# mynameisfiber/baton

Measured on NVIDIA H100. Metric: federated local samples/sec (whole box), ResNet-18 FedAvg, synthetic non-IID 32x32 shards, higher is better.
Workload: dtype bf16

## Files before the change

### baton_b200/build_ext.py

```python
from __future__ import annotations

import os
import shutil
import subprocess
import sys
import sysconfig
import time
from concurrent.futures import ThreadPoolExecutor

HERE = os.path.dirname(os.path.abspath(__file__))
CSRC = os.path.join(HERE, "csrc")
BUILD = os.path.join(HERE, "csrc", "build")
TRACE = os.environ.get("BATON_BUILD_TRACE") == "1"
if TRACE:
    BUILD = os.path.join(HERE, "csrc", "build_trace")
TARGET = os.path.join(HERE, "_C_trace.so" if TRACE else "_C.so")

CU_SOURCES = ["gemm_wgmma.cu", "gemm_fp8.cu", "quant.cu", "attention.cu", "im2col_tma.cu", "gemm_simt.cu", "fedavg.cu", "elementwise.cu", "conv.cu", "norm.cu", "loss.cu", "conv_halo.cu"]
HEADERS = ["ptx.cuh", "launch.h", "pdl.cuh", "mx.cuh", "sgd.cuh", "dp.cuh", "epilogue.cuh"]
NVCC_FLAGS = ["-gencode", "arch=compute_90a,code=sm_90a", "-lineinfo", "-O3", "-std=c++17",
              "-Xcompiler", "-fPIC", "--use_fast_math", "-Xptxas", "-v"]
if os.environ.get("BATON_BUILD_PHASE_TIMING") == "1":
    NVCC_FLAGS.append("-DB200_FEDAVG_PHASE_TIMING")
if TRACE:
    NVCC_FLAGS += ["-DB200_TRACE", "-DB200_FEDAVG_PHASE_TIMING"]


def _nvcc() -> str:
    for cand in (os.environ.get("CUDA_HOME", "") + "/bin/nvcc", "/usr/local/cuda/bin/nvcc", shutil.which("nvcc") or ""):
        if cand and os.path.exists(cand):
            return cand
    raise RuntimeError("nvcc not found")


def _newer(src_paths, out_path) -> bool:
    if not os.path.exists(out_path):
        return True
    t = os.path.getmtime(out_path)
    return any(os.path.getmtime(p) > t for p in src_paths)


def _run(cmd, verbose, log_path=None):
    proc = subprocess.run(cmd, stdout=subprocess.PIPE, stderr=subprocess.STDOUT, text=True)
    if log_path:
        with open(log_path, "w") as f:
            f.write(" ".join(cmd) + "\n" + proc.stdout)
    if proc.returncode != 0:
        sys.stderr.write(proc.stdout)
        raise RuntimeError("build step failed: {}".format(" ".join(cmd[:3])))
    if verbose:
        sys.stdout.write(proc.stdout)


def build(force: bool = False, verbose: bool = False) -> str:
    import torch
    from torch.utils import cpp_extension

    os.makedirs(BUILD, exist_ok=True)
    nvcc = _nvcc()
    stamp = os.path.join(BUILD, "flags.txt")
    want = "\n".join([nvcc] + NVCC_FLAGS + [torch.__version__]) + "\n"
    if not force and (not os.path.exists(stamp) or open(stamp).read() != want):
        force = True
    headers = [os.path.join(CSRC, h) for h in HEADERS]
    t0 = time.time()
    jobs = []
    objs = []
    for cu in CU_SOURCES:
        src = os.path.join(CSRC, cu)
        obj = os.path.join(BUILD, cu.replace(".cu", ".o"))
        objs.append(obj)
        if force or _newer([src] + headers, obj):
            jobs.append(([nvcc] + NVCC_FLAGS + ["-I", CSRC, "-c", src, "-o", obj], obj + ".log"))
    bind_src = os.path.join(CSRC, "bindings.cpp")
    bind_obj = os.path.join(BUILD, "bindings.o")
    objs.append(bind_obj)
    if force or _newer([bind_src] + headers, bind_obj):
        inc = []
        for p in cpp_extension.include_paths("cuda") if hasattr(cpp_extension, "include_paths") else []:
            inc += ["-isystem", p]
        inc += ["-isystem", sysconfig.get_paths()["include"]]
        abi = int(getattr(torch._C, "_GLIBCXX_USE_CXX11_ABI", True))
        jobs.append((["g++", "-O2", "-std=c++17", "-fPIC", "-DTORCH_EXTENSION_NAME=_C",
                      "-DTORCH_API_INCLUDE_EXTENSION_H", "-D_GLIBCXX_USE_CXX11_ABI={}".format(abi),
                      "-I", CSRC] + inc + ["-c", bind_src, "-o", bind_obj], bind_obj + ".log"))
    if jobs:
        with ThreadPoolExecutor(max_workers=min(8, len(jobs))) as pool:
            list(pool.map(lambda j: _run(j[0], verbose, j[1]), jobs))
    if jobs or force or not os.path.exists(TARGET):
        torch_lib = os.path.join(os.path.dirname(torch.__file__), "lib")
        cuda_lib = os.path.join(os.path.dirname(os.path.dirname(nvcc)), "lib64")
        link = ["g++", "-shared", "-o", TARGET] + objs + [
            "-L" + torch_lib, "-L" + cuda_lib, "-lc10", "-lc10_cuda", "-ltorch_cpu", "-ltorch_cuda", "-ltorch",
            "-ltorch_python", "-lcudart", "-Wl,-rpath," + torch_lib, "-Wl,--no-as-needed"]
        _run(link, verbose)
    with open(stamp, "w") as fh:
        fh.write(want)
    if verbose:
        print("built {} in {:.1f}s ({} compile steps)".format(TARGET, time.time() - t0, len(jobs)))
    return TARGET


if __name__ == "__main__":
    build(force="--force" in sys.argv, verbose="--verbose" in sys.argv or "-v" in sys.argv)
    print(TARGET)
```

### baton_b200/csrc/bindings.cpp

```cpp
#include <ATen/cuda/CUDAContext.h>
#include <c10/cuda/CUDAGuard.h>
#include <torch/extension.h>

#include <optional>
#include <vector>

#include "launch.h"

namespace {

inline cudaStream_t cur_stream() { return at::cuda::getCurrentCUDAStream().stream(); }
inline void check(int rc, const char* what) {
  TORCH_CHECK(rc == 0, "baton_b200::", what, " failed with code ", rc,
              rc > 0 ? std::string(" (") + cudaGetErrorString(static_cast<cudaError_t>(rc)) + ")" : std::string());
}
inline const void* cptr(const at::Tensor& t) { return t.data_ptr(); }
inline void* ptr(at::Tensor& t) { return t.data_ptr(); }
template <class T>
inline T* opt_ptr(const std::optional<at::Tensor>& t) {
  return (t.has_value() && t->defined()) ? reinterpret_cast<T*>(t->data_ptr()) : nullptr;
}
#define CHECK_CUDA(x) TORCH_CHECK((x).is_cuda(), #x " must be a CUDA tensor")

inline const float* prox_anchor(const std::optional<at::Tensor>& anchor, int64_t numel, const at::Tensor& hyper) {
  if (!anchor.has_value() || !anchor->defined()) return nullptr;
  CHECK_CUDA(*anchor);
  TORCH_CHECK(anchor->scalar_type() == at::kFloat && anchor->is_contiguous() && anchor->numel() >= numel,
              "prox anchor: contiguous fp32 covering the parameters");
  TORCH_CHECK(hyper.numel() >= 5, "prox anchor: hyper needs 5 floats {lr, momentum, weight_decay, dampening, prox_mu}");
  return anchor->data_ptr<float>();
}

inline const float* scaf_corr(const std::optional<at::Tensor>& corr, int64_t numel, const float* anchor) {
  if (!corr.has_value() || !corr->defined()) return nullptr;
  CHECK_CUDA(*corr);
  TORCH_CHECK(corr->scalar_type() == at::kFloat && corr->is_contiguous() && corr->numel() >= numel,
              "scaffold correction: contiguous fp32 covering the parameters");
  TORCH_CHECK(anchor == nullptr, "an SGD step takes a FedProx anchor or a SCAFFOLD correction, not both");
  return corr->data_ptr<float>();
}

inline float* adam_v_ptr(const std::optional<at::Tensor>& v, int64_t numel, const float* mom, const at::Tensor& hyper,
                         const float* anchor, const float* corr) {
  if (!v.has_value() || !v->defined()) return nullptr;
  CHECK_CUDA(*v);
  TORCH_CHECK(v->scalar_type() == at::kFloat && v->is_contiguous() && v->numel() >= numel,
              "adamw second moment: contiguous fp32 covering the parameters");
  TORCH_CHECK(mom != nullptr, "an AdamW step needs the first-moment (momentum) buffer");
  TORCH_CHECK(hyper.numel() >= 12, "an AdamW step takes its step row (12 floats) as hyper");
  TORCH_CHECK(anchor == nullptr && corr == nullptr, "an AdamW step takes no FedProx anchor or SCAFFOLD correction");
  return v->data_ptr<float>();
}

inline std::optional<B200SgdEpilogue> sgd_epilogue(const std::optional<at::Tensor>& theta,
                                                   const std::optional<at::Tensor>& theta_bf16,
                                                   const std::optional<at::Tensor>& mom,
                                                   const std::optional<at::Tensor>& hyper, bool nesterov,
                                                   const std::optional<at::Tensor>& anchor,
                                                   const std::optional<at::Tensor>& corr,
                                                   const std::optional<at::Tensor>& adam_v) {
  if (!hyper.has_value() || !hyper->defined()) return std::nullopt;
  TORCH_CHECK(theta.has_value() && theta->scalar_type() == at::kFloat && hyper->scalar_type() == at::kFloat &&
                  (!theta_bf16.has_value() || theta_bf16->scalar_type() == at::kBFloat16) &&
                  (!mom.has_value() || mom->scalar_type() == at::kFloat),
              "sgd epilogue: fp32 theta / momentum / hyper, bf16 shadow");
  const float* a = prox_anchor(anchor, theta->numel(), *hyper);
  const float* c = scaf_corr(corr, 0, a);
  return B200SgdEpilogue{theta->data_ptr<float>(), opt_ptr<void>(theta_bf16), opt_ptr<float>(mom),
                         hyper->data_ptr<float>(), nesterov ? 1 : 0, a, c,
                         adam_v_ptr(adam_v, 0, opt_ptr<float>(mom), *hyper, a, c)};
}

inline std::optional<B200AffineEpilogue> affine_epilogue(const std::optional<at::Tensor>& scale,
                                                         const std::optional<at::Tensor>& shift,
                                                         const std::optional<at::Tensor>& residual, bool relu,
                                                         int64_t rows, int64_t N) {
  if (!scale.has_value() || !scale->defined()) return std::nullopt;
  TORCH_CHECK(shift.has_value() && shift->defined(), "affine epilogue: scale without shift");
  CHECK_CUDA(*scale); CHECK_CUDA(*shift);
  TORCH_CHECK(scale->scalar_type() == at::kFloat && shift->scalar_type() == at::kFloat &&
                  scale->is_contiguous() && shift->is_contiguous() && scale->numel() >= N && shift->numel() >= N,
              "affine epilogue: fp32 [N] scale / shift");
  long long ldr = 0;
  if (residual.has_value() && residual->defined()) {
    CHECK_CUDA(*residual);
    TORCH_CHECK(residual->scalar_type() == at::kBFloat16 && residual->stride(-1) == 1 && residual->size(-1) == N &&
                    residual->numel() >= rows * N,
                "affine epilogue: bf16 [rows, N] residual with unit inner stride");
    ldr = residual->dim() >= 2 ? residual->stride(-2) : N;
  }
  return B200AffineEpilogue{scale->data_ptr<float>(), shift->data_ptr<float>(), opt_ptr<const void>(residual), ldr,
                            relu ? 1 : 0};
}

extern "C" {
#define B200_TRACE_TUS(X) X(gemm_wgmma) X(gemm_fp8) X(quant) X(attention) X(im2col_tma) X(gemm_simt) X(fedavg) \
  X(elementwise) X(conv) X(norm) X(loss) X(conv_halo)
#define B200_DECL(tu) int b200_trace_set_##tu(unsigned long long* p);
B200_TRACE_TUS(B200_DECL)
#undef B200_DECL
}
bool trace_set(const std::optional<at::Tensor>& buf) {
  unsigned long long* p = nullptr;
  if (buf.has_value() && buf->defined()) {
    CHECK_CUDA(*buf);
    TORCH_CHECK(buf->scalar_type() == at::kLong && buf->is_contiguous() && buf->numel() >= 4, "trace buffer: int64 [2+2n]");
    p = reinterpret_cast<unsigned long long*>(buf->data_ptr());
  }
  int rc = 0;
#define B200_SET(tu) rc |= b200_trace_set_##tu(p);
  B200_TRACE_TUS(B200_SET)
#undef B200_SET
  return rc == 0;
}

bool gemm(const at::Tensor& a, const at::Tensor& b, at::Tensor d, const std::optional<at::Tensor>& bias, int64_t M,
          int64_t N, int64_t K, int64_t lda, int64_t ldb, int64_t ldd, bool a_mn, bool b_mn, int64_t act,
          int64_t split_k, bool accumulate, double alpha, const std::optional<at::Tensor>& flags, int64_t flag_epoch,
          int64_t flag_elem_off, int64_t flag_tile_elems, int64_t flag_bias_off, int64_t force_bn, bool simt,
          const std::optional<at::Tensor>& col_stats, const std::optional<at::Tensor>& flag_epoch_word,
          const std::optional<at::Tensor>& sgd_theta, const std::optional<at::Tensor>& sgd_theta_bf16,
          const std::optional<at::Tensor>& sgd_mom, const std::optional<at::Tensor>& sgd_hyper, bool sgd_nesterov,
          const std::optional<at::Tensor>& sgd_anchor, const std::optional<at::Tensor>& sgd_corr,
          const std::optional<at::Tensor>& sgd_v, const std::optional<at::Tensor>& bn_scale, const std::optional<at::Tensor>& bn_shift,
          const std::optional<at::Tensor>& residual, bool bn_relu) {
  CHECK_CUDA(a); CHECK_CUDA(b); CHECK_CUDA(d);
  TORCH_CHECK(a.scalar_type() == at::kBFloat16 && b.scalar_type() == at::kBFloat16, "gemm operands must be bf16");
  TORCH_CHECK(d.scalar_type() == at::kBFloat16 || d.scalar_type() == at::kFloat, "gemm output must be bf16/fp32");
  const c10::cuda::CUDAGuard guard(a.device());
  const int out_fp32 = d.scalar_type() == at::kFloat;
  const float* bp = opt_ptr<const float>(bias);
  TORCH_CHECK(!col_stats.has_value() || (!simt && col_stats->scalar_type() == at::kFloat && col_stats->numel() >= 2 * N),
              "col_stats needs the tensor-core path and a [2N] fp32 buffer");
  if (simt) {
    TORCH_CHECK(!sgd_hyper.has_value(), "the SIMT GEMM has no optimizer epilogue");
    TORCH_CHECK(!bn_scale.has_value(), "the SIMT GEMM has no BatchNorm epilogue");
    check(b200_gemm_simt(cptr(a), cptr(b), ptr(d), bp, M, N, K, lda, ldb, ldd, a_mn, b_mn, out_fp32, act, accumulate,
                         static_cast<float>(alpha), cur_stream()),
          "gemm_simt");
    return true;
  }
  const std::optional<B200SgdEpilogue> sgd =
      sgd_epilogue(sgd_theta, sgd_theta_bf16, sgd_mom, sgd_hyper, sgd_nesterov, sgd_anchor, sgd_corr, sgd_v);
  const std::optional<B200AffineEpilogue> affine = affine_epilogue(bn_scale, bn_shift, residual, bn_relu, M, N);
  const int rc = b200_gemm_bf16(cptr(a), cptr(b), ptr(d), bp, M, N, K, lda, ldb, ldd, a_mn, b_mn, out_fp32, act, split_k,
                                accumulate, static_cast<float>(alpha), opt_ptr<const uint32_t>(flags),
                                static_cast<uint32_t>(flag_epoch), flag_elem_off, static_cast<int>(flag_tile_elems),
                                flag_bias_off, static_cast<int>(force_bn), opt_ptr<float>(col_stats),
                                opt_ptr<const uint32_t>(flag_epoch_word), sgd ? &*sgd : nullptr,
                                affine ? &*affine : nullptr, cur_stream());
  if (rc == B200_SGD_EPILOGUE_DECLINED || rc == B200_AFFINE_EPILOGUE_DECLINED) return false;
  check(rc, "gemm_bf16");
  return true;
}

void gemm_batched(const at::Tensor& a, const at::Tensor& b, at::Tensor d, int64_t M, int64_t N, int64_t K, int64_t lda,
                  int64_t ldb, int64_t ldd, bool a_mn, bool b_mn, int64_t act, double alpha, int64_t n_outer,
                  int64_t n_inner, int64_t a_outer, int64_t a_inner, int64_t b_outer, int64_t b_inner, int64_t d_outer,
                  int64_t d_inner, bool accumulate) {
  CHECK_CUDA(a); CHECK_CUDA(b); CHECK_CUDA(d);
  TORCH_CHECK(a.scalar_type() == at::kBFloat16 && b.scalar_type() == at::kBFloat16, "gemm operands must be bf16");
  const c10::cuda::CUDAGuard guard(a.device());
  check(b200_gemm_bf16_batched(cptr(a), cptr(b), ptr(d), M, N, K, lda, ldb, ldd, a_mn, b_mn,
                               d.scalar_type() == at::kFloat, act, static_cast<float>(alpha), n_outer, n_inner, a_outer,
                               a_inner, b_outer, b_inner, d_outer, d_inner, accumulate, cur_stream()),
        "gemm_bf16_batched");
}

bool attention_fwd(const at::Tensor& qkv, at::Tensor out, at::Tensor probs, int64_t B, int64_t S, int64_t H, int64_t dh,
                   double scale) {
  CHECK_CUDA(qkv); CHECK_CUDA(out); CHECK_CUDA(probs);
  TORCH_CHECK(qkv.scalar_type() == at::kBFloat16 && out.scalar_type() == at::kBFloat16 &&
              probs.scalar_type() == at::kBFloat16 && qkv.is_contiguous() && out.is_contiguous() && probs.is_contiguous());
  const c10::cuda::CUDAGuard guard(qkv.device());
  const int rc = b200_attention_fwd(cptr(qkv), ptr(out), ptr(probs), static_cast<int>(B), static_cast<int>(S),
                                    static_cast<int>(H), static_cast<int>(dh), static_cast<float>(scale), cur_stream());
  if (rc == -2) return false;
  check(rc, "attention_fwd");
  return true;
}

bool im2col_tma_probe(const at::Tensor& x, at::Tensor col, int64_t kh, int64_t kw, int64_t stride, int64_t pad,
                      int64_t ho, int64_t wo) {
  CHECK_CUDA(x); CHECK_CUDA(col);
  TORCH_CHECK(x.scalar_type() == at::kBFloat16 && col.scalar_type() == at::kBFloat16 && x.dim() == 4 && x.is_contiguous() &&
              col.is_contiguous());
  const c10::cuda::CUDAGuard guard(x.device());
  const int rc = b200_im2col_tma_probe(cptr(x), ptr(col), static_cast<int>(x.size(0)), static_cast<int>(x.size(1)),
                                       static_cast<int>(x.size(2)), static_cast<int>(x.size(3)), static_cast<int>(kh),
                                       static_cast<int>(kw), static_cast<int>(stride), static_cast<int>(pad),
                                       static_cast<int>(ho), static_cast<int>(wo), cur_stream());
  if (rc == -2) return false;
  check(rc, "im2col_tma_probe");
  return true;
}

bool attention_bwd(const at::Tensor& qkv, const at::Tensor& dout, const at::Tensor& probs, at::Tensor dqkv, int64_t B,
                   int64_t S, int64_t H, int64_t dh, double scale) {
  CHECK_CUDA(qkv); CHECK_CUDA(dout); CHECK_CUDA(probs); CHECK_CUDA(dqkv);
  TORCH_CHECK(qkv.scalar_type() == at::kBFloat16 && dout.scalar_type() == at::kBFloat16 &&
              probs.scalar_type() == at::kBFloat16 && dqkv.scalar_type() == at::kBFloat16 && qkv.is_contiguous() &&
              dout.is_contiguous() && probs.is_contiguous() && dqkv.is_contiguous());
  const c10::cuda::CUDAGuard guard(qkv.device());
  const int rc = b200_attention_bwd(cptr(qkv), cptr(dout), cptr(probs), ptr(dqkv), static_cast<int>(B), static_cast<int>(S),
                                    static_cast<int>(H), static_cast<int>(dh), static_cast<float>(scale), cur_stream());
  if (rc == -2) return false;
  check(rc, "attention_bwd");
  return true;
}

bool conv_igemm_fwd(const at::Tensor& x, const at::Tensor& w, at::Tensor y, int64_t kh, int64_t kw, int64_t stride,
                    int64_t pad, int64_t ho, int64_t wo, int64_t cluster_k, int64_t force_bn,
                    const std::optional<at::Tensor>& col_stats, const std::optional<at::Tensor>& bn_scale,
                    const std::optional<at::Tensor>& bn_shift, const std::optional<at::Tensor>& residual, bool bn_relu) {
  CHECK_CUDA(x); CHECK_CUDA(w); CHECK_CUDA(y);
  TORCH_CHECK(x.scalar_type() == at::kBFloat16 && w.scalar_type() == at::kBFloat16 && y.scalar_type() == at::kBFloat16 &&
              x.dim() == 4 && x.is_contiguous() && w.is_contiguous() && y.is_contiguous());
  TORCH_CHECK(y.numel() == x.size(0) * ho * wo * w.size(0), "conv_igemm_fwd: y must hold [N*Ho*Wo, Cout] elements");
  const c10::cuda::CUDAGuard guard(x.device());
  const std::optional<B200AffineEpilogue> affine =
      affine_epilogue(bn_scale, bn_shift, residual, bn_relu, x.size(0) * ho * wo, w.size(0));
  const int rc = b200_conv_igemm_fwd(cptr(x), cptr(w), ptr(y), static_cast<int>(x.size(0)), static_cast<int>(x.size(1)),
                                     static_cast<int>(x.size(2)), static_cast<int>(x.size(3)), static_cast<int>(w.size(0)),
                                     static_cast<int>(kh), static_cast<int>(kw), static_cast<int>(stride),
                                     static_cast<int>(pad), static_cast<int>(ho), static_cast<int>(wo),
                                     static_cast<int>(cluster_k), static_cast<int>(force_bn), opt_ptr<float>(col_stats),
                                     affine ? &*affine : nullptr, cur_stream());
  if (rc == -2 || rc == B200_AFFINE_EPILOGUE_DECLINED) return false;
  check(rc, "conv_igemm_fwd");
  return true;
}
bool conv_igemm_dgrad(const at::Tensor& dy, const at::Tensor& w, at::Tensor dx, int64_t kh, int64_t kw, int64_t pad,
                      int64_t cluster_k, int64_t force_bn) {
  CHECK_CUDA(dy); CHECK_CUDA(w); CHECK_CUDA(dx);
  TORCH_CHECK(dy.scalar_type() == at::kBFloat16 && w.scalar_type() == at::kBFloat16 && dx.scalar_type() == at::kBFloat16 &&
              dy.dim() == 4 && dx.dim() == 4 && dy.is_contiguous() && w.is_contiguous() && dx.is_contiguous());
  const c10::cuda::CUDAGuard guard(dy.device());
  const int rc = b200_conv_igemm_dgrad(cptr(dy), cptr(w), ptr(dx), static_cast<int>(dx.size(0)), static_cast<int>(dx.size(1)),
                                       static_cast<int>(dx.size(2)), static_cast<int>(dx.size(3)), static_cast<int>(dy.size(3)),
                                       static_cast<int>(kh), static_cast<int>(kw), static_cast<int>(pad),
                                       static_cast<int>(dy.size(1)), static_cast<int>(dy.size(2)),
                                       static_cast<int>(cluster_k), static_cast<int>(force_bn), cur_stream());
  if (rc == -2) return false;
  check(rc, "conv_igemm_dgrad");
  return true;
}
bool conv_halo(const at::Tensor& src, const at::Tensor& w, at::Tensor out, bool dgrad, int64_t mc,
               const std::optional<at::Tensor>& col_stats) {
  CHECK_CUDA(src); CHECK_CUDA(w); CHECK_CUDA(out);
  TORCH_CHECK(src.scalar_type() == at::kBFloat16 && w.scalar_type() == at::kBFloat16 && out.scalar_type() == at::kBFloat16 &&
              src.dim() == 4 && src.size(3) == 64 && src.is_contiguous() && w.is_contiguous() && out.is_contiguous());
  const int64_t rows = src.size(0) * src.size(1) * src.size(2);
  TORCH_CHECK(rows > 0 && out.numel() % rows == 0, "conv_halo: out must hold [N*H*W, Nout] elements");
  const int64_t nout = out.numel() / rows;
  TORCH_CHECK(w.numel() == (dgrad ? 64 * 9 * nout : nout * 9 * 64), "conv_halo: w must be [Cout, 9*Cin]");
  TORCH_CHECK(dgrad ? !col_stats.has_value()
                    : (!col_stats.has_value() || (col_stats->scalar_type() == at::kFloat && col_stats->numel() >= 2 * nout)),
              "conv_halo: col_stats is a [2 Cout] fp32 buffer of the forward");
  const c10::cuda::CUDAGuard guard(src.device());
  const int rc = b200_conv_halo(cptr(src), cptr(w), ptr(out), static_cast<int>(src.size(0)), static_cast<int>(src.size(1)),
                                static_cast<int>(src.size(2)), static_cast<int>(nout), dgrad ? 1 : 0,
                                static_cast<int>(mc), opt_ptr<float>(col_stats), cur_stream());
  if (rc == -2) return false;
  check(rc, "conv_halo");
  return true;
}
bool conv_igemm_dgrad_s2(const at::Tensor& dy, const at::Tensor& w, at::Tensor dx, int64_t kh, int64_t kw,
                         const std::vector<int64_t>& ntaps, const std::vector<int64_t>& taps, int64_t force_bn) {
  CHECK_CUDA(dy); CHECK_CUDA(w); CHECK_CUDA(dx);
  TORCH_CHECK(dy.scalar_type() == at::kBFloat16 && w.scalar_type() == at::kBFloat16 && dx.scalar_type() == at::kBFloat16 &&
              dy.dim() == 4 && dx.dim() == 4 && dy.is_contiguous() && w.is_contiguous() && dx.is_contiguous());
  TORCH_CHECK(ntaps.size() == 4 && taps.size() == 16, "conv_igemm_dgrad_s2: 4 classes x 4 taps");
  int nt[4], tw[16];
  for (int i = 0; i < 4; ++i) nt[i] = static_cast<int>(ntaps[i]);
  for (int i = 0; i < 16; ++i) tw[i] = static_cast<int>(taps[i]);
  const c10::cuda::CUDAGuard guard(dy.device());
  const int rc = b200_conv_igemm_dgrad_s2(cptr(dy), cptr(w), ptr(dx), static_cast<int>(dx.size(0)),
                                          static_cast<int>(dx.size(1)), static_cast<int>(dx.size(2)),
                                          static_cast<int>(dx.size(3)), static_cast<int>(dy.size(3)), static_cast<int>(kh),
                                          static_cast<int>(kw), static_cast<int>(dy.size(1)), static_cast<int>(dy.size(2)),
                                          nt, tw, static_cast<int>(force_bn), cur_stream());
  if (rc == -2) return false;
  check(rc, "conv_igemm_dgrad_s2");
  return true;
}
bool conv_igemm_wgrad(const at::Tensor& dy, const at::Tensor& x, at::Tensor dw, int64_t cout, int64_t kh, int64_t kw,
                      int64_t stride, int64_t pad, int64_t ho, int64_t wo, int64_t split_k, int64_t force_bn,
                      const std::optional<at::Tensor>& sgd_theta, const std::optional<at::Tensor>& sgd_theta_bf16,
                      const std::optional<at::Tensor>& sgd_mom, const std::optional<at::Tensor>& sgd_hyper,
                      bool sgd_nesterov, const std::optional<at::Tensor>& sgd_anchor,
                      const std::optional<at::Tensor>& sgd_corr, const std::optional<at::Tensor>& sgd_v) {
  CHECK_CUDA(dy); CHECK_CUDA(x); CHECK_CUDA(dw);
  TORCH_CHECK(x.scalar_type() == at::kBFloat16 && dy.scalar_type() == at::kBFloat16 && dw.scalar_type() == at::kFloat &&
              x.dim() == 4 && x.is_contiguous() && dy.is_contiguous());
  const c10::cuda::CUDAGuard guard(x.device());
  const std::optional<B200SgdEpilogue> sgd =
      sgd_epilogue(sgd_theta, sgd_theta_bf16, sgd_mom, sgd_hyper, sgd_nesterov, sgd_anchor, sgd_corr, sgd_v);
  const int rc = b200_conv_igemm_wgrad(cptr(dy), cptr(x), dw.data_ptr<float>(), static_cast<int>(x.size(0)),
                                       static_cast<int>(x.size(1)), static_cast<int>(x.size(2)), static_cast<int>(x.size(3)),
                                       static_cast<int>(cout), static_cast<int>(kh), static_cast<int>(kw),
                                       static_cast<int>(stride), static_cast<int>(pad), static_cast<int>(ho),
                                       static_cast<int>(wo), static_cast<int>(split_k), static_cast<int>(force_bn),
                                       sgd ? &*sgd : nullptr, cur_stream());
  if (rc == -2 || rc == B200_SGD_EPILOGUE_DECLINED) return false;
  check(rc, "conv_igemm_wgrad");
  return true;
}

void gemm_fp8(const at::Tensor& a, const at::Tensor& b, at::Tensor d, const std::optional<at::Tensor>& bias,
              const std::optional<at::Tensor>& sfa, const std::optional<at::Tensor>& sfb, int64_t M, int64_t N, int64_t K,
              int64_t lda, int64_t ldb, int64_t ldd, int64_t act, int64_t split_k, bool accumulate, double alpha) {
  CHECK_CUDA(a); CHECK_CUDA(b); CHECK_CUDA(d);
  TORCH_CHECK(a.element_size() == 1 && b.element_size() == 1, "gemm_fp8 operands must be 1-byte (e4m3)");
  const c10::cuda::CUDAGuard guard(a.device());
  check(b200_gemm_fp8(cptr(a), cptr(b), ptr(d), opt_ptr<const float>(bias), opt_ptr<const void>(sfa),
                      opt_ptr<const void>(sfb), M, N, K, lda, ldb, ldd, d.scalar_type() == at::kFloat, act, split_k,
                      accumulate, static_cast<float>(alpha), cur_stream()),
        "gemm_fp8");
}
void quant_mx_rows(const at::Tensor& x, at::Tensor q, at::Tensor sf, int64_t R, int64_t C, int64_t ld_in, int64_t Cp) {
  CHECK_CUDA(x);
  const c10::cuda::CUDAGuard guard(x.device());
  check(b200_quant_mx_rows(x.data_ptr(), q.data_ptr(), sf.data_ptr(), R, C, ld_in, Cp, cur_stream()), "quant_mx_rows");
}
void quant_mx_cols(const at::Tensor& x, at::Tensor q, at::Tensor sf, int64_t R, int64_t C, int64_t ld_in, int64_t Rp) {
  CHECK_CUDA(x);
  const c10::cuda::CUDAGuard guard(x.device());
  check(b200_quant_mx_cols(x.data_ptr(), q.data_ptr(), sf.data_ptr(), R, C, ld_in, Rp, cur_stream()), "quant_mx_cols");
}
void dequant_mx(const at::Tensor& q, const at::Tensor& sf, at::Tensor out, int64_t R, int64_t C, int64_t Cp) {
  CHECK_CUDA(q);
  const c10::cuda::CUDAGuard guard(q.device());
  check(b200_dequant_mx(q.data_ptr(), sf.data_ptr(), out.data_ptr<float>(), R, C, Cp, cur_stream()), "dequant_mx");
}

void fused_sgd(at::Tensor w, at::Tensor g, const std::optional<at::Tensor>& mom, const std::optional<at::Tensor>& wb,
               const at::Tensor& hyper, bool zero_grad, bool nesterov, const std::optional<at::Tensor>& wire_slot,
               const std::optional<at::Tensor>& pack_global, const std::optional<at::Tensor>& pack_scale, int64_t n_pack,
               bool wire_fp32, const std::optional<at::Tensor>& prox_anchor_, const std::optional<at::Tensor>& corr,
               const std::optional<at::Tensor>& adam_v) {
  CHECK_CUDA(w);
  TORCH_CHECK(w.scalar_type() == at::kFloat && g.scalar_type() == at::kFloat && hyper.scalar_type() == at::kFloat);
  TORCH_CHECK(w.is_contiguous() && g.is_contiguous() && w.numel() == g.numel());
  const c10::cuda::CUDAGuard guard(w.device());
  const float* anchor = prox_anchor(prox_anchor_, w.numel(), hyper);
  const float* c = scaf_corr(corr, w.numel(), anchor);
  check(b200_fused_sgd(w.data_ptr<float>(), g.data_ptr<float>(), opt_ptr<float>(mom), opt_ptr<void>(wb), w.numel(),
                       hyper.data_ptr<float>(), zero_grad, nesterov,
                       reinterpret_cast<const unsigned long long*>(opt_ptr<const int64_t>(wire_slot)),
                       opt_ptr<const float>(pack_global), opt_ptr<const float>(pack_scale), n_pack, wire_fp32, anchor,
                       c, adam_v_ptr(adam_v, w.numel(), opt_ptr<float>(mom), hyper, anchor, c), cur_stream()),
        "fused_sgd");
}

void fused_sgd_segments(at::Tensor w, at::Tensor g, const std::optional<at::Tensor>& mom,
                        const std::optional<at::Tensor>& wb, const at::Tensor& segments, const at::Tensor& hyper,
                        bool nesterov, const std::optional<at::Tensor>& prox_anchor_,
                        const std::optional<at::Tensor>& corr, const std::optional<at::Tensor>& adam_v) {
  CHECK_CUDA(w); CHECK_CUDA(segments);
  TORCH_CHECK(w.scalar_type() == at::kFloat && g.scalar_type() == at::kFloat && hyper.scalar_type() == at::kFloat);
  TORCH_CHECK(segments.scalar_type() == at::kLong && segments.dim() == 2 && segments.size(1) == 3 &&
              segments.is_contiguous(), "segments: contiguous int64 [n, 3]");
  const c10::cuda::CUDAGuard guard(w.device());
  const float* anchor = prox_anchor(prox_anchor_, w.numel(), hyper);
  const float* c = scaf_corr(corr, g.numel(), anchor);
  check(b200_fused_sgd_segments(w.data_ptr<float>(), g.data_ptr<float>(), opt_ptr<float>(mom), opt_ptr<void>(wb),
                                reinterpret_cast<const long long*>(segments.data_ptr<int64_t>()),
                                static_cast<int>(segments.size(0)), hyper.data_ptr<float>(), nesterov, anchor, c,
                                adam_v_ptr(adam_v, g.numel(), opt_ptr<float>(mom), hyper, anchor, c), cur_stream()),
        "fused_sgd_segments");
}

inline void check_cv(const at::Tensor& t, int64_t n) {
  CHECK_CUDA(t);
  TORCH_CHECK(t.scalar_type() == at::kFloat && t.is_contiguous() && t.numel() >= n,
              "scaffold: contiguous fp32 buffers covering the parameters");
}
void scaffold_corr(at::Tensor corr, const at::Tensor& c, const at::Tensor& ci) {
  const int64_t n = corr.numel();
  check_cv(corr, n); check_cv(c, n); check_cv(ci, n);
  const c10::cuda::CUDAGuard guard(corr.device());
  check(b200_scaffold_corr(corr.data_ptr<float>(), c.data_ptr<float>(), ci.data_ptr<float>(), n, cur_stream()),
        "scaffold_corr");
}
void scaffold_dc(at::Tensor up, at::Tensor ci, const at::Tensor& c, const at::Tensor& global_w, const at::Tensor& theta,
                 double inv_k_eta, bool first) {
  const int64_t n = up.numel();
  check_cv(up, n); check_cv(ci, n); check_cv(c, n); check_cv(global_w, n); check_cv(theta, n);
  const c10::cuda::CUDAGuard guard(up.device());
  check(b200_scaffold_dc(up.data_ptr<float>(), ci.data_ptr<float>(), c.data_ptr<float>(), global_w.data_ptr<float>(),
                         theta.data_ptr<float>(), n, static_cast<float>(inv_k_eta), first ? 1 : 0, cur_stream()),
        "scaffold_dc");
}

void fold_client(at::Tensor acc, at::Tensor theta, const at::Tensor& global_w, const std::optional<at::Tensor>& wb,
                 const std::optional<at::Tensor>& mom, double nk, int64_t mode, bool reset) {
  CHECK_CUDA(acc);
  TORCH_CHECK(acc.scalar_type() == at::kFloat && theta.scalar_type() == at::kFloat && global_w.scalar_type() == at::kFloat);
  TORCH_CHECK(acc.numel() == theta.numel() && theta.numel() == global_w.numel());
  const c10::cuda::CUDAGuard guard(acc.device());
  check(b200_fold_client(acc.data_ptr<float>(), theta.data_ptr<float>(), global_w.data_ptr<float>(), opt_ptr<void>(wb),
                         opt_ptr<float>(mom), mom.has_value() && mom->defined() ? mom->numel() : 0, theta.numel(),
                         static_cast<float>(nk), static_cast<int>(mode), reset, cur_stream()),
        "fold_client");
}

void weighted_sum(at::Tensor dst, const std::vector<at::Tensor>& srcs, const std::vector<double>& weights) {
  CHECK_CUDA(dst);
  TORCH_CHECK(srcs.size() == weights.size() && !srcs.empty() && srcs.size() <= B200_MAX_RANKS);
  TORCH_CHECK(dst.is_contiguous());
  const c10::cuda::CUDAGuard guard(dst.device());
  std::vector<const void*> ps;
  std::vector<float> ws;
  for (size_t i = 0; i < srcs.size(); ++i) {
    TORCH_CHECK(srcs[i].is_cuda() && srcs[i].is_contiguous() && srcs[i].scalar_type() == dst.scalar_type() &&
                srcs[i].numel() == dst.numel());
    ps.push_back(srcs[i].data_ptr());
// ... 363 lines not shown
  if (rc == -2) return false;
  check(rc, "bn_relu_maxpool");
  return true;
}
bool bn_maxpool_bwd(const at::Tensor& z, const at::Tensor& p, const at::Tensor& arg, const at::Tensor& dy_a,
                    const std::optional<at::Tensor>& dy_b, at::Tensor dz, const std::optional<at::Tensor>& gamma,
                    const at::Tensor& mean, const at::Tensor& rstd, at::Tensor sums, const std::optional<at::Tensor>& dgamma,
                    const std::optional<at::Tensor>& dbeta, int64_t N, int64_t H, int64_t W, int64_t C, int64_t k,
                    int64_t stride, int64_t pad, int64_t Ho, int64_t Wo) {
  CHECK_CUDA(z);
  const c10::cuda::CUDAGuard guard(z.device());
  const int rc = b200_bn_maxpool_bwd(z.data_ptr(), p.data_ptr(), arg.data_ptr(), dy_a.data_ptr(), opt_ptr<const void>(dy_b),
                                     dz.data_ptr(), opt_ptr<const float>(gamma), mean.data_ptr<float>(),
                                     rstd.data_ptr<float>(), sums.data_ptr<float>(), opt_ptr<float>(dgamma),
                                     opt_ptr<float>(dbeta), static_cast<int>(N), static_cast<int>(H), static_cast<int>(W),
                                     static_cast<int>(C), static_cast<int>(k), static_cast<int>(stride),
                                     static_cast<int>(pad), static_cast<int>(Ho), static_cast<int>(Wo), cur_stream());
  if (rc == -2) return false;
  check(rc, "bn_maxpool_bwd");
  return true;
}
bool bn_bwd_cluster(const at::Tensor& x, const at::Tensor& y, const at::Tensor& dy_a, const std::optional<at::Tensor>& dy_b,
                    at::Tensor dx, const std::optional<at::Tensor>& dres, const std::optional<at::Tensor>& gamma,
                    const at::Tensor& mean, const at::Tensor& rstd, const std::optional<at::Tensor>& dgamma,
                    const std::optional<at::Tensor>& dbeta, int64_t rows, int64_t C, bool relu, int64_t max_cluster) {
  CHECK_CUDA(x);
  const c10::cuda::CUDAGuard guard(x.device());
  const int rc = b200_bn_bwd_cluster(x.data_ptr(), y.data_ptr(), dy_a.data_ptr(), opt_ptr<const void>(dy_b), dx.data_ptr(),
                                     opt_ptr<void>(dres), opt_ptr<const float>(gamma), mean.data_ptr<float>(),
                                     rstd.data_ptr<float>(), opt_ptr<float>(dgamma), opt_ptr<float>(dbeta), rows, C, relu,
                                     static_cast<int>(max_cluster), cur_stream());
  if (rc == -2) return false;
  check(rc, "bn_bwd_cluster");
  return true;
}
void bn_fold_eval(const at::Tensor& arena, const at::Tensor& table, at::Tensor out) {
  CHECK_CUDA(arena); CHECK_CUDA(table); CHECK_CUDA(out);
  TORCH_CHECK(arena.scalar_type() == at::kFloat && out.scalar_type() == at::kFloat && table.scalar_type() == at::kLong &&
                  table.dim() == 2 && table.size(1) == 7 && table.is_contiguous() && out.is_contiguous(),
              "bn_fold_eval: fp32 arena / out, int64 [n, 7] table");
  const c10::cuda::CUDAGuard guard(arena.device());
  check(b200_bn_fold_eval(arena.data_ptr<float>(), reinterpret_cast<const long long*>(table.data_ptr<int64_t>()),
                          static_cast<int>(table.size(0)), out.data_ptr<float>(), cur_stream()),
        "bn_fold_eval");
}
void layernorm_fwd(const at::Tensor& x, const std::optional<at::Tensor>& res, at::Tensor y, const at::Tensor& gamma,
                   const at::Tensor& beta, at::Tensor mean, at::Tensor rstd, int64_t rows, int64_t C, double eps) {
  CHECK_CUDA(x);
  const c10::cuda::CUDAGuard guard(x.device());
  check(b200_layernorm_fwd(x.data_ptr(), opt_ptr<const void>(res), y.data_ptr(), gamma.data_ptr<float>(),
                           beta.data_ptr<float>(), mean.data_ptr<float>(), rstd.data_ptr<float>(), rows, C,
                           static_cast<float>(eps), cur_stream()),
        "layernorm_fwd");
}
void layernorm_bwd(const at::Tensor& x, const at::Tensor& dy, at::Tensor dx, const at::Tensor& gamma,
                   const at::Tensor& mean, const at::Tensor& rstd, at::Tensor dgamma, at::Tensor dbeta, int64_t rows,
                   int64_t C) {
  CHECK_CUDA(x);
  const c10::cuda::CUDAGuard guard(x.device());
  check(b200_layernorm_bwd(x.data_ptr(), dy.data_ptr(), dx.data_ptr(), gamma.data_ptr<float>(), mean.data_ptr<float>(),
                           rstd.data_ptr<float>(), dgamma.data_ptr<float>(), dbeta.data_ptr<float>(), rows, C,
                           cur_stream()),
        "layernorm_bwd");
}
void softmax_fwd(const at::Tensor& x, at::Tensor y, int64_t rows, int64_t C, double scale) {
  CHECK_CUDA(x);
  const c10::cuda::CUDAGuard guard(x.device());
  check(b200_softmax_fwd(x.data_ptr(), y.data_ptr(), rows, C, static_cast<float>(scale), cur_stream()), "softmax_fwd");
}
void softmax_bwd(const at::Tensor& y, const at::Tensor& dy, at::Tensor dx, int64_t rows, int64_t C, double scale) {
  CHECK_CUDA(y);
  const c10::cuda::CUDAGuard guard(y.device());
  check(b200_softmax_bwd(y.data_ptr(), dy.data_ptr(), dx.data_ptr(), rows, C, static_cast<float>(scale), cur_stream()),
        "softmax_bwd");
}

void softmax_xent(const at::Tensor& logits, const at::Tensor& target, const std::optional<at::Tensor>& dlogits,
                  at::Tensor loss_acc, int64_t rows, int64_t C, int64_t ld, double grad_scale) {
  CHECK_CUDA(logits);
  TORCH_CHECK(target.scalar_type() == at::kLong && loss_acc.scalar_type() == at::kFloat && loss_acc.numel() >= 2);
  const c10::cuda::CUDAGuard guard(logits.device());
  const int in32 = logits.scalar_type() == at::kFloat;
  const int out32 = dlogits.has_value() && dlogits->defined() && dlogits->scalar_type() == at::kFloat;
  check(b200_softmax_xent(logits.data_ptr(), in32, reinterpret_cast<const long long*>(target.data_ptr<int64_t>()),
                          opt_ptr<void>(dlogits), out32, loss_acc.data_ptr<float>(), rows, C, ld,
                          static_cast<float>(grad_scale), cur_stream()),
        "softmax_xent");
}
bool linear_xent_head(const at::Tensor& x, const at::Tensor& w, const std::optional<at::Tensor>& bias, const at::Tensor& target,
                      const std::optional<at::Tensor>& dx, at::Tensor dw, const std::optional<at::Tensor>& db,
                      at::Tensor loss_acc, const std::optional<at::Tensor>& logits_out, double grad_scale) {
  CHECK_CUDA(x);
  TORCH_CHECK(x.scalar_type() == at::kBFloat16 && w.scalar_type() == at::kBFloat16 && x.dim() == 2 && w.dim() == 2 &&
              x.is_contiguous() && w.is_contiguous() && x.size(1) == w.size(1));
  TORCH_CHECK(target.scalar_type() == at::kLong && dw.scalar_type() == at::kFloat && dw.is_contiguous() &&
              dw.numel() == w.numel() && loss_acc.scalar_type() == at::kFloat && loss_acc.numel() >= 2);
  const c10::cuda::CUDAGuard guard(x.device());
  const int rc = b200_linear_xent_head(x.data_ptr(), w.data_ptr(), opt_ptr<const float>(bias),
                                       reinterpret_cast<const long long*>(target.data_ptr<int64_t>()), opt_ptr<void>(dx),
                                       dw.data_ptr<float>(), opt_ptr<float>(db), loss_acc.data_ptr<float>(),
                                       opt_ptr<float>(logits_out), static_cast<int>(x.size(0)), static_cast<int>(x.size(1)),
                                       static_cast<int>(w.size(0)), static_cast<float>(grad_scale), cur_stream());
  if (rc == -2) return false;
  check(rc, "linear_xent_head");
  return true;
}
bool linear_xent_eval(const at::Tensor& x, const at::Tensor& w, const std::optional<at::Tensor>& bias, const at::Tensor& target,
                      at::Tensor loss_acc, const std::optional<at::Tensor>& logits_out) {
  CHECK_CUDA(x);
  TORCH_CHECK(x.scalar_type() == at::kBFloat16 && w.scalar_type() == at::kBFloat16 && x.dim() == 2 && w.dim() == 2 &&
              x.is_contiguous() && w.is_contiguous() && x.size(1) == w.size(1));
  TORCH_CHECK(target.scalar_type() == at::kLong && target.numel() >= x.size(0) && loss_acc.scalar_type() == at::kFloat &&
              loss_acc.numel() >= 2);
  TORCH_CHECK(!bias.has_value() || (bias->scalar_type() == at::kFloat && bias->numel() == w.size(0)));
  TORCH_CHECK(!logits_out.has_value() || (logits_out->scalar_type() == at::kFloat && logits_out->is_contiguous() &&
                                          logits_out->numel() == x.size(0) * w.size(0)));
  const c10::cuda::CUDAGuard guard(x.device());
  const int rc = b200_linear_xent_eval(x.data_ptr(), w.data_ptr(), opt_ptr<const float>(bias),
                                       reinterpret_cast<const long long*>(target.data_ptr<int64_t>()),
                                       loss_acc.data_ptr<float>(), opt_ptr<float>(logits_out), static_cast<int>(x.size(0)),
                                       static_cast<int>(x.size(1)), static_cast<int>(w.size(0)), cur_stream());
  if (rc == -2) return false;
  check(rc, "linear_xent_eval");
  return true;
}
void mse(const at::Tensor& pred, const at::Tensor& target, const std::optional<at::Tensor>& dpred, at::Tensor loss_acc,
         double grad_scale) {
  CHECK_CUDA(pred);
  TORCH_CHECK(target.scalar_type() == at::kFloat && target.numel() == pred.numel());
  const c10::cuda::CUDAGuard guard(pred.device());
  const int in32 = pred.scalar_type() == at::kFloat;
  const int out32 = dpred.has_value() && dpred->defined() && dpred->scalar_type() == at::kFloat;
  check(b200_mse(pred.data_ptr(), in32, target.data_ptr<float>(), opt_ptr<void>(dpred), out32,
                 loss_acc.data_ptr<float>(), pred.numel(), static_cast<float>(grad_scale), cur_stream()),
        "mse");
}

}

PYBIND11_MODULE(TORCH_EXTENSION_NAME, m) {
  m.doc() = "baton_b200 sm_90a kernels";
  m.attr("MAX_RANKS") = B200_MAX_RANKS;
  m.def("gemm", &gemm);
  m.def("trace_set", &trace_set);
  m.def("attention_fwd", &attention_fwd);
  m.def("attention_bwd", &attention_bwd);
  m.def("bn_bwd_cluster", &bn_bwd_cluster);
  m.def("im2col_tma_probe", &im2col_tma_probe);
  m.def("conv_igemm_fwd", &conv_igemm_fwd);
  m.def("conv_igemm_wgrad", &conv_igemm_wgrad);
  m.def("conv_igemm_dgrad", &conv_igemm_dgrad);
  m.def("conv_igemm_dgrad_s2", &conv_igemm_dgrad_s2);
  m.def("conv_halo", &conv_halo);
  m.def("gemm_batched", &gemm_batched);
  m.def("gemm_fp8", &gemm_fp8);
  m.def("quant_mx_rows", &quant_mx_rows);
  m.def("quant_mx_cols", &quant_mx_cols);
  m.def("dequant_mx", &dequant_mx);
  m.def("fused_sgd", &fused_sgd);
  m.def("fused_sgd_segments", &fused_sgd_segments);
  m.def("weighted_sum", &weighted_sum);
  m.def("fold_client", &fold_client);
  m.def("scaffold_corr", &scaffold_corr);
  m.def("scaffold_dc", &scaffold_dc);
  m.def("cast", &cast);
  m.def("gather_rows", &gather_rows);
  m.def("colsum", &colsum);
  m.def("add_bf16", &add_bf16);
  m.def("relu_bwd", &relu_bwd);
  m.def("gelu", &gelu);
  m.def("gelu_bwd", &gelu_bwd);
  m.def("pad_rows", &pad_rows);
  m.def("embedding_bwd", &embedding_bwd);
  m.def("fedavg_allreduce", &fedavg_allreduce);
  m.def("fedavg_allreduce_robust", &fedavg_allreduce_robust);
  m.def("pack_client", &pack_client);
  m.attr("MAX_ROBUST_CLIENTS") = B200_MAX_ROBUST_CLIENTS;
  m.def("flag_barrier", &flag_barrier);
  m.attr("DP_WORK_WORDS") = B200_DP_WORK_WORDS;
  m.def("dp_clip_factor", &dp_clip_factor);
  m.def("fold_client_scaled", &fold_client_scaled);
  m.def("im2col", &im2col);
  m.def("col2im", &col2im);
  m.def("maxpool", &maxpool);
  m.def("maxpool_bwd", &maxpool_bwd);
  m.def("avgpool", &avgpool);
  m.def("avgpool_bwd", &avgpool_bwd);
  m.def("bn_stats", &bn_stats);
  m.def("bn_apply", &bn_apply);
  m.def("bn_bwd_reduce", &bn_bwd_reduce);
  m.def("bn_bwd_apply", &bn_bwd_apply);
  m.def("bn_relu_maxpool", &bn_relu_maxpool);
  m.def("bn_maxpool_bwd", &bn_maxpool_bwd);
  m.def("layernorm_fwd", &layernorm_fwd);
  m.def("layernorm_bwd", &layernorm_bwd);
  m.def("softmax_fwd", &softmax_fwd);
  m.def("softmax_bwd", &softmax_bwd);
  m.def("softmax_xent", &softmax_xent);
  m.def("mse", &mse);
  m.def("linear_xent_head", &linear_xent_head);
  m.def("linear_xent_eval", &linear_xent_eval);
  m.def("bn_fold_eval", &bn_fold_eval);
}
```

### baton_b200/csrc/epilogue.cuh

```cuda
#pragma once
#include "ptx.cuh"

namespace b200 {

__device__ __forceinline__ uint32_t cluster_ctarank() {
  uint32_t r;
  asm volatile("mov.u32 %0, %%cluster_ctarank;" : "=r"(r));
  return r;
}
__device__ __forceinline__ void cluster_sync_all() {
  asm volatile("barrier.cluster.arrive.release.aligned;" ::: "memory");
  asm volatile("barrier.cluster.wait.acquire.aligned;" ::: "memory");
}

#define COLSUM_STEP(OFF, HALF)                                                  \
  {                                                                             \
    const bool upper = (lane & (OFF)) != 0;                                     \
    _Pragma("unroll") for (int i = 0; i < (HALF); ++i) {                        \
      const float keep = upper ? t[i + (HALF)] : t[i];                          \
      const float send = upper ? t[i] : t[i + (HALF)];                          \
      t[i] = keep + __shfl_xor_sync(0xffffffffu, send, (OFF));                  \
    }                                                                           \
  }
__device__ __forceinline__ float warp_colsum32(float (&t)[32]) {
  const uint32_t lane = lane_id();
  COLSUM_STEP(16, 16) COLSUM_STEP(8, 8) COLSUM_STEP(4, 4) COLSUM_STEP(2, 2) COLSUM_STEP(1, 1)
  return t[0];
}
#undef COLSUM_STEP

__device__ __forceinline__ void stage_col_stats(float* sbuf, int BNv, int c, const float (&v)[32]) {
  float s[32], q[32];
#pragma unroll
  for (int j = 0; j < 32; ++j) {
    const float r = __bfloat162float(__float2bfloat16_rn(v[j]));
    s[j] = r;
    q[j] = r * r;
  }
  const float cs = warp_colsum32(s), cq = warp_colsum32(q);
  const int lane = static_cast<int>(lane_id());
  sbuf[c + lane] = cs;
  sbuf[BNv + c + lane] = cq;
}

}
```

### baton_b200/csrc/gemm_wgmma.cu

```cuda
#define B200_TU_TAG 1
#include "ptx.cuh"
#include "epilogue.cuh"
#include "launch.h"
#include "pdl.cuh"
#include "sgd.cuh"

namespace b200 {

constexpr int BM = 128;
constexpr int BK = 64;
constexpr int WG_K = 16;
constexpr int GEMM_THREADS = 384;
constexpr int CONSUMER_WARPS = 8;
constexpr int CONSUMER_THREADS = 32 * CONSUMER_WARPS;
constexpr int MAX_STAGES = 8;
constexpr int S2_MAX_TAPS = 4;

struct GemmParams {
  int M, N, K;
  void* D;
  long long ldd;
  const float* bias;
  int out_fp32;
  int act;
  float* col_stats;
  int a_mn, b_mn;
  int k_tiles_per_split;
  int atomic_out;
  int cluster_k;
  int stages;
  const uint32_t* tile_flags;
  uint32_t flag_epoch;
  long long flag_elem_off;
  int flag_tile_elems;
  long long flag_bias_off;
  long long ldb;
  float alpha;
  int batched, batch_inner;
  int batch_count;
  long long d_outer, d_inner;
  int conv_ho, conv_wo;
  int conv_stride, conv_pad;
  int conv_kw;
  int conv_cin;
  int conv_taps;
  int conv_ncol;
  const uint32_t* flag_epoch_ptr;
  const float* sgd_hyper = nullptr;
  float* sgd_theta = nullptr;
  __nv_bfloat16* sgd_wb = nullptr;
  float* sgd_mom = nullptr;
  int sgd_nesterov = 0;
  int conv_h = 0, conv_w = 0;
  int s2_ntaps[4] = {0, 0, 0, 0};
  int s2_tap[4][S2_MAX_TAPS] = {};
  const float* bn_scale = nullptr;
  const float* bn_shift = nullptr;
  const __nv_bfloat16* residual = nullptr;
  long long ldr = 0;
  const float* sgd_anchor = nullptr;
  const float* sgd_corr = nullptr;
  float* sgd_v = nullptr;
};

__device__ __forceinline__ void wait_arrival_flags(const uint32_t* flags, long long e0, long long e1, int granule,
                                                   uint32_t need) {
  for (long long t = e0 / granule; t <= e1 / granule; ++t) {
    unsigned long long spins = 0;
    while (static_cast<int32_t>(ld_acquire_sys(flags + t) - need) < 0) {
      if (++spins > (1ull << 26)) break;
    }
  }
}

template <int BN>
struct SmemLayout {
  static constexpr int A_BYTES = BM * BK * 2;
  static constexpr int B_BYTES = BN * BK * 2;
  static constexpr int STAGE_BYTES = A_BYTES + B_BYTES;
  static constexpr int PART_PITCH = BN + 4;
  static constexpr int PART_BYTES = BM * PART_PITCH * 4;
};

__device__ __forceinline__ float apply_act(float v, int act) {
  if (act == 1) return fmaxf(v, 0.f);
  if (act == 2) {
    const float k0 = 0.7978845608028654f, k1 = 0.044715f;
    float t = tanhf(k0 * (v + k1 * v * v * v));
    return 0.5f * v * (1.f + t);
  }
  return v;
}

__device__ __forceinline__ float4 ld_dsmem_f4(uint32_t local_smem_addr, uint32_t cta_rank) {
  uint32_t remote;
  asm volatile("mapa.shared::cluster.u32 %0, %1, %2;" : "=r"(remote) : "r"(local_smem_addr), "r"(cta_rank));
  float4 v;
  asm volatile("ld.shared::cluster.v4.f32 {%0, %1, %2, %3}, [%4];"
               : "=f"(v.x), "=f"(v.y), "=f"(v.z), "=f"(v.w)
               : "r"(remote)
               : "memory");
  return v;
}

__device__ __forceinline__ void accumulate_col_stats(const GemmParams& p, int col0, const float (&v)[32]) {
  float s[32], q[32];
#pragma unroll
  for (int j = 0; j < 32; ++j) {
    const float r = __bfloat162float(__float2bfloat16_rn(v[j]));
    s[j] = r;
    q[j] = r * r;
  }
  const float cs = warp_colsum32(s), cq = warp_colsum32(q);
  const int col = col0 + static_cast<int>(lane_id());
  if (col < p.N) {
    atomicAdd(p.col_stats + col, cs);
    atomicAdd(p.col_stats + p.N + col, cq);
  }
}

template <int NV, int ACT, bool BIAS>
__device__ __forceinline__ void transform_chunk_t(const GemmParams& p, int col0, float (&v)[NV]) {
  float b[NV];
  if (BIAS) {
    if (col0 + NV <= p.N && ((reinterpret_cast<uintptr_t>(p.bias + col0) & 15) == 0)) {
#pragma unroll
      for (int j = 0; j < NV; j += 4) {
        const float4 t = __ldg(reinterpret_cast<const float4*>(p.bias + col0 + j));
        b[j] = t.x; b[j + 1] = t.y; b[j + 2] = t.z; b[j + 3] = t.w;
      }
    } else {
#pragma unroll
      for (int j = 0; j < NV; ++j) b[j] = (col0 + j) < p.N ? __ldg(p.bias + col0 + j) : 0.f;
    }
  }
  const float alpha = p.alpha;
#pragma unroll
  for (int j = 0; j < NV; ++j) {
    float x = v[j] * alpha;
    if (BIAS) x += b[j];
    if (ACT == 1) x = fmaxf(x, 0.f);
    if (ACT == 2) {
      const float k0 = 0.7978845608028654f, k1 = 0.044715f;
      x = 0.5f * x * (1.f + tanhf(k0 * (x + k1 * x * x * x)));
    }
    v[j] = x;
  }
}
template <int NV>
__device__ __forceinline__ void transform_chunk(const GemmParams& p, int col0, float (&v)[NV]) {
  if (p.bias == nullptr) {
    if (p.act == 0) transform_chunk_t<NV, 0, false>(p, col0, v);
    else if (p.act == 1) transform_chunk_t<NV, 1, false>(p, col0, v);
    else transform_chunk_t<NV, 2, false>(p, col0, v);
  } else {
    if (p.act == 0) transform_chunk_t<NV, 0, true>(p, col0, v);
    else if (p.act == 1) transform_chunk_t<NV, 1, true>(p, col0, v);
    else transform_chunk_t<NV, 2, true>(p, col0, v);
  }
}

template <int NV>
__device__ __forceinline__ void affine_chunk(const GemmParams& p, int row, int col0, float (&v)[NV]) {
  static_assert(NV % 8 == 0, "affine epilogue works on groups of 8 columns");
  const bool relu = p.act == 1;
  const __nv_bfloat16* res = p.residual != nullptr ? p.residual + static_cast<size_t>(row) * p.ldr + col0 : nullptr;
#pragma unroll
  for (int j = 0; j < NV; j += 8) {
    if (col0 + j >= p.N) break;
    const float4 s0 = __ldg(reinterpret_cast<const float4*>(p.bn_scale + col0 + j));
    const float4 s1 = __ldg(reinterpret_cast<const float4*>(p.bn_scale + col0 + j + 4));
    const float4 h0 = __ldg(reinterpret_cast<const float4*>(p.bn_shift + col0 + j));
    const float4 h1 = __ldg(reinterpret_cast<const float4*>(p.bn_shift + col0 + j + 4));
    const float sc[8] = {s0.x, s0.y, s0.z, s0.w, s1.x, s1.y, s1.z, s1.w};
    const float sh[8] = {h0.x, h0.y, h0.z, h0.w, h1.x, h1.y, h1.z, h1.w};
    float r[8] = {0.f, 0.f, 0.f, 0.f, 0.f, 0.f, 0.f, 0.f};
    if (res != nullptr) {
      const uint4 rv = *reinterpret_cast<const uint4*>(res + j);
      const uint32_t rw[4] = {rv.x, rv.y, rv.z, rv.w};
#pragma unroll
      for (int i = 0; i < 4; ++i) {
        const float2 f = unpack_bf16x2(rw[i]);
        r[2 * i] = f.x;
        r[2 * i + 1] = f.y;
      }
    }
#pragma unroll
    for (int i = 0; i < 8; ++i) {
      const float x = fmaf(v[j + i], sc[i], sh[i]) + r[i];
      v[j + i] = relu ? fmaxf(x, 0.f) : x;
    }
  }
}

template <int NV, bool AFFINE = false>
__device__ __forceinline__ void store_row_chunk(const GemmParams& p, int row, int col0, float (&v)[NV], bool vec_ok,
                                                size_t d_off = 0) {
  if constexpr (AFFINE)
    affine_chunk<NV>(p, row, col0, v);
  else
    transform_chunk<NV>(p, col0, v);
  const bool full = (col0 + NV <= p.N);
  if (p.out_fp32) {
    float* d = reinterpret_cast<float*>(p.D) + d_off + static_cast<size_t>(row) * p.ldd + col0;
    if (p.atomic_out) {
      if (full && vec_ok) {
#pragma unroll
        for (int j = 0; j < NV; j += 4)
          asm volatile("red.global.add.v4.f32 [%0], {%1, %2, %3, %4};" ::"l"(d + j), "f"(v[j]), "f"(v[j + 1]),
                       "f"(v[j + 2]), "f"(v[j + 3])
                       : "memory");
      } else {
        _Pragma("unroll") for (int j = 0; j < NV; ++j) if (col0 + j < p.N) atomicAdd(d + j, v[j]);
      }
    } else if (full && vec_ok) {
#pragma unroll
      for (int j = 0; j < NV; j += 4) *reinterpret_cast<float4*>(d + j) = make_float4(v[j], v[j + 1], v[j + 2], v[j + 3]);
    } else {
      _Pragma("unroll") for (int j = 0; j < NV; ++j) if (col0 + j < p.N) d[j] = v[j];
    }
  } else {
    __nv_bfloat16* d = reinterpret_cast<__nv_bfloat16*>(p.D) + d_off + static_cast<size_t>(row) * p.ldd + col0;
    if (full && vec_ok) {
#pragma unroll
      for (int j = 0; j < NV; j += 8) {
        uint4 o;
        o.x = pack_bf16x2(v[j], v[j + 1]);
        o.y = pack_bf16x2(v[j + 2], v[j + 3]);
        o.z = pack_bf16x2(v[j + 4], v[j + 5]);
        o.w = pack_bf16x2(v[j + 6], v[j + 7]);
        *reinterpret_cast<uint4*>(d + j) = o;
      }
    } else {
      _Pragma("unroll") for (int j = 0; j < NV; ++j) if (col0 + j < p.N) d[j] = __float2bfloat16_rn(v[j]);
    }
  }
}

template <bool PROX, bool SCAF = false>
__device__ __forceinline__ void sgd_epilogue_chunk(const GemmParams& p, size_t e, int col0, const float (&v)[32],
                                                   bool vec);

__device__ __forceinline__ void adamw_epilogue_chunk(const GemmParams& p, size_t e, int col0, const float (&v)[32],
                                                     bool vec) {
  const AdamHyper h = load_adam_hyper(p.sgd_hyper);
  float* w = p.sgd_theta + e;
  float* m = p.sgd_mom + e;
  float* sq = p.sgd_v + e;
  __nv_bfloat16* wb = p.sgd_wb != nullptr ? p.sgd_wb + e : nullptr;
  if (vec && col0 + 32 <= p.N) {
#pragma unroll
    for (int j = 0; j < 32; j += 4) {
      float4 mv = *reinterpret_cast<const float4*>(m + j), vv = *reinterpret_cast<const float4*>(sq + j);
      const float4 gv = make_float4(__fadd_rn(0.f, v[j]), __fadd_rn(0.f, v[j + 1]), __fadd_rn(0.f, v[j + 2]),
                                    __fadd_rn(0.f, v[j + 3]));
      const float4 wv = adamw_update4(h, *reinterpret_cast<const float4*>(w + j), gv, mv, vv);
      *reinterpret_cast<float4*>(w + j) = wv;
// ... 1246 lines not shown
```

### baton_b200/csrc/launch.h

```cpp
#pragma once
#include <cuda_runtime.h>
#include <stdint.h>

#define B200_MAX_RANKS 16

extern "C" {

struct B200SgdEpilogue {
  float* theta;
  void* theta_bf16;
  float* mom;
  const float* hyper;
  int nesterov;
  const float* anchor;
  const float* corr;
  float* v;
};
#define B200_SGD_EPILOGUE_DECLINED (-6)

struct B200AffineEpilogue {
  const float* scale;
  const float* shift;
  const void* residual;
  long long ldr;
  int relu;
};
#define B200_AFFINE_EPILOGUE_DECLINED (-7)

int b200_gemm_bf16(const void* a, const void* b, void* d, const float* bias, int M, int N, int K, long long lda,
                   long long ldb, long long ldd, int a_mn, int b_mn, int out_fp32, int act, int split_k, int accumulate,
                   float alpha, const uint32_t* tile_flags, uint32_t flag_epoch, long long flag_elem_off, int flag_tile_elems,
                   long long flag_bias_off, int force_bn, float* col_stats, const uint32_t* flag_epoch_ptr,
                   const B200SgdEpilogue* sgd, const B200AffineEpilogue* affine, cudaStream_t stream);
int b200_gemm_bf16_batched(const void* a, const void* b, void* d, int M, int N, int K, long long lda, long long ldb,
                           long long ldd, int a_mn, int b_mn, int out_fp32, int act, float alpha, int n_outer,
                           int n_inner, long long a_outer, long long a_inner, long long b_outer, long long b_inner,
                           long long d_outer, long long d_inner, int accumulate, cudaStream_t stream);
int b200_attention_fwd(const void* qkv, void* out, void* probs, int B, int S, int H, int dh, float scale,
                       cudaStream_t stream);
int b200_attention_bwd(const void* qkv, const void* dout, const void* probs, void* dqkv, int B, int S, int H, int dh,
                       float scale, cudaStream_t stream);
int b200_conv_igemm_fwd(const void* x, const void* w, void* y, int N, int H, int W, int Cin, int Cout, int KH, int KW,
                        int stride, int pad, int Ho, int Wo, int cluster_k, int force_bn, float* col_stats,
                        const B200AffineEpilogue* affine, cudaStream_t stream);
int b200_conv_igemm_dgrad(const void* dy, const void* w, void* dx, int N, int H, int W, int Cin, int Cout, int KH, int KW,
                          int pad, int Ho, int Wo, int cluster_k, int force_bn, cudaStream_t stream);
int b200_conv_igemm_dgrad_s2(const void* dy, const void* w, void* dx, int N, int H, int W, int Cin, int Cout, int KH,
                             int KW, int Ho, int Wo, const int* ntaps, const int* taps, int force_bn, cudaStream_t stream);
int b200_conv_igemm_wgrad(const void* dy, const void* x, float* dw, int N, int H, int W, int Cin, int Cout, int KH, int KW,
                          int stride, int pad, int Ho, int Wo, int split_k, int force_bn, const B200SgdEpilogue* sgd,
                          cudaStream_t stream);
int b200_conv_halo(const void* src, const void* w, void* out, int N, int H, int W, int Nout, int dgrad, int mc,
                   float* col_stats, cudaStream_t stream);
int b200_im2col_tma_probe(const void* x, void* col, int N, int H, int W, int C, int KH, int KW, int stride, int pad,
                          int Ho, int Wo, cudaStream_t stream);
int b200_gemm_fp8(const void* a, const void* b, void* d, const float* bias, const void* sfa, const void* sfb, int M, int N,
                  int K, long long lda, long long ldb, long long ldd, int out_fp32, int act, int split_k, int accumulate,
                  float alpha, cudaStream_t stream);
int b200_quant_mx_rows(const void* x, void* q, void* sf, long long R, int C, long long ld_in, int Cp, cudaStream_t stream);
int b200_quant_mx_cols(const void* x, void* q, void* sf, long long R, int C, long long ld_in, long long Rp,
                       cudaStream_t stream);
int b200_dequant_mx(const void* q, const void* sf, float* out, long long R, int C, int Cp, cudaStream_t stream);
int b200_gemm_simt(const void* a, const void* b, void* d, const float* bias, int M, int N, int K, long long lda,
                   long long ldb, long long ldd, int a_mn, int b_mn, int out_fp32, int act, int accumulate,
                   float alpha, cudaStream_t stream);

int b200_fused_sgd(float* w, float* g, float* mom, void* w_bf16, long long n, const float* hyper, int zero_grad,
                   int nesterov, const unsigned long long* wire_slot, const float* pack_global,
                   const float* pack_scale, long long n_pack, int wire_fp32, const float* prox_anchor,
                   const float* corr, float* adam_v, cudaStream_t stream);
int b200_fused_sgd_segments(float* w, float* g, float* mom, void* w_bf16, const long long* segments, int n_seg,
                            const float* hyper, int nesterov, const float* prox_anchor, const float* corr,
                            float* adam_v, cudaStream_t stream);
int b200_scaffold_corr(float* corr, const float* c, const float* ci, long long n, cudaStream_t stream);
int b200_scaffold_dc(float* up, float* ci, const float* c, const float* global_w, const float* theta, long long n,
                     float inv_k_eta, int first, cudaStream_t stream);
int b200_fold_client(float* acc, float* theta, const float* global_w, void* w_bf16, float* mom, long long n_mom, long long n,
                     float nk, int mode, int reset, cudaStream_t stream);
int b200_weighted_sum(void* dst, const void* const* srcs, const float* weights, int n_src, long long n, int dtype,
                      cudaStream_t stream);
int b200_cast_f32_bf16(const float* src, void* dst, long long n, cudaStream_t stream);
int b200_cast_bf16_f32(const void* src, float* dst, long long n, cudaStream_t stream);
int b200_gather_rows(const void* src, const long long* idx, void* dst, long long n_rows, long long row_bytes,
                     cudaStream_t stream);
int b200_gather_rows_i64(const long long* src, const long long* idx, long long* dst, long long n,
                         cudaStream_t stream);
int b200_colsum(const void* x, float* out, long long rows, int cols, int accumulate, cudaStream_t stream);
int b200_add_bf16(const void* a, const void* b, void* out, long long n, int relu, cudaStream_t stream);
int b200_relu_bwd_bf16(const void* y, const void* dy, void* dx, long long n, cudaStream_t stream);
int b200_gelu_bf16(const void* x, void* y, long long n, cudaStream_t stream);
int b200_gelu_bwd_bf16(const void* x, const void* dy, void* dx, long long n, cudaStream_t stream);
int b200_embedding_bwd(const void* dy, const long long* idx, float* grad, long long n_rows, int width,
                       cudaStream_t stream);
int b200_pad_rows_bf16(const void* src, void* dst, long long rows, int k, int kp, const uint32_t* flags,
                       const uint32_t* epoch_word, long long elem_off, int granule, cudaStream_t stream);

struct FedAvgArgs {
  void* wire[B200_MAX_RANKS];
  unsigned long long* pads[B200_MAX_RANKS];
  void* wire_mc;
  float* theta;
  float* global_w;
  void* theta_bf16;
  float* momentum;
  long long n_momentum;
  long long* int_local;
  long long* int_wire[B200_MAX_RANKS];
  float* loss_local;
  float* loss_wire[B200_MAX_RANKS];
  float* loss_out;
  int n_loss;
  float n_samples[B200_MAX_RANKS];
  int counts_from_flags;
  float nvls_prescale;
  uint32_t alive_mask;
  int rank, world;
  long long n;
  int n_int;
  int wire_kind;
  int delta;
  int use_nvls;
  uint32_t epoch;
  uint32_t* tile_flags;
  uint32_t flag_value;
  int tile_elems;
  int prepacked;
  int timeout_log2;
  int* status;
  unsigned long long* phase_ns;
};
struct FedAvgDPArgs : FedAvgArgs {
  const float* clip_page[B200_MAX_RANKS];
  float noise_std;
  unsigned long long seed;
  uint32_t round;
};
struct FedAvgScaffoldArgs : FedAvgArgs {
  const float* dc;
  float* c;
  long long n_c;
  long long seg1_off;
  float inv_clients;
};
#define B200_MAX_ROBUST_CLIENTS 32
struct FedAvgRobustArgs : FedAvgArgs {
  uint32_t* seg_page[B200_MAX_RANKS];
  uint32_t my_segs;
  long long seg_stride;
  int kind;
  uint8_t trim_b[B200_MAX_ROBUST_CLIENTS + 1];
};
int b200_fedavg_allreduce(const FedAvgArgs* args, int n_ctas, cudaStream_t stream);
int b200_fedavg_allreduce_robust(const FedAvgRobustArgs* args, int n_ctas, cudaStream_t stream);
int b200_pack_client(void* seg, float* theta, const float* global_w, void* w_bf16, float* mom, long long n_mom,
                     long long n, int wire_kind, int reset, cudaStream_t stream);
int b200_fedavg_allreduce_dp(const FedAvgDPArgs* args, int n_ctas, cudaStream_t stream);
int b200_fedavg_allreduce_scaffold(const FedAvgScaffoldArgs* args, int n_ctas, cudaStream_t stream);
#define B200_DP_NORM_BLOCKS 264
#define B200_DP_WORK_WORDS (B200_DP_NORM_BLOCKS + 1)
int b200_dp_clip_factor(const float* theta, const float* global_w, long long n, float clip, void* work, float* s_out,
                        float* norm_out, float* s_copy, int* nonfinite, cudaStream_t stream);
int b200_fold_client_scaled(float* acc, float* theta, const float* global_w, void* w_bf16, float* mom, long long n_mom,
                            long long n, const float* s, int first, int reset, cudaStream_t stream);
int b200_flag_barrier(unsigned long long* const* pads, int rank, int world, uint32_t alive_mask, uint32_t epoch,
                      int slot, cudaStream_t stream);

int b200_im2col_nhwc(const void* x, void* col, int N, int H, int W, int C, int KH, int KW, int stride, int pad,
                     int Ho, int Wo, int kp, cudaStream_t stream);
int b200_col2im_nhwc(const void* col, void* dx, int N, int H, int W, int C, int KH, int KW, int stride, int pad,
                     int Ho, int Wo, int kp, cudaStream_t stream);
int b200_maxpool_nhwc(const void* x, void* y, int* argmax, int N, int H, int W, int C, int k, int stride, int pad,
                      int Ho, int Wo, int arg_u8, cudaStream_t stream);
int b200_maxpool_bwd_nhwc(const void* dy, const void* dy_b, const int* argmax, void* dx, int N, int H, int W, int C, int Ho,
                          int Wo, int k, int stride, int pad, int arg_u8, cudaStream_t stream);
int b200_avgpool_nhwc(const void* x, void* y, int N, int HW, int C, cudaStream_t stream);
int b200_avgpool_bwd_nhwc(const void* dy, void* dx, int N, int HW, int C, cudaStream_t stream);

int b200_bn_stats(const void* x, float* sums, long long rows, int C, cudaStream_t stream);
int b200_bn_apply(const void* x, const void* residual, void* y, float* sums, const float* gamma, const float* beta,
                  float* running_mean, float* running_var, float* save_mean, float* save_rstd, long long* nbt,
                  long long rows, int C, float eps, float momentum, int relu, int training, cudaStream_t stream);
int b200_bn_bwd_reduce(const void* x, const void* y, const void* dy, const float* save_mean, const float* save_rstd,
                       float* sums, long long rows, int C, int relu, cudaStream_t stream);
int b200_bn_bwd_apply(const void* x, const void* y, const void* dy, void* dx, void* dres, const float* gamma,
                      const float* save_mean, const float* save_rstd, float* sums, float* dgamma, float* dbeta,
                      long long rows, int C, int relu, cudaStream_t stream);
int b200_bn_relu_maxpool(const void* z, void* p, void* argmax, const float* sums, const float* gamma, const float* beta,
                         float* running_mean, float* running_var, float* save_mean, float* save_rstd, long long* nbt, int N,
                         int H, int W, int C, int k, int stride, int pad, int Ho, int Wo, float eps, float momentum,
                         cudaStream_t stream);
int b200_bn_maxpool_bwd(const void* z, const void* p, const void* argmax, const void* dy_a, const void* dy_b, void* dz,
                        const float* gamma, const float* save_mean, const float* save_rstd, float* sums, float* dgamma,
                        float* dbeta, int N, int H, int W, int C, int k, int stride, int pad, int Ho, int Wo,
                        cudaStream_t stream);
int b200_bn_bwd_cluster(const void* x, const void* y, const void* dy_a, const void* dy_b, void* dx, void* dres,
                        const float* gamma, const float* save_mean, const float* save_rstd, float* dgamma, float* dbeta,
                        long long rows, int C, int relu, int max_cluster, cudaStream_t stream);
int b200_bn_fold_eval(const float* arena, const long long* table, int n_bn, float* out, cudaStream_t stream);
int b200_layernorm_fwd(const void* x, const void* residual, void* y, const float* gamma, const float* beta,
                       float* mean, float* rstd, long long rows, int C, float eps, cudaStream_t stream);
int b200_layernorm_bwd(const void* x, const void* dy, void* dx, const float* gamma, const float* mean,
                       const float* rstd, float* dgamma, float* dbeta, long long rows, int C, cudaStream_t stream);
int b200_softmax_fwd(const void* x, void* y, long long rows, int C, float scale, cudaStream_t stream);
int b200_softmax_bwd(const void* y, const void* dy, void* dx, long long rows, int C, float scale,
                     cudaStream_t stream);

int b200_softmax_xent(const void* logits, int logits_fp32, const long long* target, void* dlogits, int dl_fp32,
                      float* loss_acc, long long rows, int C, long long ld, float grad_scale, cudaStream_t stream);
int b200_linear_xent_head(const void* x, const void* w, const float* bias, const long long* target, void* dx, float* dw,
                          float* db, float* loss_acc, float* logits_out, int rows, int K, int NC, float grad_scale,
                          cudaStream_t stream);
int b200_linear_xent_eval(const void* x, const void* w, const float* bias, const long long* target, float* loss_acc,
                          float* logits_out, int rows, int K, int NC, cudaStream_t stream);
int b200_mse(const void* pred, int pred_fp32, const float* target, void* dpred, int dp_fp32, float* loss_acc,
             long long n, float grad_scale, cudaStream_t stream);
}
```

### baton_b200/csrc/norm.cu

```cuda
#define B200_TU_TAG 10
#include "launch.h"
#include "pdl.cuh"
#include "ptx.cuh"

namespace b200 {

__device__ __forceinline__ uint32_t cluster_ctarank_any() {
  uint32_t r;
  asm volatile("mov.u32 %0, %%cluster_ctarank;" : "=r"(r));
  return r;
}
__device__ __forceinline__ uint32_t cluster_nctarank_y() {
  uint32_t r;
  asm volatile("mov.u32 %0, %%cluster_nctarank;" : "=r"(r));
  return r;
}
__device__ __forceinline__ void cluster_arrive_norm() { asm volatile("barrier.cluster.arrive.release.aligned;" ::: "memory"); }
__device__ __forceinline__ void cluster_wait_norm() { asm volatile("barrier.cluster.wait.acquire.aligned;" ::: "memory"); }
__device__ __forceinline__ void cluster_sync_all_norm() {
  cluster_arrive_norm();
  cluster_wait_norm();
}
__device__ __forceinline__ float ld_dsmem_f1(uint32_t local_smem_addr, uint32_t cta_rank) {
  uint32_t remote;
// ... 489 lines not shown
          s1 += w;
          s2 = fmaf(w, h, s2);
        }
      }
    }
    s1 = group_sum<LPR>(s1) / C;
    s2 = group_sum<LPR>(s2) / C;
    if (row_ok) {
      uint4* dr = reinterpret_cast<uint4*>(dx + row * C);
#pragma unroll
      for (int k = 0; k < VPL; ++k) {
        const int idx = gl + k * LPR;
        if (idx < nvec) {
          float o[8];
#pragma unroll
          for (int j = 0; j < 8; ++j) o[j] = rs * (gw[k][j] - s1 - xh[k][j] * s2);
          dr[idx] = pack8(o);
        }
      }
    }
  }
#pragma unroll
  for (int k = 0; k < VPL; ++k) {
    const int idx = gl + k * LPR;
    if (idx < nvec) {
#pragma unroll
      for (int j = 0; j < 8; ++j) {
        atomicAdd(sg + idx * 8 + j, dg[k][j]);
        atomicAdd(sb + idx * 8 + j, db[k][j]);
      }
    }
  }
  __syncthreads();
  for (int c = threadIdx.x; c < C; c += blockDim.x) {
    atomicAdd(dgamma + c, sg[c]);
    atomicAdd(dbeta + c, sb[c]);
  }
}

template <int LPR, int VPL>
__global__ void __launch_bounds__(256)
softmax_fwd_vec_kernel(const __nv_bfloat16* __restrict__ x, __nv_bfloat16* __restrict__ y, long long rows, int C,
                       float scale) {
  griddep_launch_dependents();
  griddep_wait();
  constexpr int RPW = 32 / LPR;
  const int gl = threadIdx.x & (LPR - 1);
  const long long row = (blockIdx.x * static_cast<long long>(blockDim.x >> 5) + (threadIdx.x >> 5)) * RPW +
                        ((threadIdx.x & 31) / LPR);
  const bool row_ok = row < rows;
  const int nvec = C >> 3;
  const uint4* xr = reinterpret_cast<const uint4*>(x + (row_ok ? row : 0) * C);
  float v[VPL][8];
  float m = -INFINITY;
#pragma unroll
  for (int k = 0; k < VPL; ++k) {
    const int idx = gl + k * LPR;
    if (row_ok && idx < nvec) {
      unpack8(__ldcs(xr + idx), v[k]);
#pragma unroll
      for (int j = 0; j < 8; ++j) {
        v[k][j] *= scale;
        m = fmaxf(m, v[k][j]);
      }
    }
  }
  m = group_max<LPR>(m);
  float s = 0.f;
#pragma unroll
  for (int k = 0; k < VPL; ++k)
    if (row_ok && gl + k * LPR < nvec) {
#pragma unroll
      for (int j = 0; j < 8; ++j) {
        v[k][j] = __expf(v[k][j] - m);
        s += v[k][j];
      }
    }
  s = group_sum<LPR>(s);
  if (!row_ok) return;
  const float inv = 1.f / s;
  uint4* yr = reinterpret_cast<uint4*>(y + row * C);
#pragma unroll
  for (int k = 0; k < VPL; ++k) {
    const int idx = gl + k * LPR;
    if (idx < nvec) {
#pragma unroll
      for (int j = 0; j < 8; ++j) v[k][j] *= inv;
      yr[idx] = pack8(v[k]);
    }
  }
}

template <int LPR, int VPL>
__global__ void __launch_bounds__(256)
softmax_bwd_vec_kernel(const __nv_bfloat16* __restrict__ y, const __nv_bfloat16* __restrict__ dy,
                       __nv_bfloat16* __restrict__ dx, long long rows, int C, float scale) {
  griddep_launch_dependents();
  griddep_wait();
  constexpr int RPW = 32 / LPR;
  const int gl = threadIdx.x & (LPR - 1);
  const long long row = (blockIdx.x * static_cast<long long>(blockDim.x >> 5) + (threadIdx.x >> 5)) * RPW +
                        ((threadIdx.x & 31) / LPR);
  const bool row_ok = row < rows;
  const int nvec = C >> 3;
  const uint4* yr = reinterpret_cast<const uint4*>(y + (row_ok ? row : 0) * C);
  const uint4* gr = reinterpret_cast<const uint4*>(dy + (row_ok ? row : 0) * C);
  float p[VPL][8], g[VPL][8];
  float s = 0.f;
#pragma unroll
  for (int k = 0; k < VPL; ++k) {
    const int idx = gl + k * LPR;
    if (row_ok && idx < nvec) {
      unpack8(__ldcs(yr + idx), p[k]);
      unpack8(__ldcs(gr + idx), g[k]);
#pragma unroll
      for (int j = 0; j < 8; ++j) s = fmaf(p[k][j], g[k][j], s);
    }
  }
  s = group_sum<LPR>(s);
  if (!row_ok) return;
  uint4* dr = reinterpret_cast<uint4*>(dx + row * C);
#pragma unroll
  for (int k = 0; k < VPL; ++k) {
    const int idx = gl + k * LPR;
    if (idx < nvec) {
      float o[8];
#pragma unroll
      for (int j = 0; j < 8; ++j) o[j] = scale * p[k][j] * (g[k][j] - s);
      dr[idx] = pack8(o);
    }
  }
}

#define ROW_DISPATCH(C, CALL)                                     \
  do {                                                           \
    const int nvec_ = (C) >> 3;                                  \
    if (nvec_ <= 8) { CALL(8, 1); }                              \
    else if (nvec_ <= 16) { CALL(16, 1); }                       \
    else if (nvec_ <= 32) { CALL(32, 1); }                       \
    else if (nvec_ <= 64) { CALL(32, 2); }                       \
    else if (nvec_ <= 96) { CALL(32, 3); }                       \
    else { CALL(32, 4); }                                        \
  } while (0)
static inline bool row_vec_ok(int C, const void* a, const void* b, const void* c) {
  return C % 8 == 0 && C <= 1024 && ((reinterpret_cast<uintptr_t>(a) | reinterpret_cast<uintptr_t>(b) |
                                       reinterpret_cast<uintptr_t>(c)) & 15) == 0;
}
static inline int rows_per_block(int C) {
  const int nvec = C >> 3;
  return 8 * (nvec <= 8 ? 4 : (nvec <= 16 ? 2 : 1));
}


__device__ __forceinline__ void unpack8_bn(const uint4& u, float (&f)[8]) {
  const float2 a = unpack_bf16x2(u.x), b = unpack_bf16x2(u.y), c = unpack_bf16x2(u.z), d = unpack_bf16x2(u.w);
  f[0] = a.x; f[1] = a.y; f[2] = b.x; f[3] = b.y; f[4] = c.x; f[5] = c.y; f[6] = d.x; f[7] = d.y;
}
__device__ __forceinline__ void colred_finish(float (&a)[8], float (&q)[8], float* sm, int tpr, int cg, int rg,
                                              float* __restrict__ sums, int C) {
  float* mine = sm + static_cast<size_t>(rg) * 2 * C + cg * 8;
#pragma unroll
  for (int j = 0; j < 8; ++j) { mine[j] = a[j]; mine[C + j] = q[j]; }
  __syncthreads();
  const int rpp = 256 / tpr;
  for (int c = threadIdx.x; c < 2 * C; c += 256) {
    float t = 0.f;
    for (int r = 0; r < rpp; ++r) t += sm[static_cast<size_t>(r) * 2 * C + c];
    atomicAdd(sums + c, t);
  }
}

__global__ void __launch_bounds__(256)
bn_stats_vec_kernel(const uint4* __restrict__ x, float* __restrict__ sums, long long rows, int C, int rows_per_cta) {
  griddep_launch_dependents();
  griddep_wait();
  extern __shared__ float sm[];
  const int tpr = C >> 3, rpp = 256 / tpr;
  const int cg = threadIdx.x % tpr, rg = threadIdx.x / tpr;
  const long long r0 = static_cast<long long>(blockIdx.x) * rows_per_cta;
  long long r1 = r0 + rows_per_cta;
  if (r1 > rows) r1 = rows;
  float a[8], q[8];
#pragma unroll
  for (int j = 0; j < 8; ++j) { a[j] = 0.f; q[j] = 0.f; }
  for (long long r = r0 + rg; r < r1; r += 4ll * rpp) {
    uint4 v[4];
#pragma unroll
    for (int u = 0; u < 4; ++u)
      if (r + static_cast<long long>(u) * rpp < r1) v[u] = x[(r + static_cast<long long>(u) * rpp) * tpr + cg];
#pragma unroll
    for (int u = 0; u < 4; ++u)
      if (r + static_cast<long long>(u) * rpp < r1) {
        float f[8];
        unpack8_bn(v[u], f);
#pragma unroll
        for (int j = 0; j < 8; ++j) { a[j] += f[j]; q[j] = fmaf(f[j], f[j], q[j]); }
      }
  }
  colred_finish(a, q, sm, tpr, cg, rg, sums, C);
}

__global__ void __launch_bounds__(256)
bn_bwd_reduce_vec_kernel(const uint4* __restrict__ x, const uint4* __restrict__ y, const uint4* __restrict__ dy,
                         const float* __restrict__ mean, const float* __restrict__ rstd, float* __restrict__ sums,
                         long long rows, int C, int relu, int rows_per_cta) {
  griddep_launch_dependents();
  griddep_wait();
  extern __shared__ float sm[];
  const int tpr = C >> 3, rpp = 256 / tpr;
  const int cg = threadIdx.x % tpr, rg = threadIdx.x / tpr;
  const long long r0 = static_cast<long long>(blockIdx.x) * rows_per_cta;
  long long r1 = r0 + rows_per_cta;
  if (r1 > rows) r1 = rows;
  float m[8], rs[8], a[8], q[8];
#pragma unroll
  for (int j = 0; j < 8; ++j) { m[j] = mean[cg * 8 + j]; rs[j] = rstd[cg * 8 + j]; a[j] = 0.f; q[j] = 0.f; }
  for (long long r = r0 + rg; r < r1; r += 2ll * rpp) {
    uint4 xv[2], gv[2], yv[2];
#pragma unroll
    for (int u = 0; u < 2; ++u) {
      const long long rr = r + static_cast<long long>(u) * rpp;
      if (rr < r1) {
        xv[u] = x[rr * tpr + cg];
        gv[u] = dy[rr * tpr + cg];
        if (relu) yv[u] = y[rr * tpr + cg];
      }
    }
#pragma unroll
    for (int u = 0; u < 2; ++u) {
      if (r + static_cast<long long>(u) * rpp < r1) {
        float xf[8], gf[8];
        unpack8_bn(xv[u], xf);
        unpack8_bn(gv[u], gf);
        if (relu) {
          float yf[8];
          unpack8_bn(yv[u], yf);
#pragma unroll
          for (int j = 0; j < 8; ++j)
            if (!(yf[j] > 0.f)) gf[j] = 0.f;
        }
#pragma unroll
        for (int j = 0; j < 8; ++j) {
          a[j] += gf[j];
          q[j] = fmaf(gf[j], (xf[j] - m[j]) * rs[j], q[j]);
        }
      }
    }
  }
  colred_finish(a, q, sm, tpr, cg, rg, sums, C);
}


constexpr int BNC_CW = 16;
constexpr int BNC_LANES = 128;

template <int ITER>
__global__ void __launch_bounds__(256)
bn_bwd_cluster_kernel(const uint4* __restrict__ x, const uint4* __restrict__ y, const uint4* __restrict__ dy_a,
                      const uint4* __restrict__ dy_b, uint4* __restrict__ dx, uint4* __restrict__ dres,
                      const float* __restrict__ gamma, const float* __restrict__ mean, const float* __restrict__ rstd,
                      float* __restrict__ dgamma, float* __restrict__ dbeta, int rows, int C, int relu, int rows_per_cta) {
  griddep_launch_dependents();
  __shared__ float wpart[8][2][16];
  __shared__ __align__(16) float cpart[32];
  __shared__ float tot[32];
  const int chunk = threadIdx.x & 1, lane_r = threadIdx.x >> 1;
  const int c0 = blockIdx.x * BNC_CW + chunk * 8;
  const int C8 = C >> 3;
  const uint32_t S = cluster_nctarank_y();
  const uint32_t me = cluster_ctarank_any();
  const int r_begin = static_cast<int>(me) * rows_per_cta;
  int r_end = r_begin + rows_per_cta;
  if (r_end > rows) r_end = rows;
  float m[8], rs[8];
#pragma unroll
  for (int j = 0; j < 8; ++j) { m[j] = mean[c0 + j]; rs[j] = rstd[c0 + j]; }
  griddep_wait();
  constexpr int NC = ITER > 0 ? ITER : 1;
  float xh[NC][8], g[NC][8];
  float sg[8], sgx[8];
#pragma unroll
  for (int j = 0; j < 8; ++j) { sg[j] = 0.f; sgx[j] = 0.f; }
  auto load_row = [&](int r, float (&xh_)[8], float (&g_)[8]) {
    const long long i = static_cast<long long>(r) * C8 + (c0 >> 3);
    float xf[8];
    unpack8_bn(x[i], xf);
    unpack8_bn(dy_a[i], g_);
    if (dy_b != nullptr) {
      float t[8];
      unpack8_bn(dy_b[i], t);
#pragma unroll
      for (int j = 0; j < 8; ++j) g_[j] += t[j];
    }
    if (relu) {
      float yf[8];
      unpack8_bn(y[i], yf);
#pragma unroll
      for (int j = 0; j < 8; ++j)
        if (!(yf[j] > 0.f)) g_[j] = 0.f;
    }
#pragma unroll
    for (int j = 0; j < 8; ++j) xh_[j] = (xf[j] - m[j]) * rs[j];
  };
  if constexpr (ITER > 0) {
#pragma unroll
    for (int it = 0; it < ITER; ++it) {
      const int r = r_begin + it * BNC_LANES + lane_r;
      if (r < r_end) {
        load_row(r, xh[it], g[it]);
#pragma unroll
// ... 416 lines not shown
    cudaGetLastError();
  }
  if (S > 8 && !np16) return -2;
  cudaLaunchConfig_t cfg = {};
  cfg.gridDim = grid;
  cfg.blockDim = dim3(256);
  cfg.dynamicSmemBytes = 0;
  cfg.stream = stream;
  cudaLaunchAttribute attr[2];
  int na = 0;
  if (pdl_enabled()) {
    attr[na].id = cudaLaunchAttributeProgrammaticStreamSerialization;
    attr[na].val.programmaticStreamSerializationAllowed = 1;
    ++na;
  }
  if (S > 1) {
    attr[na].id = cudaLaunchAttributeClusterDimension;
    attr[na].val.clusterDim.x = 1;
    attr[na].val.clusterDim.y = static_cast<unsigned>(S);
    attr[na].val.clusterDim.z = 1;
    ++na;
  }
  cfg.attrs = attr;
  cfg.numAttrs = na;
  cudaError_t e = cudaLaunchKernelEx(&cfg, bn_bwd_cluster_kernel<ITER>, x, y, dy_a, dy_b, dx, dres, gamma, mean, rstd, dgamma,
                                     dbeta, rows, C, relu, rpc);
  if (e != cudaSuccess) return static_cast<int>(e);
  return static_cast<int>(cudaGetLastError());
}

extern "C" int b200_bn_bwd_cluster(const void* x, const void* y, const void* dy_a, const void* dy_b, void* dx, void* dres,
                                   const float* gamma, const float* save_mean, const float* save_rstd, float* dgamma,
                                   float* dbeta, long long rows, int C, int relu, int max_cluster, cudaStream_t stream) {
  const bool allow_uncached = max_cluster < 0;
  if (max_cluster < 0) max_cluster = -max_cluster;
  if (rows <= 0) return 0;
  const uintptr_t al = reinterpret_cast<uintptr_t>(x) | reinterpret_cast<uintptr_t>(relu ? y : x) |
                       reinterpret_cast<uintptr_t>(dy_a) | reinterpret_cast<uintptr_t>(dy_b) |
                       reinterpret_cast<uintptr_t>(dx) | reinterpret_cast<uintptr_t>(dres);
  if (C % BNC_CW != 0 || (al & 15) || rows > (1ll << 30)) return -2;
  if (max_cluster <= 0 || max_cluster > 16) max_cluster = 16;
  const int slices = C / BNC_CW;
  int S = 1;
  while (S < max_cluster && (rows + S - 1) / S > BNC_LANES) S <<= 1;
  while (S > 1 && static_cast<long long>(slices) * S > 2 * device_sm_count()) S >>= 1;
  const int rpc = static_cast<int>((rows + S - 1) / S);
  const int iters = (rpc + BNC_LANES - 1) / BNC_LANES;
  const dim3 grid(static_cast<unsigned>(slices), static_cast<unsigned>(S));
#define BNC_GO(I)                                                                                                        \
  return launch_bn_bwd_cluster<I>(grid, S, stream, reinterpret_cast<const uint4*>(x), reinterpret_cast<const uint4*>(y), \
                                  reinterpret_cast<const uint4*>(dy_a), reinterpret_cast<const uint4*>(dy_b),            \
                                  reinterpret_cast<uint4*>(dx), reinterpret_cast<uint4*>(dres), gamma, save_mean,        \
                                  save_rstd, dgamma, dbeta, static_cast<int>(rows), C, relu, rpc)
  if (iters <= 1) BNC_GO(1);
  if (iters <= 2) BNC_GO(2);
  if (iters <= 4) BNC_GO(4);
  if (iters <= 8) BNC_GO(8);
  if (!allow_uncached) return -2;
  BNC_GO(0);
#undef BNC_GO
}

extern "C" int b200_layernorm_fwd(const void* x, const void* residual, void* y, const float* gamma, const float* beta,
                                  float* mean, float* rstd, long long rows, int C, float eps, cudaStream_t stream) {
  if (rows <= 0) return 0;
  if (C > 32 * LN_MAX_PER_LANE) return -2;
  const __nv_bfloat16* xp = reinterpret_cast<const __nv_bfloat16*>(x);
  const __nv_bfloat16* rp = reinterpret_cast<const __nv_bfloat16*>(residual);
  __nv_bfloat16* yp = reinterpret_cast<__nv_bfloat16*>(y);
  if (row_vec_ok(C, x, residual, y) && ((reinterpret_cast<uintptr_t>(gamma) | reinterpret_cast<uintptr_t>(beta)) & 15) == 0) {
    const int rpb = rows_per_block(C);
    const unsigned grid = static_cast<unsigned>((rows + rpb - 1) / rpb);
#define LN_FWD(LPR, VPL) launch_pdl(layernorm_fwd_vec_kernel<LPR, VPL>, grid, 256, 0, stream, xp, rp, yp, gamma, beta, mean, rstd, rows, C, eps)
    ROW_DISPATCH(C, LN_FWD);
#undef LN_FWD
    RET_LAST();
  }
  const int warps = 8;
  launch_pdl(layernorm_fwd_kernel, static_cast<unsigned>((rows + warps - 1) / warps), warps * 32, 0, stream, xp, rp, yp,
             gamma, beta, mean, rstd, rows, C, eps);
  RET_LAST();
}
extern "C" int b200_layernorm_bwd(const void* x, const void* dy, void* dx, const float* gamma, const float* mean,
                                  const float* rstd, float* dgamma, float* dbeta, long long rows, int C,
                                  cudaStream_t stream) {
  if (rows <= 0) return 0;
  if (C > 32 * LN_MAX_PER_LANE) return -2;
  const __nv_bfloat16* xp = reinterpret_cast<const __nv_bfloat16*>(x);
  const __nv_bfloat16* gp = reinterpret_cast<const __nv_bfloat16*>(dy);
  __nv_bfloat16* dp = reinterpret_cast<__nv_bfloat16*>(dx);
  if (row_vec_ok(C, x, dy, dx) && (reinterpret_cast<uintptr_t>(gamma) & 15) == 0) {
    const int rpb = rows_per_block(C);
    long long gv = (rows + rpb - 1) / rpb;
    if (gv > device_sm_count() * 2) gv = device_sm_count() * 2;
#define LN_BWD(LPR, VPL) launch_pdl(layernorm_bwd_vec_kernel<LPR, VPL>, static_cast<unsigned>(gv), 256, 2 * C * sizeof(float), stream, xp, gp, dp, gamma, mean, rstd, dgamma, dbeta, rows, C)
    ROW_DISPATCH(C, LN_BWD);
#undef LN_BWD
    RET_LAST();
  }
  long long g = (rows + 7) / 8;
  if (g > device_sm_count() * 2) g = device_sm_count() * 2;
  launch_pdl(layernorm_bwd_kernel, static_cast<unsigned>(g), 256, 2 * C * sizeof(float), stream, xp, gp, dp, gamma, mean,
             rstd, dgamma, dbeta, rows, C);
  RET_LAST();
}
extern "C" int b200_softmax_fwd(const void* x, void* y, long long rows, int C, float scale, cudaStream_t stream) {
  if (rows <= 0) return 0;
  if (C > 32 * LN_MAX_PER_LANE) return -2;
  const __nv_bfloat16* xp = reinterpret_cast<const __nv_bfloat16*>(x);
  __nv_bfloat16* yp = reinterpret_cast<__nv_bfloat16*>(y);
  if (row_vec_ok(C, x, y, nullptr)) {
    const int rpb = rows_per_block(C);
    const unsigned grid = static_cast<unsigned>((rows + rpb - 1) / rpb);
#define SM_FWD(LPR, VPL) launch_pdl(softmax_fwd_vec_kernel<LPR, VPL>, grid, 256, 0, stream, xp, yp, rows, C, scale)
    ROW_DISPATCH(C, SM_FWD);
#undef SM_FWD
    RET_LAST();
  }
  launch_pdl(softmax_fwd_kernel, static_cast<unsigned>((rows + 7) / 8), 256, 0, stream, xp, yp, rows, C, scale);
  RET_LAST();
}
extern "C" int b200_softmax_bwd(const void* y, const void* dy, void* dx, long long rows, int C, float scale,
                                cudaStream_t stream) {
  if (rows <= 0) return 0;
  if (C > 32 * LN_MAX_PER_LANE) return -2;
  const __nv_bfloat16* yp = reinterpret_cast<const __nv_bfloat16*>(y);
  const __nv_bfloat16* gp = reinterpret_cast<const __nv_bfloat16*>(dy);
  __nv_bfloat16* dp = reinterpret_cast<__nv_bfloat16*>(dx);
  if (row_vec_ok(C, y, dy, dx)) {
    const int rpb = rows_per_block(C);
    const unsigned grid = static_cast<unsigned>((rows + rpb - 1) / rpb);
#define SM_BWD(LPR, VPL) launch_pdl(softmax_bwd_vec_kernel<LPR, VPL>, grid, 256, 0, stream, yp, gp, dp, rows, C, scale)
    ROW_DISPATCH(C, SM_BWD);
#undef SM_BWD
    RET_LAST();
  }
  launch_pdl(softmax_bwd_kernel, static_cast<unsigned>((rows + 7) / 8), 256, 0, stream, yp, gp, dp, rows, C, scale);
  RET_LAST();
}


extern "C" int b200_bn_relu_maxpool(const void* z, void* p, void* argmax, const float* sums, const float* gamma,
                                    const float* beta, float* running_mean, float* running_var, float* save_mean,
                                    float* save_rstd, long long* nbt, int N, int H, int W, int C, int k, int stride, int pad,
                                    int Ho, int Wo, float eps, float momentum, cudaStream_t stream) {
  if (C % 8 || k * k > 255) return -2;
  const long long total = static_cast<long long>(N) * Ho * Wo * (C / 8);
  if (total <= 0) return 0;
  launch_pdl(bn_relu_maxpool_kernel, stream_grid(total), 256, 2 * C * sizeof(float), stream,
             reinterpret_cast<const uint4*>(z), reinterpret_cast<uint4*>(p), reinterpret_cast<uint2*>(argmax), sums, gamma,
             beta, running_mean, running_var, save_mean, save_rstd, nbt, N, H, W, C, k, stride, pad, Ho, Wo, eps, momentum);
  RET_LAST();
}
extern "C" int b200_bn_maxpool_bwd(const void* z, const void* p, const void* argmax, const void* dy_a, const void* dy_b,
                                   void* dz, const float* gamma, const float* save_mean, const float* save_rstd, float* sums,
                                   float* dgamma, float* dbeta, int N, int H, int W, int C, int k, int stride, int pad, int Ho,
                                   int Wo, cudaStream_t stream) {
  if (k * k > 255 || !colred_vec_ok(C, z, p, dy_a) || (dy_b != nullptr && (reinterpret_cast<uintptr_t>(dy_b) & 15)))
    return -2;
  const long long prow = static_cast<long long>(N) * Ho * Wo;
  if (prow <= 0) return 0;
  int rpc = 2 * (256 / (C >> 3));
  if (rpc < colred_rows_per_cta(prow, C, 2)) rpc = colred_rows_per_cta(prow, C, 2);
  launch_pdl(bn_maxpool_bwd_reduce_kernel, static_cast<unsigned>((prow + rpc - 1) / rpc), 256, 256 * 16 * sizeof(float),
             stream, reinterpret_cast<const __nv_bfloat16*>(z), reinterpret_cast<const uint4*>(p),
             reinterpret_cast<const uint2*>(argmax), reinterpret_cast<const uint4*>(dy_a),
             reinterpret_cast<const uint4*>(dy_b), save_mean, save_rstd, sums, N, H, W, C, k, stride, pad, Ho, Wo, rpc);
  cudaError_t e = cudaGetLastError();
  if (e != cudaSuccess) return static_cast<int>(e);
  const long long total = static_cast<long long>(N) * H * W * (C / 8);
  launch_pdl(bn_maxpool_bwd_apply_kernel, stream_grid(total), 256, 5 * C * sizeof(float), stream,
             reinterpret_cast<const uint4*>(z), reinterpret_cast<const uint4*>(p), reinterpret_cast<const uint2*>(argmax),
             reinterpret_cast<const uint4*>(dy_a), reinterpret_cast<const uint4*>(dy_b), reinterpret_cast<uint4*>(dz), gamma,
             save_mean, save_rstd, sums, dgamma, dbeta, N, H, W, C, k, stride, pad, Ho, Wo);
  RET_LAST();
}

B200_TRACE_REGISTER(norm)
```

### baton_b200/csrc/ptx.cuh

```cuda
#pragma once
#include <cuda.h>
#include <cuda_bf16.h>
#include <cuda_runtime.h>
#include <stdint.h>

namespace b200 {

__device__ __forceinline__ uint32_t smem_u32(const void* p) {
  return static_cast<uint32_t>(__cvta_generic_to_shared(p));
}
__device__ __forceinline__ uint32_t lane_id() {
  uint32_t l;
  asm volatile("mov.u32 %0, %%laneid;" : "=r"(l));
  return l;
}
__device__ __forceinline__ bool elect_one() {
  uint32_t pred;
  asm volatile(
      "{\n\t.reg .pred p;\n\t"
      "elect.sync _|p, 0xffffffff;\n\t"
      "selp.u32 %0, 1, 0, p;\n\t}"
      : "=r"(pred));
  return pred != 0;
}
// ... 142 lines not shown
        "+f"(d[24]), "+f"(d[25]), "+f"(d[26]), "+f"(d[27]), "+f"(d[28]), "+f"(d[29]), "+f"(d[30]), "+f"(d[31])
      : "r"(a[0]), "r"(a[1]), "r"(a[2]), "r"(a[3]), "l"(db), "r"(scale_d), "n"(TB));
}
__device__ __forceinline__ void ldmatrix_x4(uint32_t (&r)[4], uint32_t smem_addr) {
  asm volatile("ldmatrix.sync.aligned.m8n8.x4.shared.b16 {%0, %1, %2, %3}, [%4];"
               : "=r"(r[0]), "=r"(r[1]), "=r"(r[2]), "=r"(r[3])
               : "r"(smem_addr)
               : "memory");
}
__device__ __forceinline__ void wgmma_e4m3_n64(float (&d)[32], uint64_t da, uint64_t db, uint32_t scale_d) {
  asm volatile(
      "{\n\t.reg .pred p;\n\tsetp.ne.b32 p, %34, 0;\n\t"
      "wgmma.mma_async.sync.aligned.m64n64k32.f32.e4m3.e4m3 "
      "{"
      "%0, %1, %2, %3, %4, %5, %6, %7, %8, %9, %10, %11, %12, %13, %14, %15, "
      "%16, %17, %18, %19, %20, %21, %22, %23, %24, %25, %26, %27, %28, %29, %30, %31"
      "}, %32, %33, p, 1, 1;\n\t}"
      : "+f"(d[0]), "+f"(d[1]), "+f"(d[2]), "+f"(d[3]), "+f"(d[4]), "+f"(d[5]), "+f"(d[6]), "+f"(d[7]),
        "+f"(d[8]), "+f"(d[9]), "+f"(d[10]), "+f"(d[11]), "+f"(d[12]), "+f"(d[13]), "+f"(d[14]), "+f"(d[15]),
        "+f"(d[16]), "+f"(d[17]), "+f"(d[18]), "+f"(d[19]), "+f"(d[20]), "+f"(d[21]), "+f"(d[22]), "+f"(d[23]),
        "+f"(d[24]), "+f"(d[25]), "+f"(d[26]), "+f"(d[27]), "+f"(d[28]), "+f"(d[29]), "+f"(d[30]), "+f"(d[31])
      : "l"(da), "l"(db), "r"(scale_d));
}
__device__ __forceinline__ void wgmma_e4m3_n128(float (&d)[64], uint64_t da, uint64_t db, uint32_t scale_d) {
  asm volatile(
      "{\n\t.reg .pred p;\n\tsetp.ne.b32 p, %66, 0;\n\t"
      "wgmma.mma_async.sync.aligned.m64n128k32.f32.e4m3.e4m3 "
      "{"
      "%0, %1, %2, %3, %4, %5, %6, %7, %8, %9, %10, %11, %12, %13, %14, %15, "
      "%16, %17, %18, %19, %20, %21, %22, %23, %24, %25, %26, %27, %28, %29, %30, %31, "
      "%32, %33, %34, %35, %36, %37, %38, %39, %40, %41, %42, %43, %44, %45, %46, %47, "
      "%48, %49, %50, %51, %52, %53, %54, %55, %56, %57, %58, %59, %60, %61, %62, %63"
      "}, %64, %65, p, 1, 1;\n\t}"
      : "+f"(d[0]), "+f"(d[1]), "+f"(d[2]), "+f"(d[3]), "+f"(d[4]), "+f"(d[5]), "+f"(d[6]), "+f"(d[7]),
        "+f"(d[8]), "+f"(d[9]), "+f"(d[10]), "+f"(d[11]), "+f"(d[12]), "+f"(d[13]), "+f"(d[14]), "+f"(d[15]),
        "+f"(d[16]), "+f"(d[17]), "+f"(d[18]), "+f"(d[19]), "+f"(d[20]), "+f"(d[21]), "+f"(d[22]), "+f"(d[23]),
        "+f"(d[24]), "+f"(d[25]), "+f"(d[26]), "+f"(d[27]), "+f"(d[28]), "+f"(d[29]), "+f"(d[30]), "+f"(d[31]),
        "+f"(d[32]), "+f"(d[33]), "+f"(d[34]), "+f"(d[35]), "+f"(d[36]), "+f"(d[37]), "+f"(d[38]), "+f"(d[39]),
        "+f"(d[40]), "+f"(d[41]), "+f"(d[42]), "+f"(d[43]), "+f"(d[44]), "+f"(d[45]), "+f"(d[46]), "+f"(d[47]),
        "+f"(d[48]), "+f"(d[49]), "+f"(d[50]), "+f"(d[51]), "+f"(d[52]), "+f"(d[53]), "+f"(d[54]), "+f"(d[55]),
        "+f"(d[56]), "+f"(d[57]), "+f"(d[58]), "+f"(d[59]), "+f"(d[60]), "+f"(d[61]), "+f"(d[62]), "+f"(d[63])
      : "l"(da), "l"(db), "r"(scale_d));
}
template <int N>
__device__ __forceinline__ void wgmma_bf16(float (&d)[N / 2], uint64_t da, uint64_t db, uint32_t scale_d, int a_mn,
                                           int b_mn) {
  if constexpr (N == 64) {
    if (a_mn) {
      if (b_mn) wgmma_bf16_n64<1, 1>(d, da, db, scale_d); else wgmma_bf16_n64<1, 0>(d, da, db, scale_d);
    } else {
      if (b_mn) wgmma_bf16_n64<0, 1>(d, da, db, scale_d); else wgmma_bf16_n64<0, 0>(d, da, db, scale_d);
    }
  } else {
    static_assert(N == 128, "wgmma_bf16: N must be 64 or 128");
    if (a_mn) {
      if (b_mn) wgmma_bf16_n128<1, 1>(d, da, db, scale_d); else wgmma_bf16_n128<1, 0>(d, da, db, scale_d);
    } else {
      if (b_mn) wgmma_bf16_n128<0, 1>(d, da, db, scale_d); else wgmma_bf16_n128<0, 0>(d, da, db, scale_d);
    }
  }
}

template <int N>
__device__ __forceinline__ void wg_store_acc(const float (&d)[N / 2], float* tile, int pitch, int row0) {
  const int lane = static_cast<int>(threadIdx.x & 31), w = static_cast<int>((threadIdx.x >> 5) & 3);
  float* r0 = tile + (row0 + 16 * w + (lane >> 2)) * pitch + 2 * (lane & 3);
  float* r1 = r0 + 8 * pitch;
#pragma unroll
  for (int i = 0; i < N / 8; ++i) {
    *reinterpret_cast<float2*>(r0 + 8 * i) = make_float2(d[4 * i], d[4 * i + 1]);
    *reinterpret_cast<float2*>(r1 + 8 * i) = make_float2(d[4 * i + 2], d[4 * i + 3]);
  }
}
__device__ __forceinline__ void acc_ld_row32(const float* tile_row, uint32_t (&r)[32]) {
#pragma unroll
  for (int j = 0; j < 32; j += 4) {
    const float4 v = *reinterpret_cast<const float4*>(tile_row + j);
    r[j] = __float_as_uint(v.x); r[j + 1] = __float_as_uint(v.y); r[j + 2] = __float_as_uint(v.z); r[j + 3] = __float_as_uint(v.w);
  }
}
__device__ __forceinline__ void named_bar_sync(uint32_t id, uint32_t n) {
  asm volatile("bar.sync %0, %1;" ::"r"(id), "r"(n) : "memory");
}

__device__ __forceinline__ uint32_t ld_acquire_sys(const uint32_t* p) {
  uint32_t v;
  asm volatile("ld.acquire.sys.global.u32 %0, [%1];" : "=r"(v) : "l"(p) : "memory");
  return v;
}
__device__ __forceinline__ uint32_t ld_relaxed_sys(const uint32_t* p) {
  uint32_t v;
  asm volatile("ld.relaxed.sys.global.u32 %0, [%1];" : "=r"(v) : "l"(p) : "memory");
  return v;
}
__device__ __forceinline__ void st_release_sys(uint32_t* p, uint32_t v) {
  asm volatile("st.release.sys.global.u32 [%0], %1;" ::"l"(p), "r"(v) : "memory");
}
__device__ __forceinline__ void red_add_release_sys(uint32_t* p, uint32_t v) {
  asm volatile("red.release.sys.global.add.u32 [%0], %1;" ::"l"(p), "r"(v) : "memory");
}
__device__ __forceinline__ void fence_sys() { asm volatile("fence.acq_rel.sys;" ::: "memory"); }

__device__ __forceinline__ uint4 ld_nc_v4(const void* p) {
  uint4 r;
  asm volatile("ld.global.nc.L1::no_allocate.v4.u32 {%0, %1, %2, %3}, [%4];"
               : "=r"(r.x), "=r"(r.y), "=r"(r.z), "=r"(r.w)
               : "l"(p));
  return r;
}
__device__ __forceinline__ uint4 ld_volatile_v4(const void* p) {
  uint4 r;
  asm volatile("ld.volatile.global.v4.u32 {%0, %1, %2, %3}, [%4];"
               : "=r"(r.x), "=r"(r.y), "=r"(r.z), "=r"(r.w)
               : "l"(p)
               : "memory");
  return r;
}
__device__ __forceinline__ void st_na_v4(void* p, const uint4& v) {
  asm volatile("st.global.L1::no_allocate.v4.u32 [%0], {%1, %2, %3, %4};" ::"l"(p), "r"(v.x), "r"(v.y),
               "r"(v.z), "r"(v.w)
               : "memory");
}

__device__ __forceinline__ uint4 multimem_ld_reduce_bf16x8(const void* mc_ptr) {
  uint4 r;
  asm volatile("multimem.ld_reduce.relaxed.sys.global.add.acc::f32.v4.bf16x2 {%0, %1, %2, %3}, [%4];"
               : "=r"(r.x), "=r"(r.y), "=r"(r.z), "=r"(r.w)
               : "l"(mc_ptr)
               : "memory");
  return r;
}
__device__ __forceinline__ float4 multimem_ld_reduce_f32x4(const void* mc_ptr) {
  float4 r;
  asm volatile("multimem.ld_reduce.relaxed.sys.global.add.v4.f32 {%0, %1, %2, %3}, [%4];"
               : "=f"(r.x), "=f"(r.y), "=f"(r.z), "=f"(r.w)
               : "l"(mc_ptr)
               : "memory");
  return r;
}
__device__ __forceinline__ void multimem_st_v4(void* mc_ptr, const uint4& v) {
  asm volatile("multimem.st.relaxed.sys.global.v4.f32 [%0], {%1, %2, %3, %4};" ::"l"(mc_ptr), "r"(v.x),
               "r"(v.y), "r"(v.z), "r"(v.w)
               : "memory");
}

__device__ __forceinline__ uint32_t pack_bf16x2(float lo, float hi) {
  __nv_bfloat162 v = __floats2bfloat162_rn(lo, hi);
  return *reinterpret_cast<uint32_t*>(&v);
}
__device__ __forceinline__ float2 unpack_bf16x2(uint32_t u) {
  __nv_bfloat162 v = *reinterpret_cast<__nv_bfloat162*>(&u);
  return __bfloat1622float2(v);
}

}
```

### baton_b200/models/resnet.py

```python
from __future__ import annotations

from typing import List, Optional, Sequence, Type

import torch
from torch import nn

from ..ops import nn as bnn
from .base import FederatedModule


def _conv_bn_fwd(conv: "bnn.Conv2d", bn: "bnn.BatchNorm2d", x, residual=None, after_conv=None):
    cc, cb = bnn.Ctx(), bnn.Ctx()
    stats = conv._fusable_stats(x)
    z = bnn._ConvFn.forward(cc, x, conv.weight, conv._w_bf16(), conv.kernel_size, conv.kernel_size, conv.stride,
                            conv.padding, None, stats, conv.flags_cfg)
    if after_conv is not None:
        after_conv()
    y = bnn._BNFn.forward(cb, z, residual, bn.weight, bn.bias, bn.running_mean, bn.running_var, bn.num_batches_tracked,
                          bn.eps, bn.momentum, bn.relu, True, bn.workspace, None, stats is not None)
    return y, (cc, cb)


def _conv_bn_bwd(ctxs, dy_a, dy_b=None, needs_dx=True):
    cc, cb = ctxs
    cc.needs_dx = needs_dx
    out = bnn._BNFn.backward(cb, dy_a, dy_b)
    dz, dres = out[0], out[1]
    dx = bnn._ConvFn.backward(cc, dz)[0]
    return dx, dres




def _stem_fwd(conv, bn, pool, x, after_conv=None):
    stats = conv._fusable_stats(x)
    if (stats is None or bn.workspace is None or not bn.relu or not bn.training or bn.num_features % 8
            or bnn._grad_target(bn.weight) is None or bnn._grad_target(bn.bias) is None):
        return None
    cc = bnn.Ctx()
    z = bnn._ConvFn.forward(cc, x, conv.weight, conv._w_bf16(), conv.kernel_size, conv.kernel_size, conv.stride,
                            conv.padding, None, stats, conv.flags_cfg)
    if after_conv is not None:
        after_conv()
    c = bn.num_features
    out = bnn.F.bn_relu_maxpool(z, bn.workspace[: 2 * c], bnn._unwrap(bn.weight), bnn._unwrap(bn.bias), bn.running_mean,
                                bn.running_var, bn.num_batches_tracked, bn.eps, bn.momentum, pool.k, pool.stride, pool.pad)
    if out is None:
        raise RuntimeError("bn_relu_maxpool rejected a shape _stem_fwd accepted")
    p, arg, mean, rstd = out
    return p, cc, z, arg, mean, rstd


def _stem_bwd(saved, bn, pool, dy_a, dy_b=None):
    p, cc, z, arg, mean, rstd = saved
    c = bn.num_features
    gamma = bnn._unwrap(bn.weight)
    tg, tb = bnn._grad_target(gamma), bnn._grad_target(bnn._unwrap(bn.bias))
    dz = bnn.F.bn_maxpool_bwd(z, p, arg, dy_a.contiguous(), dy_b.contiguous() if dy_b is not None else None, gamma, mean,
                              rstd, bn.workspace[2 * c:], tg, tb, pool.k, pool.stride, pool.pad)
    if dz is None:
        raise RuntimeError("bn_maxpool_bwd rejected a shape bn_relu_maxpool accepted")
    cc.needs_dx = False
    bnn._ConvFn.backward(cc, dz)


def _conv_bn_eval(conv, bn, x, table, residual=None):
    F = bnn.F
    n, h, w, c = x.shape
    k, s, p = conv.kernel_size, conv.stride, conv.padding
    cout = conv.out_channels
    ho, wo = F.conv_out_size(h, k, s, p), F.conv_out_size(w, k, s, p)
    wt = conv.eval_weight
    af = F.affine_epilogue_args(table, bn.eval_off, cout, bn.relu, residual)
    centre = h == 1 and w == 1 and k % 2 == 1 and p == k // 2 and c % 8 == 0 and k > 1
    if centre:
        y = F.gemm(x.view(n, c), wt.view(cout, k * k, c)[:, (k // 2) * k + k // 2, :], affine=af)
    elif k == 1 and s == 1 and p == 0 and c % 8 == 0:
        y = F.gemm(x.view(n * h * w, c), wt, affine=af)
    elif c % 64 == 0:
        y = F.conv_igemm_fwd(x, wt, k, k, s, p, affine=af)
    else:
        y = F.gemm(F.im2col(x, k, k, s, p)[0], wt, affine=af)
    if y is None:
        z = bnn._ConvFn.forward(bnn.Ctx(), x, conv.weight, wt, k, k, s, p, None)
        y = bnn._BNFn.forward(bnn.Ctx(), z, residual, bn.weight, bn.bias, bn.running_mean, bn.running_var, None, bn.eps,
                              bn.momentum, bn.relu, False, None, None)
    return y.view(n, ho, wo, cout)


class BasicBlock(nn.Module):
    expansion = 1

    def __init__(self, inplanes: int, planes: int, stride: int = 1, downsample: Optional[nn.Module] = None):
        super().__init__()
        self.conv1 = bnn.Conv2d(inplanes, planes, 3, stride, 1)
        self.bn1 = bnn.BatchNorm2d(planes, relu=True)
        self.conv2 = bnn.Conv2d(planes, planes, 3, 1, 1)
        self.bn2 = bnn.BatchNorm2d(planes, relu=True)
        self.downsample = downsample

    def forward(self, x):
        identity = x if self.downsample is None else self.downsample(x)
        out = self.bn1(self.conv1(x))
        return self.bn2(self.conv2(out), identity)

    units = (("conv1", "bn1"), ("conv2", "bn2"))


class Bottleneck(nn.Module):
    expansion = 4

    def __init__(self, inplanes: int, planes: int, stride: int = 1, downsample: Optional[nn.Module] = None):
        super().__init__()
        self.conv1 = bnn.Conv2d(inplanes, planes, 1, 1, 0)
        self.bn1 = bnn.BatchNorm2d(planes, relu=True)
        self.conv2 = bnn.Conv2d(planes, planes, 3, stride, 1)
        self.bn2 = bnn.BatchNorm2d(planes, relu=True)
        self.conv3 = bnn.Conv2d(planes, planes * 4, 1, 1, 0)
        self.bn3 = bnn.BatchNorm2d(planes * 4, relu=True)
        self.downsample = downsample

    def forward(self, x):
        identity = x if self.downsample is None else self.downsample(x)
        out = self.bn1(self.conv1(x))
        out = self.bn2(self.conv2(out))
        return self.bn3(self.conv3(out), identity)

    units = (("conv1", "bn1"), ("conv2", "bn2"), ("conv3", "bn3"))


class _Downsample(nn.Sequential):

    def __init__(self, inplanes: int, outplanes: int, stride: int):
        super().__init__(bnn.Conv2d(inplanes, outplanes, 1, stride, 0), bnn.BatchNorm2d(outplanes, relu=False))


class ResNet(FederatedModule):
    loss_kind = "ce"
    default_lr = 0.05
    default_batch_size = 128

    def __init__(self, block: Type[nn.Module], layers: Sequence[int], num_classes: int = 1000,
                 in_channels: int = 3, name: Optional[str] = None):
        super().__init__()
        if name:
            self.name = name
        self.inplanes = 64
        self.conv1 = bnn.Conv2d(in_channels, 64, 7, 2, 3)
        self.bn1 = bnn.BatchNorm2d(64, relu=True)
        self.maxpool = bnn.MaxPool2d(3, 2, 1)
        self.layer1 = self._make_layer(block, 64, layers[0], 1)
        self.layer2 = self._make_layer(block, 128, layers[1], 2)
        self.layer3 = self._make_layer(block, 256, layers[2], 2)
        self.layer4 = self._make_layer(block, 512, layers[3], 2)
        self.avgpool = bnn.GlobalAvgPool()
        self.fc = bnn.Linear(512 * block.expansion, num_classes, out_fp32=True)
        self.stats_workspace = None
        self.zeroes_own_workspace = True
        for m in self.modules():
            if isinstance(m, BasicBlock):
                nn.init.zeros_(m.bn2.weight)
            elif isinstance(m, Bottleneck):
                nn.init.zeros_(m.bn3.weight)

    def _make_layer(self, block, planes: int, blocks: int, stride: int) -> nn.Sequential:
        downsample = None
        if stride != 1 or self.inplanes != planes * block.expansion:
            downsample = _Downsample(self.inplanes, planes * block.expansion, stride)
        layers: List[nn.Module] = [block(self.inplanes, planes, stride, downsample)]
        self.inplanes = planes * block.expansion
        for _ in range(1, blocks):
            layers.append(block(self.inplanes, planes))
        return nn.Sequential(*layers)

    def set_precision(self, dtype: str = "bf16") -> "ResNet":
        assert dtype in ("bf16", "fp8")
        for m in self.modules():
            if isinstance(m, bnn.Conv2d):
                m.fp8 = dtype == "fp8"
        self.compute_dtype = dtype
        return self

    def forward(self, x):
        if self.stats_workspace is not None and self.training:
            self.stats_workspace.zero_()
        x = self.maxpool(self.bn1(self.conv1(x)))
        x = self.layer4(self.layer3(self.layer2(self.layer1(x))))
        return self.fc(self.avgpool(x))

    def _block_fwd(self, blk, x, tape):
        ds_ctx = None
        identity = x
        if blk.downsample is not None:
            with bnn.BRANCH.fork(x):
                identity, ds_ctx = _conv_bn_fwd(blk.downsample[0], blk.downsample[1], x)
        out = x
        ctxs = []
        n = len(blk.units)
        for i, (cn, bnn_) in enumerate(blk.units):
            last = i == n - 1
            if last:
                bnn.BRANCH.join()
            out, c = _conv_bn_fwd(getattr(blk, cn), getattr(blk, bnn_), out, identity if last else None)
            ctxs.append(c)
        tape.append((ctxs, ds_ctx))
        return out

    def _block_bwd(self, entry, pieces):
        ctxs, ds_ctx = entry
        d, dres = _conv_bn_bwd(ctxs[-1], pieces[0], pieces[1] if len(pieces) > 1 else None)
        dx_ds = None
        if ds_ctx is not None:
            with bnn.BRANCH.fork(dres):
                dx_ds, _ = _conv_bn_bwd(ds_ctx, dres)
        for c in reversed(ctxs[:-1]):
            d, _ = _conv_bn_bwd(c, d)
        if ds_ctx is not None:
            bnn.BRANCH.join()
            return [d, dx_ds]
        return [d, dres]

    def explicit_step(self, x, target, loss_acc=None, after_first_gemm=None):
        F = bnn.F
        if self.stats_workspace is not None:
            self.stats_workspace.zero_()
        stem = cp = None
        fused_stem = _stem_fwd(self.conv1, self.bn1, self.maxpool, x, after_first_gemm)
        if fused_stem is not None:
            h = fused_stem[0]
        else:
            h, stem = _conv_bn_fwd(self.conv1, self.bn1, x, after_conv=after_first_gemm)
            cp = bnn.Ctx()
            h = bnn._MaxPoolFn.forward(cp, h, self.maxpool.k, self.maxpool.stride, self.maxpool.pad)
        tape = []
        for layer in (self.layer1, self.layer2, self.layer3, self.layer4):
            for blk in layer:
                h = self._block_fwd(blk, h, tape)
        ca = None
        if h.shape[1] == 1 and h.shape[2] == 1:
            feat = h.reshape(h.shape[0], h.shape[3])
        else:
            ca = bnn.Ctx()
            feat = bnn._AvgPoolFn.forward(ca, h)
        fc = self.fc
        head = None
        tw, tb = bnn._grad_target(fc.weight), bnn._grad_target(fc.bias)
        if fc.out_features <= 32 and tw is not None and (fc.bias is None or tb is not None) and fc.act == 0:
            head = F.linear_xent_head(feat.contiguous(), bnn._shadow(fc, "weight", fc.weight), fc.bias, target, tw, tb,
                                      acc=loss_acc)
        if head is not None:
            stats, d, _ = head
        else:
            cl = bnn.Ctx()
            logits = bnn._LinearFn.forward(cl, feat, fc.weight, fc.bias, bnn._shadow(fc, "weight", fc.weight), fc.act,
                                           fc.out_fp32, None, None)
            cl.needs_dx = True
            stats, dlogits = F.softmax_xent(logits.contiguous(), target, want_grad=True, acc=loss_acc)
            d = bnn._LinearFn.backward(cl, dlogits)[0]
        d = d.reshape(h.shape) if ca is None else bnn._AvgPoolFn.backward(ca, d)
        pieces = [d]
        for bi in range(len(tape) - 1, -1, -1):
            pieces = self._block_bwd(tape[bi], pieces)
        if fused_stem is not None:
            _stem_bwd(fused_stem, self.bn1, self.maxpool, pieces[0], pieces[1] if len(pieces) > 1 else None)
        else:
            d = bnn._MaxPoolFn.backward(cp, pieces[0], pieces[1] if len(pieces) > 1 else None)[0]
            _conv_bn_bwd(stem, d, needs_dx=False)
        bnn.WGRAD.join()
        return stats

    def _block_eval(self, blk, x, table):
        identity = x
        if blk.downsample is not None:
            with bnn.BRANCH.fork(x):
                identity = _conv_bn_eval(blk.downsample[0], blk.downsample[1], x, table)
        out = x
        n = len(blk.units)
        for i, (cn, bn_name) in enumerate(blk.units):
            last = i == n - 1
            if last:
                bnn.BRANCH.join()
            out = _conv_bn_eval(getattr(blk, cn), getattr(blk, bn_name), out, table, identity if last else None)
        return out

    def prepare_eval(self):
        for m in self.modules():
            if isinstance(m, bnn.Conv2d):
                m.eval_weight = m._w_bf16(gated=False)

    def explicit_eval(self, x, target, acc, want_logits: bool = False):
        F = bnn.F
        table = self.eval_bn_table
        h = _conv_bn_eval(self.conv1, self.bn1, x, table)
        h = F.maxpool(h, self.maxpool.k, self.maxpool.stride, self.maxpool.pad)[0]
        for layer in (self.layer1, self.layer2, self.layer3, self.layer4):
            for blk in layer:
                h = self._block_eval(blk, h, table)
        feat = h.reshape(h.shape[0], h.shape[3]) if h.shape[1] == 1 and h.shape[2] == 1 else F.avgpool(h)
        fc = self.fc
        w = bnn._shadow(fc, "weight", fc.weight)
        if fc.act == 0:
            head = F.linear_xent_eval(feat.contiguous(), w, fc.bias, target, acc, want_logits=want_logits)
            if head is not None:
                return head[1]
        logits = F.gemm(feat.contiguous(), w, bias=fc.bias, act=fc.act, out_dtype=torch.float32)
        F.softmax_xent(logits, target, want_grad=False, acc=acc, loss_scale=1.0)
        return logits if want_logits else None

    def build_workspace(self, device) -> torch.Tensor:
        bns = [m for m in self.modules() if isinstance(m, bnn.BatchNorm2d)]
        total = sum(4 * m.num_features for m in bns)
        ws = torch.zeros(total, dtype=torch.float32, device=device)
        off = 0
        for m in bns:
            m.workspace = ws[off: off + 4 * m.num_features]
            off += 4 * m.num_features
        self.stats_workspace = ws
        for parent in self.modules():
            for conv_name, bn_name in (("conv1", "bn1"), ("conv2", "bn2"), ("conv3", "bn3")):
                conv, bn = getattr(parent, conv_name, None), getattr(parent, bn_name, None)
                if isinstance(conv, bnn.Conv2d) and isinstance(bn, bnn.BatchNorm2d):
                    conv.bn_ws = bn.workspace
            if isinstance(parent, _Downsample):
                parent[0].bn_ws = parent[1].workspace
        return ws


def resnet18(num_classes: int = 10, **kw) -> ResNet:
    kw.setdefault("name", "resnet18")
    return ResNet(BasicBlock, [2, 2, 2, 2], num_classes=num_classes, **kw)


def resnet50(num_classes: int = 1000, **kw) -> ResNet:
    kw.setdefault("name", "resnet50")
    return ResNet(Bottleneck, [3, 4, 6, 3], num_classes=num_classes, **kw)
```

### baton_b200/ops/functional.py

```python
from __future__ import annotations

from typing import List, Optional, Sequence, Tuple

import torch

from ._ext import load

BF16 = torch.bfloat16
NUM_SMS = 132


def _pitch(t: torch.Tensor) -> int:
    assert t.dim() == 2 and (t.stride(1) == 1 or t.shape[1] == 1), "GEMM operand must have unit inner stride"
    return t.stride(0) if t.shape[0] > 1 else max(t.stride(0), t.shape[1])


def _tma_ok(t: torch.Tensor) -> bool:
    return t.dtype == BF16 and _pitch(t) % 8 == 0 and t.data_ptr() % 16 == 0


def pick_bn(M: int, N: int) -> int:
    m_tiles = (M + 127) // 128
    if N >= 128 and m_tiles * ((N + 127) // 128) >= NUM_SMS:
        return 128
# ... 148 lines not shown
            free.append((pos, s))
        pos = e
    if pos < n:
        free.append((pos, n))
    ng = sorted((o, o + l) for o, l in nograd)
    out = []
    for s, e in free:
        cuts = sorted({s, e} | {b for r in ng for b in r if s < b < e})
        for a, b in zip(cuts, cuts[1:]):
            kind = 1 if any(lo <= a and b <= hi for lo, hi in ng) else 0
            out.extend((c, min(chunk, b - c), kind) for c in range(a, b, chunk))
    return out


def fused_sgd_segments(w: torch.Tensor, g: torch.Tensor, hyper: torch.Tensor, segments: torch.Tensor,
                       momentum_buf: Optional[torch.Tensor] = None, w_bf16: Optional[torch.Tensor] = None,
                       nesterov: bool = False, prox_anchor: Optional[torch.Tensor] = None,
                       corr: Optional[torch.Tensor] = None, adam_v: Optional[torch.Tensor] = None) -> None:
    load().fused_sgd_segments(w, g, momentum_buf, w_bf16, segments, hyper, nesterov, prox_anchor, corr, adam_v)


def scaffold_corr(corr: torch.Tensor, c: torch.Tensor, c_i: torch.Tensor) -> None:
    load().scaffold_corr(corr, c, c_i)


def scaffold_dc(up: torch.Tensor, c_i: torch.Tensor, c: torch.Tensor, global_w: torch.Tensor, theta: torch.Tensor,
                inv_k_eta: float, *, first: bool) -> None:
    load().scaffold_dc(up, c_i, c, global_w, theta, float(inv_k_eta), bool(first))


def weighted_sum_(dst: torch.Tensor, srcs: Sequence[torch.Tensor], weights: Sequence[float]) -> torch.Tensor:
    C = load()
    flat_dst = dst.view(-1) if dst.is_contiguous() else None
    if flat_dst is None or dst.dtype not in (torch.float32, BF16) or len(srcs) > C.MAX_RANKS:
        acc = torch.zeros_like(dst, dtype=torch.float32)
        for s, w in zip(srcs, weights):
            acc.add_(s.to(device=dst.device, dtype=torch.float32), alpha=float(w))
        dst.copy_(acc.to(dst.dtype))
        return dst
    ss = [s.to(device=dst.device, dtype=dst.dtype).contiguous().view(-1) for s in srcs]
    C.weighted_sum(flat_dst, ss, [float(w) for w in weights])
    return dst


def fold_client(acc: torch.Tensor, theta: torch.Tensor, global_w: torch.Tensor, nk: float, *, first: bool = False,
                reset: bool = False, w_bf16: Optional[torch.Tensor] = None, momentum: Optional[torch.Tensor] = None) -> None:
    load().fold_client(acc, theta, global_w, w_bf16, momentum, float(nk), 1 if first else 0, reset)


def fold_finish(acc: torch.Tensor, theta: torch.Tensor, global_w: torch.Tensor, total: float) -> None:
    load().fold_client(acc, theta, global_w, None, None, 1.0 / float(total), 2, False)


def dp_clip_factor(theta: torch.Tensor, global_w: torch.Tensor, clip: float, work: torch.Tensor, s_out: torch.Tensor,
                   norm_out: torch.Tensor, *, s_copy_ptr: int = 0, nonfinite: Optional[torch.Tensor] = None) -> None:
    load().dp_clip_factor(theta, global_w, float(clip), work, s_out, norm_out, int(s_copy_ptr), nonfinite)


def fold_client_scaled(acc: torch.Tensor, theta: torch.Tensor, global_w: torch.Tensor, s: torch.Tensor, *,
                       first: bool = False, reset: bool = False, w_bf16: Optional[torch.Tensor] = None,
                       momentum: Optional[torch.Tensor] = None) -> None:
    load().fold_client_scaled(acc, theta, global_w, w_bf16, momentum, s, first, reset)


def cast(src: torch.Tensor, dtype: torch.dtype, out: Optional[torch.Tensor] = None) -> torch.Tensor:
    if out is None:
        out = torch.empty(src.shape, dtype=dtype, device=src.device)
    load().cast(src.contiguous(), out)
    return out


def gather_rows(src: torch.Tensor, idx: torch.Tensor, out: Optional[torch.Tensor] = None) -> torch.Tensor:
    if out is None:
        out = torch.empty((idx.numel(),) + tuple(src.shape[1:]), dtype=src.dtype, device=src.device)
    load().gather_rows(src, idx, out)
    return out


def colsum_(x2d: torch.Tensor, out: torch.Tensor, accumulate: bool = True) -> torch.Tensor:
    load().colsum(x2d, out, x2d.shape[0], x2d.shape[1], accumulate)
    return out


def add(a: torch.Tensor, b: torch.Tensor, relu: bool = False) -> torch.Tensor:
    out = torch.empty_like(a)
    load().add_bf16(a, b, out, relu)
    return out


def relu_bwd(y: torch.Tensor, dy: torch.Tensor) -> torch.Tensor:
    dx = torch.empty_like(dy)
    load().relu_bwd(y, dy, dx)
    return dx


def gelu(x: torch.Tensor) -> torch.Tensor:
    y = torch.empty_like(x)
    load().gelu(x, y)
    return y


def gelu_bwd(x: torch.Tensor, dy: torch.Tensor) -> torch.Tensor:
    dx = torch.empty_like(x)
    load().gelu_bwd(x, dy, dx)
    return dx


def pad_rows(src2d: torch.Tensor, kp: int, out: Optional[torch.Tensor] = None, gate: Optional[dict] = None) -> torch.Tensor:
    rows, k = src2d.shape
    if out is None:
        out = torch.empty((rows, kp), dtype=BF16, device=src2d.device)
    g = gate or {}
    load().pad_rows(src2d, out, rows, k, kp, g.get("flags"), g.get("epoch_word"), int(g.get("elem_off", 0)),
                    int(g.get("tile_elems", 0)))
    return out


def conv_out_size(h: int, k: int, stride: int, pad: int) -> int:
    return (h + 2 * pad - k) // stride + 1


def round_up(x: int, m: int) -> int:
    return (x + m - 1) // m * m


def im2col(x: torch.Tensor, kh: int, kw: int, stride: int, pad: int) -> Tuple[torch.Tensor, int, int, int]:
    n, h, w, c = x.shape
    ho, wo = conv_out_size(h, kh, stride, pad), conv_out_size(w, kw, stride, pad)
    kp = round_up(kh * kw * c, 8)
    col = torch.empty((n * ho * wo, kp), dtype=BF16, device=x.device)
    load().im2col(x, col, n, h, w, c, kh, kw, stride, pad, ho, wo, kp)
    return col, ho, wo, kp


HALO_BM = 64
_HALO_MAX_SMEM = 227 * 1024


def halo_smem_bytes(h: int, w: int) -> int:
    halo = round_up((HALO_BM // (h * w)) * (h + 2) * (w + 2) * 128, 1024)
    return halo + 9 * 8192 + 16 * 8 + 4 * 64 * 4 + 1024


def halo_eligible(kh: int, kw: int, stride: int, pad: int, c: int, h: int, w: int, affine: Optional[dict] = None) -> bool:
    return (kh == 3 and kw == 3 and stride == 1 and pad == 1 and c == 64 and h * w <= HALO_BM and
            HALO_BM % (h * w) == 0 and affine is None and halo_smem_bytes(h, w) <= _HALO_MAX_SMEM)


def halo_cluster(m_rows: int) -> int:
    tiles = (m_rows + HALO_BM - 1) // HALO_BM
    return 4 if tiles % 4 == 0 else 2 if tiles % 2 == 0 else 1


def _conv_path(path: Optional[str], eligible: bool) -> str:
    if path is None:
        return "halo" if eligible else "im2col"
    if path not in ("halo", "im2col"):
        raise ValueError("path must be None, 'halo' or 'im2col', not {!r}".format(path))
    if path == "halo" and not eligible:
        raise ValueError("the halo kernel does not take this convolution (see halo_eligible)")
    return path


def conv_igemm_fwd(x: torch.Tensor, w2d: torch.Tensor, kh: int, kw: int, stride: int, pad: int,
                   col_stats: Optional[torch.Tensor] = None, affine: Optional[dict] = None,
                   cluster_k: Optional[int] = None, force_bn: int = 0,
                   out: Optional[torch.Tensor] = None, path: Optional[str] = None,
                   mc: Optional[int] = None) -> Optional[torch.Tensor]:
    n, h, w, c = x.shape
    cout = w2d.shape[0]
    if c % 64 or w2d.shape[1] != kh * kw * c or not x.is_contiguous() or not w2d.is_contiguous():
        return None
    ho, wo = conv_out_size(h, kh, stride, pad), conv_out_size(w, kw, stride, pad)
    M, K = n * ho * wo, kh * kw * c
    if _conv_path(path, halo_eligible(kh, kw, stride, pad, c, h, w, affine) and cout % 8 == 0) == "halo":
        y = out if out is not None else torch.empty((M, cout), dtype=BF16, device=x.device)
        if not load().conv_halo(x, w2d, y, False, mc or halo_cluster(M), col_stats):
            raise RuntimeError("conv_halo declined a convolution halo_eligible admits")
        return y
    bn = force_bn or pick_bn(M, cout)
    if cluster_k is None:
        cluster_k = pick_cluster_k(M, cout, K, bn)
    y = out if out is not None else torch.empty((M, cout), dtype=BF16, device=x.device)
    af = affine or {}
    ok = load().conv_igemm_fwd(x, w2d, y, kh, kw, stride, pad, ho, wo, cluster_k, bn, col_stats, af.get("scale"),
                               af.get("shift"), af.get("residual"), bool(af.get("relu", False)))
    return y if ok else None


S2_MAX_TAPS = 4


def conv_s2_dgrad_taps(kh: int, kw: int, pad: int, ho: int, wo: int) -> Optional[List[List[Tuple[int, int, int]]]]:
    classes = []
    for a in (0, 1):
        for b in (0, 1):
            taps = []
            for r in range(kh):
                if (a + pad - r) % 2:
                    continue
                dp = (a + pad - r) // 2
                for s in range(kw):
                    if (b + pad - s) % 2:
                        continue
                    dq = (b + pad - s) // 2
                    if dp < 0 or dq < 0:
                        return None
                    if dp < ho and dq < wo:
                        taps.append((r * kw + s, dp, dq))
            if len(taps) > S2_MAX_TAPS:
                return None
            classes.append(taps)
    return classes


def conv_igemm_dgrad(dy: torch.Tensor, w2d: torch.Tensor, in_shape, kh: int, kw: int, pad: int, stride: int = 1,
                     out: Optional[torch.Tensor] = None, path: Optional[str] = None,
                     mc: Optional[int] = None) -> Optional[torch.Tensor]:
    n, h, w, c = in_shape
    cout = dy.shape[-1]
    if c % 64 or cout % 64 or w2d.shape[1] != kh * kw * c or not dy.is_contiguous() or not w2d.is_contiguous():
        return None
    if _conv_path(path, halo_eligible(kh, kw, stride, pad, cout, h, w)) == "halo":
        dx = out if out is not None else torch.empty((n, h, w, c), dtype=BF16, device=dy.device)
        if not load().conv_halo(dy, w2d, dx, True, mc or halo_cluster(n * h * w), None):
            raise RuntimeError("conv_halo declined a convolution halo_eligible admits")
        return dx
    if stride == 1:
        M, K = n * h * w, kh * kw * cout
        bn = pick_bn(M, c)
        dx = out if out is not None else torch.empty((n, h, w, c), dtype=BF16, device=dy.device)
        ok = load().conv_igemm_dgrad(dy, w2d, dx, kh, kw, pad, pick_cluster_k(M, c, K, bn), bn)
        return dx if ok else None
    if stride != 2:
        return None
    ho, wo = dy.shape[1], dy.shape[2]
    classes = conv_s2_dgrad_taps(kh, kw, pad, ho, wo)
    if classes is None:
        return None
    bn = pick_bn(4 * n * ho * wo, c)
    words = [[t | dp << 16 | dq << 24 for t, dp, dq in taps] + [0] * (S2_MAX_TAPS - len(taps)) for taps in classes]
    dx = out if out is not None else torch.empty((n, h, w, c), dtype=BF16, device=dy.device)
    ok = load().conv_igemm_dgrad_s2(dy, w2d, dx, kh, kw, [len(t) for t in classes], [x for ws in words for x in ws], bn)
    return dx if ok else None


def conv_igemm_wgrad_(dy2d: torch.Tensor, x: torch.Tensor, dw2d: torch.Tensor, kh: int, kw: int, stride: int,
                      pad: int, sgd: Optional[dict] = None) -> bool:
    n, h, w, c = x.shape
    cout = dy2d.shape[1]
    if c % 64 or not x.is_contiguous() or not dy2d.is_contiguous() or not dw2d.is_contiguous():
        return False
    ho, wo = conv_out_size(h, kh, stride, pad), conv_out_size(w, kw, stride, pad)
    M, K = n * ho * wo, kh * kw * c
    bn = pick_bn(cout, K)
    split_k = pick_split_k(cout, K, M, bn)
    if sgd is not None and split_k != 1:
        return False
    sg = sgd or {}
    return bool(load().conv_igemm_wgrad(dy2d, x, dw2d, cout, kh, kw, stride, pad, ho, wo, split_k, bn,
                                        sg.get("theta"), sg.get("theta_bf16"), sg.get("momentum"), sg.get("hyper"),
                                        bool(sg.get("nesterov", False)), sg.get("anchor"), sg.get("corr"),
                                        sg.get("adam_v")))


def col2im(col: torch.Tensor, shape: Tuple[int, int, int, int], kh: int, kw: int, stride: int, pad: int,
           ho: int, wo: int) -> torch.Tensor:
    n, h, w, c = shape
    dx = torch.empty(shape, dtype=BF16, device=col.device)
    load().col2im(col, dx, n, h, w, c, kh, kw, stride, pad, ho, wo, col.shape[1])
    return dx


def maxpool(x: torch.Tensor, k: int, stride: int, pad: int) -> Tuple[torch.Tensor, torch.Tensor]:
    n, h, w, c = x.shape
    ho, wo = conv_out_size(h, k, stride, pad), conv_out_size(w, k, stride, pad)
    y = torch.empty((n, ho, wo, c), dtype=BF16, device=x.device)
    arg = torch.empty((n, ho, wo, c), dtype=torch.uint8 if (c % 8 == 0 and k * k <= 255) else torch.int32, device=x.device)
    load().maxpool(x, y, arg, n, h, w, c, k, stride, pad, ho, wo)
    return y, arg


def maxpool_bwd(dy: torch.Tensor, arg: torch.Tensor, in_shape, k: int, stride: int, pad: int,
                dy_b: Optional[torch.Tensor] = None) -> torch.Tensor:
    n, h, w, c = in_shape
    if dy_b is not None and arg.dtype != torch.uint8:
        dy, dy_b = add(dy, dy_b), None
    dx = torch.empty(in_shape, dtype=BF16, device=dy.device)
    load().maxpool_bwd(dy, dy_b, arg, dx, n, h, w, c, dy.shape[1], dy.shape[2], k, stride, pad)
    return dx


def bn_relu_maxpool(z: torch.Tensor, sums: torch.Tensor, gamma, beta, rmean, rvar, nbt, eps: float, momentum: float,
                    k: int, stride: int, pad: int):
    n, h, w, c = z.shape
    if c % 8 or k * k > 255:
        return None
    ho, wo = conv_out_size(h, k, stride, pad), conv_out_size(w, k, stride, pad)
    p = torch.empty((n, ho, wo, c), dtype=BF16, device=z.device)
    arg = torch.empty((n, ho, wo, c), dtype=torch.uint8, device=z.device)
    mean = torch.empty(c, dtype=torch.float32, device=z.device)
    rstd = torch.empty(c, dtype=torch.float32, device=z.device)
    if not load().bn_relu_maxpool(z, p, arg, sums, gamma, beta, rmean, rvar, mean, rstd, nbt, n, h, w, c, k, stride, pad,
                                  ho, wo, eps, momentum):
        return None
    return p, arg, mean, rstd
# ... 119 lines not shown
```

### baton_b200/ops/nn.py

```python
from __future__ import annotations

import contextlib
import math
from typing import Optional

import torch
from torch import nn
from torch.nn import functional as TF

from . import functional as F
from ._ext import load

BF16 = torch.bfloat16


class _P:
    __slots__ = ("p",)

    def __init__(self, p):
        self.p = p


def _unwrap(v):
    return v.p if isinstance(v, _P) else v
# ... 221 lines not shown
        if ctx.needs_dx:
            dx = F.gemm(dy2, w_bf16, b_mn=True).view(ctx.x_shape)
        return dx, gw, gb, None, None, None, None, None


class Linear(nn.Module):

    def __init__(self, in_features: int, out_features: int, bias: bool = True, act: Optional[str] = None,
                 out_fp32: bool = False):
        super().__init__()
        self.in_features, self.out_features = in_features, out_features
        self.act = {None: 0, "relu": 1, "gelu": 2}[act]
        self.out_fp32 = out_fp32
        self.weight = nn.Parameter(torch.empty(out_features, in_features))
        self.bias = nn.Parameter(torch.empty(out_features)) if bias else None
        self.flags_cfg = None
        self.reset_parameters()

    def reset_parameters(self):
        nn.init.kaiming_uniform_(self.weight, a=math.sqrt(5))
        if self.bias is not None:
            bound = 1 / math.sqrt(self.in_features)
            nn.init.uniform_(self.bias, -bound, bound)

    def forward(self, x):
        if not x.is_cuda:
            y = TF.linear(x, self.weight.to(x.dtype), None if self.bias is None else self.bias.to(x.dtype))
            return TF.relu(y) if self.act == 1 else (TF.gelu(y, approximate="tanh") if self.act == 2 else y)
        if x.dtype != BF16:
            x = F.cast(x.contiguous(), BF16)
        if getattr(self, "fp8", False) and self.act == 0 and self.bias is None and not self.out_fp32:
            y = matmul_fp8(x.reshape(-1, x.shape[-1]), self, _shadow(self, "weight", self.weight), self.in_features)
            return y.view(*x.shape[:-1], self.out_features)
        cfg = self.flags_cfg
        if cfg is not None and cfg.get("epoch_word") is None:
            self.flags_cfg = None
        return _LinearFn.apply(x, _wrap(self.weight, x), _wrap(self.bias, x), _shadow(self, "weight", self.weight),
                               self.act, self.out_fp32, cfg, _anchor(x, self.weight))


class _ConvFn(torch.autograd.Function):
    @staticmethod
    def forward(ctx, x, weight, w_bf16, kh, kw, stride, pad, anchor, stats=None, gate=None):
        weight = _unwrap(weight)
        n, h, w, c = x.shape
        cout = w_bf16.shape[0]
        ctx.center = (h == 1 and w == 1 and kh == kw and kh % 2 == 1 and pad == kh // 2 and c % 8 == 0 and kh > 1)
        if ctx.center:
            col, ho, wo, kp = x.view(n, c), 1, 1, c
            wc = w_bf16.view(cout, kh * kw, c)[:, (kh // 2) * kw + kw // 2, :]
            y = F.gemm(col, wc, col_stats=stats)
        else:
            y = None
            ctx.igemm = False
            if kh == 1 and kw == 1 and stride == 1 and pad == 0 and c % 8 == 0:
                col, ho, wo, kp = x.view(n * h * w, c), h, w, c
            elif c % 64 == 0:
                ho, wo, kp = F.conv_out_size(h, kh, stride, pad), F.conv_out_size(w, kw, stride, pad), kh * kw * c
                y = F.conv_igemm_fwd(x, w_bf16, kh, kw, stride, pad, col_stats=stats)
                col, ctx.igemm = x, y is not None
            if y is None:
                if not (kh == 1 and kw == 1 and stride == 1 and pad == 0 and c % 8 == 0):
                    col, ho, wo, kp = F.im2col(x, kh, kw, stride, pad)
                gk = {}
                if gate is not None:
                    gk = dict(flags=gate["flags"], flag_epoch_word=gate["epoch_word"], flag_elem_off=gate["elem_off"],
                              flag_tile_elems=gate["tile_elems"], force_bn=F.pick_bn(col.shape[0], w_bf16.shape[0]))
                y = F.gemm(col, w_bf16, col_stats=stats, **gk)
        ctx.save_for_backward(col, w_bf16)
        ctx.weight = weight
        ctx.geom = (n, h, w, c, kh, kw, stride, pad, ho, wo, kp)
        ctx.needs_dx = x.requires_grad
        return y.view(n, ho, wo, cout)

    @staticmethod
    def backward(ctx, dy):
        col, w_bf16 = ctx.saved_tensors
        n, h, w, c, kh, kw, stride, pad, ho, wo, kp = ctx.geom
        cout = w_bf16.shape[0]
        dy2 = dy.reshape(n * ho * wo, cout)
        if not dy2.is_contiguous():
            dy2 = dy2.contiguous()
        weight = ctx.weight
        k_true = kh * kw * c
        gw = None
        tgt = _grad_target(weight)
        if ctx.center:
            tap = (kh // 2) * kw + kw // 2
            if tgt is None:
                gw = torch.zeros((cout, kh, kw, c), dtype=torch.float32, device=dy.device)
                g2d = gw.view(cout, kh * kw, c)[:, tap, :]
                gw = gw.permute(0, 3, 1, 2)
            else:
                full = tgt.permute(0, 2, 3, 1).reshape(cout, kh * kw, c)
                assert full.data_ptr() == tgt.data_ptr(), "conv weight grad must be channels_last in the arena"
                g2d = full[:, tap, :]
            if tgt is None:
                F.gemm(dy2, col, a_mn=True, b_mn=True, out=g2d, accumulate=True)
            tok = WGRAD.mark(dy2)
            dx = None
            if ctx.needs_dx:
                wc = w_bf16.view(cout, kh * kw, c)[:, tap, :]
                dx = F.gemm(dy2, wc, b_mn=True).view(n, 1, 1, c)
            if tgt is not None:
                WGRAD.run(lambda: _wgrad(lambda sgd: F.gemm(dy2, col, a_mn=True, b_mn=True, out=g2d, accumulate=True,
                                                            sgd=sgd) is not None, g2d, nograd_of=tgt),
                          dy2, col, after=None if SGD_EPI.active else tok)
            return dx, gw, None, None, None, None, None, None, None, None
        igemm = getattr(ctx, "igemm", False)
        tok = WGRAD.mark(dy2)
        dx = None
        if ctx.needs_dx:
            if kp == k_true and w_bf16.shape[1] == k_true and (stride == 2 or (stride == 1 and kh == kw and kh > 1)):
                dx = F.conv_igemm_dgrad(dy2.view(n, ho, wo, cout), w_bf16, (n, h, w, c), kh, kw, pad, stride=stride)
            if dx is None:
                dcol = F.gemm(dy2, w_bf16, b_mn=True)
                if kh == 1 and kw == 1 and stride == 1 and pad == 0 and c % 8 == 0:
                    dx = dcol.view(n, h, w, c)
                else:
                    dx = F.col2im(dcol, (n, h, w, c), kh, kw, stride, pad, ho, wo)
        if tgt is not None:
            out2d = tgt.permute(0, 2, 3, 1).reshape(cout, k_true) if tgt.dim() == 4 else tgt.view(cout, k_true)
            assert out2d.data_ptr() == tgt.data_ptr(), "conv weight grad must be channels_last in the arena"
            if igemm:
                WGRAD.run(lambda: _wgrad(lambda sgd: F.conv_igemm_wgrad_(dy2, col, out2d, kh, kw, stride, pad, sgd=sgd),
                                         out2d),
                          dy2, col, after=None if SGD_EPI.active else tok)
            else:
                WGRAD.run(lambda: F.gemm(dy2, col, a_mn=True, b_mn=True, out=out2d, accumulate=True, n_valid=k_true),
                          dy2, col, after=tok)
        elif igemm:
            g2 = torch.zeros((cout, k_true), dtype=torch.float32, device=dy.device)
            F.conv_igemm_wgrad_(dy2, col, g2, kh, kw, stride, pad)
            gw = g2.view(cout, kh, kw, c).permute(0, 3, 1, 2)
        else:
            g2 = F.gemm(dy2, col, a_mn=True, b_mn=True, out_dtype=torch.float32, accumulate=True, n_valid=k_true)
            gw = g2.view(cout, kh, kw, c).permute(0, 3, 1, 2)
        return dx, gw, None, None, None, None, None, None, None, None


class Conv2d(nn.Module):

    def __init__(self, in_channels: int, out_channels: int, kernel_size: int, stride: int = 1, padding: int = 0):
        super().__init__()
        self.in_channels, self.out_channels = in_channels, out_channels
        self.kernel_size, self.stride, self.padding = kernel_size, stride, padding
        w = torch.empty(out_channels, in_channels, kernel_size, kernel_size)
        nn.init.kaiming_normal_(w, mode="fan_out", nonlinearity="relu")
        self.weight = nn.Parameter(w.contiguous(memory_format=torch.channels_last))
        self.k_true = kernel_size * kernel_size * in_channels
        self.kp = F.round_up(self.k_true, 8)
        self.flags_cfg = None

    def _w_bf16(self, gated: bool = True):
        sh = getattr(self, "weight_bf16", None)
        if sh is None:
            sh = _shadow(self, "weight", self.weight)
        sh = sh.view(self.out_channels, self.k_true)
        if self.kp != self.k_true:
            sh = F.pad_rows(sh, self.kp, gate=self.flags_cfg if gated else None)
        return sh

    def forward(self, x):
        if not x.is_cuda:
            y = TF.conv2d(x.permute(0, 3, 1, 2), self.weight.to(x.dtype), None, self.stride, self.padding)
            return y.permute(0, 2, 3, 1)
        if getattr(self, "fp8", False):
            return conv2d_fp8(x, self)
        stats = self._fusable_stats(x)
        y = _ConvFn.apply(x, _wrap(self.weight, x), self._w_bf16(), self.kernel_size, self.kernel_size,
                          self.stride, self.padding, _anchor(x, self.weight), stats, self.flags_cfg)
        if stats is not None:
            y._bn_stats_ws = stats
        return y

    def _fusable_stats(self, x):
        ws = getattr(self, "bn_ws", None)
        if ws is None or not self.training or not torch.is_grad_enabled():
            return None
        n, h, w, c = x.shape
        k, s_, p_ = self.kernel_size, self.stride, self.padding
        ho, wo = (h + 2 * p_ - k) // s_ + 1, (w + 2 * p_ - k) // s_ + 1
        centre = h == 1 and w == 1 and k % 2 == 1 and p_ == k // 2 and c % 8 == 0 and k > 1
        kdim = c if (centre or (k == 1 and c % 8 == 0)) else F.round_up(k * k * c, 8)
        cout = self.weight.shape[0]
        return ws[: 2 * cout] if F.gemm_stats_fusable(n * ho * wo, cout, kdim) else None


class _BNFn(torch.autograd.Function):
    @staticmethod
    def forward(ctx, x, residual, gamma, beta, rmean, rvar, nbt, eps, momentum, relu, training, ws, anchor,
                stats_ready=False):
        gamma, beta = _unwrap(gamma), _unwrap(beta)
        C_ = load()
        c = x.shape[-1]
        rows = x.numel() // c
        y = torch.empty_like(x)
        if ws is None:
            ws = torch.zeros(4 * c, dtype=torch.float32, device=x.device)
        sums_f, sums_b = ws[: 2 * c], ws[2 * c:]
        save_mean = torch.empty(c, dtype=torch.float32, device=x.device)
        save_rstd = torch.empty(c, dtype=torch.float32, device=x.device)
        if training and not stats_ready:
            C_.bn_stats(x, sums_f, rows, c)
        C_.bn_apply(x, residual, y, sums_f, gamma, beta, rmean, rvar, save_mean, save_rstd, nbt, rows, c, eps,
                    momentum, relu, training)
        ctx.save_for_backward(x, y, save_mean, save_rstd)
        ctx.gamma, ctx.beta, ctx.sums_b = gamma, beta, sums_b
        ctx.relu, ctx.has_res, ctx.rows, ctx.c = relu, residual is not None, rows, c
        return y

    @staticmethod
    def backward(ctx, dy, dy_b=None):
        C_ = load()
        x, y, mean, rstd = ctx.saved_tensors
        if not dy.is_contiguous():
            dy = dy.contiguous()
        gamma, beta = ctx.gamma, ctx.beta
        dx = torch.empty_like(x)
        dres = torch.empty_like(x) if ctx.has_res else None
        tg, tb = _grad_target(gamma), _grad_target(beta)
        gg = gb = None
        if tg is None:
            gg = tg = torch.zeros(ctx.c, dtype=torch.float32, device=x.device)
        if tb is None:
            gb = tb = torch.zeros(ctx.c, dtype=torch.float32, device=x.device)
        if not C_.bn_bwd_cluster(x, y, dy, dy_b, dx, dres, gamma, mean, rstd, tg, tb, ctx.rows, ctx.c, ctx.relu, 16):
            if dy_b is not None:
                dy = F.add(dy, dy_b.contiguous())
            C_.bn_bwd_reduce(x, y, dy, mean, rstd, ctx.sums_b, ctx.rows, ctx.c, ctx.relu)
            C_.bn_bwd_apply(x, y, dy, dx, dres, gamma, mean, rstd, ctx.sums_b, tg, tb, ctx.rows, ctx.c, ctx.relu)
        if ctx.has_res and dres is None:
            dres = dy
        return dx, dres, gg, gb, None, None, None, None, None, None, None, None, None, None


class BatchNorm2d(nn.Module):

    def __init__(self, num_features: int, eps: float = 1e-5, momentum: float = 0.1, relu: bool = False):
        super().__init__()
        self.num_features, self.eps, self.momentum, self.relu = num_features, eps, momentum, relu
        self.weight = nn.Parameter(torch.ones(num_features))
        self.bias = nn.Parameter(torch.zeros(num_features))
        self.register_buffer("running_mean", torch.zeros(num_features))
        self.register_buffer("running_var", torch.ones(num_features))
        self.register_buffer("num_batches_tracked", torch.tensor(0, dtype=torch.long))
        self.workspace = None

    def forward(self, x, residual=None):
        if not x.is_cuda:
            xn = x.permute(0, 3, 1, 2)
            y = TF.batch_norm(xn, self.running_mean, self.running_var, self.weight, self.bias, self.training,
                              self.momentum, self.eps).permute(0, 2, 3, 1)
            if self.training:
                self.num_batches_tracked += 1
            if residual is not None:
                y = y + residual
            return TF.relu(y) if self.relu else y
        ws = self.workspace
        if ws is None:
            ws = torch.zeros(4 * self.num_features, dtype=torch.float32, device=x.device)
        fused = getattr(x, "_bn_stats_ws", None)
        ready = (fused is not None and self.workspace is not None and self.training
                 and fused.data_ptr() == self.workspace.data_ptr())
        return _BNFn.apply(x, residual, _wrap(self.weight, x), _wrap(self.bias, x), self.running_mean,
                           self.running_var, self.num_batches_tracked if self.training else None, self.eps,
                           self.momentum, self.relu, self.training, ws, _anchor(x, self.weight), ready)


class _MaxPoolFn(torch.autograd.Function):
    @staticmethod
    def forward(ctx, x, k, stride, pad):
        y, arg = F.maxpool(x, k, stride, pad)
        ctx.save_for_backward(arg)
        ctx.cfg = (tuple(x.shape), k, stride, pad)
        return y

    @staticmethod
    def backward(ctx, dy, dy_b=None):
        (arg,) = ctx.saved_tensors
        shape, k, stride, pad = ctx.cfg
        return F.maxpool_bwd(dy.contiguous(), arg, shape, k, stride, pad, dy_b=dy_b), None, None, None


class MaxPool2d(nn.Module):
    def __init__(self, kernel_size: int = 3, stride: int = 2, padding: int = 1):
        super().__init__()
        self.k, self.stride, self.pad = kernel_size, stride, padding

    def forward(self, x):
        if not x.is_cuda:
            return TF.max_pool2d(x.permute(0, 3, 1, 2), self.k, self.stride, self.pad).permute(0, 2, 3, 1)
        return _MaxPoolFn.apply(x, self.k, self.stride, self.pad)


class _AvgPoolFn(torch.autograd.Function):
    @staticmethod
    def forward(ctx, x):
        ctx.shape = tuple(x.shape)
        return F.avgpool(x)

    @staticmethod
    def backward(ctx, dy):
        return F.avgpool_bwd(dy.contiguous(), ctx.shape)


class GlobalAvgPool(nn.Module):

    def forward(self, x):
        if x.shape[1] == 1 and x.shape[2] == 1:
            return x.reshape(x.shape[0], x.shape[3])
        if not x.is_cuda:
# ... 295 lines not shown
```

### baton_b200/utils/trace.py

```python
from __future__ import annotations

import collections
import os
import re
from typing import Callable, Dict, List, Tuple

import torch

_TUS = ["?", "gemm_wgmma", "gemm_fp8", "quant", "attention", "im2col_tma", "gemm_simt", "fedavg", "elementwise",
        "conv", "norm", "loss", "conv_halo"]
_CSRC = os.path.join(os.path.dirname(os.path.dirname(os.path.abspath(__file__))), "csrc")
_NAME_CACHE: Dict[int, str] = {}


POINT_BASE = 5_000_000_000


def point_label(tag: int) -> str:
    tu, line = divmod(int(tag) - POINT_BASE, 100000)
    try:
        with open(os.path.join(_CSRC, _TUS[tu] + ".cu")) as f:
            src = f.readlines()
        text = src[line - 1]
        return text.split("//", 1)[1].strip() if "//" in text else "{}:{}".format(_TUS[tu], line)
    except (OSError, IndexError):
        return "point {}:{}".format(tu, line)


def kernel_name(tag: int) -> str:
    tag = abs(int(tag))
    if tag in _NAME_CACHE:
        return _NAME_CACHE[tag]
    tu, line = divmod(tag, 100000)
    name = "{}:{}".format(_TUS[tu] if tu < len(_TUS) else tu, line)
    try:
        with open(os.path.join(_CSRC, _TUS[tu] + ".cu")) as f:
            src = f.readlines()
        for i in range(min(line, len(src)) - 1, -1, -1):
            if "__global__" in src[i]:
                m = re.search(r"(\w+)\s*\(", " ".join(s.strip() for s in src[i:i + 4]).split("__global__", 1)[1]
                              .replace("__launch_bounds__", " ").replace("__cluster_dims__", " "))
                cands = re.findall(r"([A-Za-z_]\w*)\s*\(", " ".join(s.strip() for s in src[i:i + 4]))
                cands = [c for c in cands if c not in ("__launch_bounds__", "__cluster_dims__")]
                if cands:
                    name = cands[0]
                elif m:
                    name = m.group(1)
                break
    except OSError:
        pass
    _NAME_CACHE[tag] = name
    return name


def timeline_rows(records: List[Tuple[int, int]], name: Callable[[int], str] = kernel_name) -> List[dict]:
    resident = collections.defaultdict(collections.deque)
    rows = []
    for t, tag in records:
        if abs(tag) >= POINT_BASE:
            continue
        k = name(tag)
        if tag < 0:
            resident[k].append(t)
        else:
            pre = resident[k].popleft() if resident[k] else t
            rows.append({"t_ns": t, "tag": tag, "name": k, "early_ns": t - pre})
    for a, b in zip(rows, rows[1:]):
        a["slot_ns"] = b["t_ns"] - a["t_ns"]
    if rows:
        rows[-1]["slot_ns"] = 0
    return rows


class KernelTrace:
    def __init__(self, capacity: int = 1 << 16, device=None):
        from ..ops._ext import load
        self.C = load()
        self.device = torch.device(device or "cuda:0")
        self.capacity = capacity
        self.buf = torch.zeros(2 + 2 * capacity, dtype=torch.int64, device=self.device)
        self.buf[1] = capacity
        self.enabled = False

    def start(self) -> bool:
        self.buf[0] = 0
        self.enabled = bool(self.C.trace_set(self.buf))
        return self.enabled

    def stop(self) -> None:
        torch.cuda.synchronize(self.device)
        self.C.trace_set(None)

    def records(self) -> List[Tuple[int, int]]:
        torch.cuda.synchronize(self.device)
        host = self.buf.cpu()
        n = min(int(host[0]), self.capacity)
        rec = host[2: 2 + 2 * n].view(n, 2).tolist()
        rec.sort()
        return [(int(t), int(tag)) for t, tag in rec]

    def timeline(self) -> List[dict]:
        return timeline_rows(self.records())

    def points(self) -> List[Tuple[int, str]]:
        out = []
        for t, tag in self.records():
            if tag >= POINT_BASE:
                out.append((t, "    . " + point_label(tag)))
            elif tag > 0:
                out.append((t, "> " + kernel_name(tag)))
            else:
                out.append((t, "  (resident) " + kernel_name(tag)))
        return out

    def summary(self, skip_first: int = 0) -> List[str]:
        rows = self.timeline()[skip_first:]
        tot = collections.defaultdict(float)
        cnt = collections.Counter()
        early = collections.defaultdict(float)
        for r in rows:
            tot[r["name"]] += r["slot_ns"]
            cnt[r["name"]] += 1
            early[r["name"]] += r["early_ns"]
        total = sum(tot.values()) or 1.0
        out = ["kernels {}  critical-path total {:.1f} us".format(len(rows), total / 1e3)]
        for n, t in sorted(tot.items(), key=lambda kv: -kv[1]):
            out.append("{:9.1f} us {:5.1f}%  n={:5d}  avg slot {:6.2f} us  avg resident-before-deps {:5.2f} us  {}".format(
                t / 1e3, 100 * t / total, cnt[n], t / cnt[n] / 1e3, early[n] / cnt[n] / 1e3, n))
        return out
```

Baseline: 205,300.

## Add dedicated stem conv kernel and fused BN-maxpool backward with weight gradient

Adds a specialised stem convolution kernel that builds im2col tiles in shared memory from a staged input strip and runs a single-stage wgmma GEMM, with the BN column statistics accumulated in the epilogue. It also adds a backward kernel that fuses the BN/maxpool backward with the stem weight-gradient computation, so the dz tensor is never written out and a separate conv wgrad pass is skipped. The ResNet stem uses these paths whenever the shape is eligible. The cost is more specialised code, atomics into fp32 weight grads and a strict layout assumption on the gradient arena.

```diff
diff --git a/baton_b200/build_ext.py b/baton_b200/build_ext.py
--- a/baton_b200/build_ext.py
+++ b/baton_b200/build_ext.py
@@ -16,7 +16,8 @@
     BUILD = os.path.join(HERE, "csrc", "build_trace")
 TARGET = os.path.join(HERE, "_C_trace.so" if TRACE else "_C.so")
 
-CU_SOURCES = ["gemm_wgmma.cu", "gemm_fp8.cu", "quant.cu", "attention.cu", "im2col_tma.cu", "gemm_simt.cu", "fedavg.cu", "elementwise.cu", "conv.cu", "norm.cu", "loss.cu", "conv_halo.cu"]
+CU_SOURCES = ["gemm_wgmma.cu", "gemm_fp8.cu", "quant.cu", "attention.cu", "im2col_tma.cu", "gemm_simt.cu", "fedavg.cu", "elementwise.cu", "conv.cu", "norm.cu", "loss.cu", "conv_halo.cu",
+              "conv_stem.cu"]
 HEADERS = ["ptx.cuh", "launch.h", "pdl.cuh", "mx.cuh", "sgd.cuh", "dp.cuh", "epilogue.cuh"]
 NVCC_FLAGS = ["-gencode", "arch=compute_90a,code=sm_90a", "-lineinfo", "-O3", "-std=c++17",
               "-Xcompiler", "-fPIC", "--use_fast_math", "-Xptxas", "-v"]
diff --git a/baton_b200/csrc/bindings.cpp b/baton_b200/csrc/bindings.cpp
--- a/baton_b200/csrc/bindings.cpp
+++ b/baton_b200/csrc/bindings.cpp
@@ -95,7 +95,7 @@
 
 extern "C" {
 #define B200_TRACE_TUS(X) X(gemm_wgmma) X(gemm_fp8) X(quant) X(attention) X(im2col_tma) X(gemm_simt) X(fedavg) \
-  X(elementwise) X(conv) X(norm) X(loss) X(conv_halo)
+  X(elementwise) X(conv) X(norm) X(loss) X(conv_halo) X(conv_stem)
 #define B200_DECL(tu) int b200_trace_set_##tu(unsigned long long* p);
 B200_TRACE_TUS(B200_DECL)
 #undef B200_DECL
@@ -263,6 +263,54 @@
                                 static_cast<int>(mc), opt_ptr<float>(col_stats), cur_stream());
   if (rc == -2) return false;
   check(rc, "conv_halo");
+  return true;
+}
+bool stem_conv_fwd(const at::Tensor& x, const at::Tensor& w, at::Tensor z, const std::optional<at::Tensor>& col_stats,
+                   int64_t kh, int64_t kw, int64_t stride, int64_t pad) {
+  CHECK_CUDA(x); CHECK_CUDA(w); CHECK_CUDA(z);
+  TORCH_CHECK(x.scalar_type() == at::kBFloat16 && w.scalar_type() == at::kBFloat16 && z.scalar_type() == at::kBFloat16 &&
+              x.dim() == 4 && x.is_contiguous() && z.is_contiguous() && w.dim() == 2 && w.size(0) == 64 && w.stride(1) == 1 &&
+              w.size(1) >= kh * kw * x.size(3), "stem_conv_fwd: bf16 NHWC x, [64, >= K] weights, contiguous z");
+  const int64_t ho = (x.size(1) + 2 * pad - kh) / stride + 1, wo = (x.size(2) + 2 * pad - kw) / stride + 1;
+  TORCH_CHECK(z.numel() == x.size(0) * ho * wo * 64, "stem_conv_fwd: z must hold [N*Ho*Wo, 64] elements");
+  TORCH_CHECK(!col_stats.has_value() || (col_stats->scalar_type() == at::kFloat && col_stats->numel() >= 128),
+              "stem_conv_fwd: col_stats is a [128] fp32 buffer");
+  const c10::cuda::CUDAGuard guard(x.device());
+  const int rc = b200_stem_conv_fwd(cptr(x), cptr(w), static_cast<int>(w.stride(0)), ptr(z), opt_ptr<float>(col_stats),
+                                    static_cast<int>(x.size(0)), static_cast<int>(x.size(1)), static_cast<int>(x.size(2)),
+                                    static_cast<int>(x.size(3)), static_cast<int>(kh), static_cast<int>(kw),
+                                    static_cast<int>(stride), static_cast<int>(pad), cur_stream());
+  if (rc == -2) return false;
+  check(rc, "stem_conv_fwd");
+  return true;
+}
+bool stem_bn_wgrad(const at::Tensor& x, const at::Tensor& z, const at::Tensor& p, const at::Tensor& arg,
+                   const at::Tensor& dy_a, const std::optional<at::Tensor>& dy_b, const std::optional<at::Tensor>& gamma,
+                   const at::Tensor& mean, const at::Tensor& rstd, at::Tensor sums, const std::optional<at::Tensor>& dgamma,
+                   const std::optional<at::Tensor>& dbeta, at::Tensor dw, int64_t kh, int64_t kw, int64_t stride, int64_t pad,
+                   int64_t pk, int64_t pstride, int64_t ppad) {
+  CHECK_CUDA(x); CHECK_CUDA(z); CHECK_CUDA(p); CHECK_CUDA(dw);
+  TORCH_CHECK(x.scalar_type() == at::kBFloat16 && z.scalar_type() == at::kBFloat16 && p.scalar_type() == at::kBFloat16 &&
+              dy_a.scalar_type() == at::kBFloat16 && arg.scalar_type() == at::kByte && x.dim() == 4 && z.dim() == 4 &&
+              p.dim() == 4 && z.size(3) == 64 && p.size(3) == 64 && x.is_contiguous() && z.is_contiguous() &&
+              p.is_contiguous() && arg.is_contiguous() && dy_a.is_contiguous() && dy_a.sizes() == p.sizes() &&
+              arg.sizes() == p.sizes() && (!dy_b.has_value() || (dy_b->is_contiguous() && dy_b->sizes() == p.sizes())),
+              "stem_bn_wgrad: bf16 NHWC x / z / pooled tensors, byte argmax");
+  TORCH_CHECK(dw.scalar_type() == at::kFloat && dw.dim() == 2 && dw.size(0) == 64 && dw.stride(1) == 1 &&
+              dw.size(1) >= kh * kw * x.size(3), "stem_bn_wgrad: dw is fp32 [64, >= K]");
+  TORCH_CHECK(sums.scalar_type() == at::kFloat && sums.numel() >= 128, "stem_bn_wgrad: sums is a [128] fp32 buffer");
+  const c10::cuda::CUDAGuard guard(x.device());
+  const int rc = b200_stem_bn_wgrad(cptr(x), cptr(z), cptr(p), cptr(arg), cptr(dy_a), opt_ptr<const void>(dy_b),
+                                    opt_ptr<const float>(gamma), mean.data_ptr<float>(), rstd.data_ptr<float>(),
+                                    sums.data_ptr<float>(), opt_ptr<float>(dgamma), opt_ptr<float>(dbeta),
+                                    dw.data_ptr<float>(), static_cast<int>(dw.stride(0)), static_cast<int>(x.size(0)),
+                                    static_cast<int>(x.size(1)), static_cast<int>(x.size(2)), static_cast<int>(x.size(3)),
+                                    static_cast<int>(kh), static_cast<int>(kw), static_cast<int>(stride),
+                                    static_cast<int>(pad), static_cast<int>(pk), static_cast<int>(pstride),
+                                    static_cast<int>(ppad), static_cast<int>(p.size(1)), static_cast<int>(p.size(2)),
+                                    cur_stream());
+  if (rc == -2) return false;
+  check(rc, "stem_bn_wgrad");
   return true;
 }
 bool conv_igemm_dgrad_s2(const at::Tensor& dy, const at::Tensor& w, at::Tensor dx, int64_t kh, int64_t kw,
@@ -932,6 +980,8 @@
   m.def("conv_igemm_dgrad", &conv_igemm_dgrad);
   m.def("conv_igemm_dgrad_s2", &conv_igemm_dgrad_s2);
   m.def("conv_halo", &conv_halo);
+  m.def("stem_conv_fwd", &stem_conv_fwd);
+  m.def("stem_bn_wgrad", &stem_bn_wgrad);
   m.def("gemm_batched", &gemm_batched);
   m.def("gemm_fp8", &gemm_fp8);
   m.def("quant_mx_rows", &quant_mx_rows);
diff --git a/baton_b200/csrc/conv_stem.cu b/baton_b200/csrc/conv_stem.cu
--- /dev/null
+++ b/baton_b200/csrc/conv_stem.cu
@@ -0,0 +1,477 @@
+#define B200_TU_TAG 13
+#include "ptx.cuh"
+#include "epilogue.cuh"
+#include "launch.h"
+#include "pdl.cuh"
+
+namespace b200 {
+
+constexpr int STEM_BM = 128;
+constexpr int STEM_N = 64;
+constexpr int STEM_KT = 3;
+constexpr int STEM_THREADS = 256;
+constexpr int STEM_COL_BYTES = STEM_KT * STEM_BM * 128;
+constexpr int STEM_W_BYTES = STEM_KT * STEM_N * 128;
+constexpr int STEM_DZ_BYTES = STEM_BM * 128;
+constexpr int STEM_PART_PITCH = STEM_N + 4;
+constexpr int STEM_WPART_PITCH = STEM_KT * 64 + 4;
+constexpr int STEM_CLUSTER = 8;
+constexpr int STEM_MAX_IN_BYTES = 32 * 1024;
+
+struct StemGeom {
+  int N, H, W, C, KH, KW, stride, pad, Ho, Wo, K;
+};
+
+__device__ __forceinline__ void stem_load_input(const StemGeom& g, const __nv_bfloat16* __restrict__ x, int m0,
+                                                uint16_t* sin) {
+  const int hw = g.Ho * g.Wo;
+  const int n = m0 / hw, r0 = m0 - n * hw;
+  const int ho0 = r0 / g.Wo, ho1 = (r0 + STEM_BM - 1) / g.Wo;
+  const int rows = (ho1 - ho0) * g.stride + g.KH;
+  const int wc = g.W * g.C, wc8 = wc >> 3;
+  const int h0 = ho0 * g.stride - g.pad;
+  for (int i = threadIdx.x; i < rows * wc8; i += STEM_THREADS) {
+    const int r = i / wc8, v = i - r * wc8;
+    const int h = h0 + r;
+    uint4 val = make_uint4(0u, 0u, 0u, 0u);
+    if (h >= 0 && h < g.H) val = __ldg(reinterpret_cast<const uint4*>(x + (static_cast<long long>(n) * g.H + h) * wc) + v);
+    reinterpret_cast<uint4*>(sin)[i] = val;
+  }
+}
+
+constexpr int STEM_TAB_BYTES = STEM_KT * 64 * 8;
+__device__ __forceinline__ void stem_build_tab(const StemGeom& g, int2* tab) {
+  for (int k = threadIdx.x; k < STEM_KT * 64; k += STEM_THREADS) {
+    const int tap = k / g.C, c = k - tap * g.C;
+    const int r = tap / g.KW, s = tap - r * g.KW;
+    tab[k] = k < g.K ? make_int2(r * g.W * g.C + s * g.C + c, s) : make_int2(0, 1 << 20);
+  }
+}
+
+static_assert(STEM_THREADS == 2 * STEM_BM, "two threads per pixel row");
+__device__ __forceinline__ void stem_build_col(const StemGeom& g, int m0, const uint16_t* sin, const int2* tab,
+                                               uint8_t* col) {
+  const int hw = g.Ho * g.Wo;
+  const int r0 = m0 % hw;
+  const int ho0 = r0 / g.Wo;
+  const int m = threadIdx.x >> 1;
+  const int rr = r0 + m;
+  const int ho = rr / g.Wo, wo = rr - ho * g.Wo;
+  const int w0 = wo * g.stride - g.pad;
+  const int base = (ho - ho0) * g.stride * g.W * g.C + w0 * g.C;
+  constexpr int HALF = STEM_KT * 4;
+  const int j0 = (threadIdx.x & 1) * HALF;
+#pragma unroll 2
+  for (int jj = 0; jj < HALF; ++jj) {
+    const int j = j0 + jj;
+    uint32_t e[8];
+#pragma unroll
+    for (int u = 0; u < 8; ++u) {
+      const int2 t = tab[j * 8 + u];
+      e[u] = static_cast<unsigned>(w0 + t.y) < static_cast<unsigned>(g.W) ? sin[base + t.x] : 0u;
+    }
+    uint4 o;
+    o.x = e[0] | (e[1] << 16);
+    o.y = e[2] | (e[3] << 16);
+    o.z = e[4] | (e[5] << 16);
+    o.w = e[6] | (e[7] << 16);
+    const int kt = j >> 3, cc = j & 7;
+    *reinterpret_cast<uint4*>(col + kt * (STEM_BM * 128) + m * 128 + ((cc ^ (m & 7)) << 4)) = o;
+  }
+}
+
+struct StemFwdParams {
+  const __nv_bfloat16* x;
+  const uint16_t* w;
+  int ldw;
+  __nv_bfloat16* z;
+  float* col_stats;
+};
+
+__global__ void __launch_bounds__(STEM_THREADS, 2)
+stem_conv_fwd_kernel(const StemFwdParams p, const StemGeom g) {
+  const __nv_bfloat16* __restrict__ x = p.x;
+  const uint16_t* __restrict__ w = p.w;
+  const int ldw = p.ldw;
+  float* col_stats = p.col_stats;
+  extern __shared__ __align__(1024) uint8_t smem_raw[];
+  uint8_t* smem = reinterpret_cast<uint8_t*>((reinterpret_cast<uintptr_t>(smem_raw) + 1023) & ~uintptr_t(1023));
+  uint8_t* sa = smem;
+  uint8_t* sb = smem + STEM_COL_BYTES;
+  float* cstat = reinterpret_cast<float*>(sb + STEM_W_BYTES);
+  int2* tab = reinterpret_cast<int2*>(cstat + 4 * 2 * STEM_N);
+  uint16_t* sin = reinterpret_cast<uint16_t*>(tab + STEM_KT * 64);
+
+  griddep_launch_dependents();
+  const int m0 = blockIdx.x * STEM_BM;
+  stem_build_tab(g, tab);
+  griddep_wait();
+  stem_load_input(g, x, m0, sin);
+  static_assert(STEM_N * STEM_KT * 8 % STEM_THREADS == 0, "whole weight chunks per thread");
+#pragma unroll
+  for (int it = 0; it < STEM_N * STEM_KT * 8 / STEM_THREADS; ++it) {
+    const int i = threadIdx.x + it * STEM_THREADS;
+    const int n = i / (STEM_KT * 8), j = i - n * (STEM_KT * 8);
+    const int kc0 = j * 8;
+    uint16_t e[8];
+#pragma unroll
+    for (int u = 0; u < 8; ++u) e[u] = kc0 + u < g.K ? w[static_cast<size_t>(n) * ldw + kc0 + u] : static_cast<uint16_t>(0);
+    uint4 o;
+    o.x = e[0] | (static_cast<uint32_t>(e[1]) << 16);
+    o.y = e[2] | (static_cast<uint32_t>(e[3]) << 16);
+    o.z = e[4] | (static_cast<uint32_t>(e[5]) << 16);
+    o.w = e[6] | (static_cast<uint32_t>(e[7]) << 16);
+    const int kt = j >> 3, cc = j & 7;
+    *reinterpret_cast<uint4*>(sb + kt * (STEM_N * 128) + n * 128 + ((cc ^ (n & 7)) << 4)) = o;
+  }
+  __syncthreads();
+  if (threadIdx.x == 0) TRACE_POINT();
+  stem_build_col(g, m0, sin, tab, sa);
+  fence_proxy_async();
+  __syncthreads();
+  if (threadIdx.x == 0) TRACE_POINT();
+
+  const int wg = threadIdx.x >> 7;
+  const int num_kt = (g.K + 63) / 64;
+  float acc[32];
+#pragma unroll
+  for (int j = 0; j < 32; ++j) acc[j] = 0.f;
+  for (int kt = 0; kt < num_kt; ++kt) {
+    const uint32_t a0 = smem_u32(sa + kt * (STEM_BM * 128)) + wg * 8192;
+    const uint32_t b0 = smem_u32(sb + kt * (STEM_N * 128));
+    wgmma_fence();
+#pragma unroll
+    for (int k = 0; k < 4; ++k)
+      wgmma_bf16_n64<0, 0>(acc, gmma_desc_sw128(a0 + k * 32, 16, 1024), gmma_desc_sw128(b0 + k * 32, 16, 1024), 1u);
+    wgmma_commit();
+  }
+  wgmma_wait<0>();
+  wgmma_fence_operands(acc);
+  if (threadIdx.x == 0) TRACE_POINT();
+
+  __syncthreads();
+  float* part = reinterpret_cast<float*>(smem);
+  wg_store_acc<STEM_N>(acc, part, STEM_PART_PITCH, 64 * wg);
+  __syncthreads();
+  const int ew = threadIdx.x >> 5;
+  const int lane = static_cast<int>(lane_id());
+  const int q = ew & 3;
+  const int c = (ew >> 2) * 32;
+  const int lrow = q * 32 + lane;
+  uint32_t r[32];
+  acc_ld_row32(part + lrow * STEM_PART_PITCH + c, r);
+  float v[32];
+#pragma unroll
+  for (int j = 0; j < 32; ++j) v[j] = __uint_as_float(r[j]);
+  if (col_stats != nullptr) stage_col_stats(cstat + q * 2 * STEM_N, STEM_N, c, v);
+  __nv_bfloat16* d = p.z + static_cast<size_t>(m0 + lrow) * STEM_N + c;
+#pragma unroll
+  for (int j = 0; j < 32; j += 8) {
+    uint4 o;
+    o.x = pack_bf16x2(v[j], v[j + 1]);
+    o.y = pack_bf16x2(v[j + 2], v[j + 3]);
+    o.z = pack_bf16x2(v[j + 4], v[j + 5]);
+    o.w = pack_bf16x2(v[j + 6], v[j + 7]);
+    *reinterpret_cast<uint4*>(d + j) = o;
+  }
+  if (col_stats != nullptr) {
+    __syncthreads();
+    for (int i = threadIdx.x; i < 2 * STEM_N; i += STEM_THREADS)
+      atomicAdd(col_stats + i, cstat[i] + cstat[2 * STEM_N + i] + cstat[4 * STEM_N + i] + cstat[6 * STEM_N + i]);
+  }
+}
+
+struct StemBwdParams {
+  const __nv_bfloat16* x;
+  const uint4* z;
+  const uint4* p;
+  const uint2* arg;
+  const uint4* dy_a;
+  const uint4* dy_b;
+  const float* gamma;
+  const float* mean;
+  const float* rstd;
+  const float* sums;
+  float* dgamma;
+  float* dbeta;
+  float* dw;
+  int ldd;
+  int M;
+  int pk, pstride, ppad, Hp, Wp;
+};
+
+__global__ void __launch_bounds__(STEM_THREADS, 2)
+stem_bn_wgrad_kernel(const StemBwdParams a, const StemGeom g) {
+  extern __shared__ __align__(1024) uint8_t smem_raw[];
+  uint8_t* smem = reinterpret_cast<uint8_t*>((reinterpret_cast<uintptr_t>(smem_raw) + 1023) & ~uintptr_t(1023));
+  uint8_t* scol = smem;
+  uint8_t* sdz = smem + STEM_COL_BYTES;
+  float* kc = reinterpret_cast<float*>(sdz + STEM_DZ_BYTES);
+  int2* tab = reinterpret_cast<int2*>(kc + 5 * STEM_N);
+  uint16_t* sin = reinterpret_cast<uint16_t*>(tab + STEM_KT * 64);
+
+  griddep_launch_dependents();
+  const int m0 = blockIdx.x * STEM_BM;
+  const bool live = m0 < a.M;
+  stem_build_tab(g, tab);
+  griddep_wait();
+  if (live) stem_load_input(g, a.x, m0, sin);
+  const float inv_rows = 1.f / static_cast<float>(static_cast<long long>(g.N) * g.Ho * g.Wo);
+  for (int c = threadIdx.x; c < STEM_N; c += STEM_THREADS) {
+    const float gm = a.gamma != nullptr ? a.gamma[c] : 1.f;
+    const float r = a.rstd[c];
+    kc[c] = gm * r;
+    kc[STEM_N + c] = a.sums[c] * inv_rows;
+    kc[2 * STEM_N + c] = a.mean[c];
+    kc[3 * STEM_N + c] = r;
+    kc[4 * STEM_N + c] = a.sums[STEM_N + c] * inv_rows;
+    if (blockIdx.x == 0) {
+      if (a.dgamma != nullptr) a.dgamma[c] += a.sums[STEM_N + c];
+      if (a.dbeta != nullptr) a.dbeta[c] += a.sums[c];
+    }
+  }
+  __syncthreads();
+  if (threadIdx.x == 0) TRACE_POINT();
+  if (live) {
+    stem_build_col(g, m0, sin, tab, scol);
+    if (threadIdx.x == 0) TRACE_POINT();
+    const float* ka = kc;
+    const float* kb = kc + STEM_N;
+    const float* km = kc + 2 * STEM_N;
+    const float* kr = kc + 3 * STEM_N;
+    const float* ks = kc + 4 * STEM_N;
+    for (int i = threadIdx.x; i < STEM_BM * 8; i += STEM_THREADS) {
+      const int m = i >> 3, c8 = i & 7;
+      const int row = m0 + m;
+      const int w = row % g.Wo;
+      const int t = row / g.Wo;
+      const int h = t % g.Ho;
+      const int n = t / g.Ho;
+      float xf[8];
+      unpack8_bn(a.z[static_cast<long long>(row) * 8 + c8], xf);
+      const int hhi = min((h + a.ppad) / a.pstride, a.Hp - 1), whi = min((w + a.ppad) / a.pstride, a.Wp - 1);
+      const int hlo = max(h + a.ppad - a.pk + a.pstride, 0) / a.pstride, wlo = max(w + a.ppad - a.pk + a.pstride, 0) / a.pstride;
+      const long long img = static_cast<long long>(n) * a.Hp;
+      float gr[8] = {0.f, 0.f, 0.f, 0.f, 0.f, 0.f, 0.f, 0.f};
+      auto add_window = [&](int ho, int wo, const uint2 av, const uint4 va, const uint4 vp, const uint4 vb) {
+        float f[8], pf[8];
+        unpack8_bn(va, f);
+        unpack8_bn(vp, pf);
+        if (a.dy_b != nullptr) {
+          float fb[8];
+          unpack8_bn(vb, fb);
+#pragma unroll
+          for (int j = 0; j < 8; ++j) f[j] += fb[j];
+        }
+        const uint32_t tap = static_cast<uint32_t>((h + a.ppad - ho * a.pstride) * a.pk + (w + a.ppad - wo * a.pstride));
+#pragma unroll
+        for (int j = 0; j < 8; ++j) {
+          const uint32_t aj = ((j < 4 ? av.x : av.y) >> (8 * (j & 3))) & 0xffu;
+          if (aj == tap && pf[j] > 0.f) gr[j] += f[j];
+        }
+      };
+      if (hhi - hlo < 2 && whi - wlo < 2) {
+        uint2 av[4];
+        uint4 va[4], vp[4], vb[4];
+#pragma unroll
+        for (int q = 0; q < 4; ++q) {
+          const int ho = hhi - (q >> 1), wo = whi - (q & 1);
+          av[q] = make_uint2(0u, 0u);
+          va[q] = vp[q] = vb[q] = make_uint4(0u, 0u, 0u, 0u);
+          if (ho >= hlo && wo >= wlo) {
+            const long long o = ((img + ho) * a.Wp + wo) * 8 + c8;
+            av[q] = a.arg[o];
+            va[q] = a.dy_a[o];
+            vp[q] = a.p[o];
+            if (a.dy_b != nullptr) vb[q] = a.dy_b[o];
+          }
+        }
+#pragma unroll
+        for (int q = 0; q < 4; ++q) {
+          const int ho = hhi - (q >> 1), wo = whi - (q & 1);
+          if (ho >= hlo && wo >= wlo) add_window(ho, wo, av[q], va[q], vp[q], vb[q]);
+        }
+      } else {
+        for (int ho = hhi; ho >= hlo; --ho)
+          for (int wo = whi; wo >= wlo; --wo) {
+            const long long o = ((img + ho) * a.Wp + wo) * 8 + c8;
+            add_window(ho, wo, a.arg[o], a.dy_a[o], a.p[o], a.dy_b != nullptr ? a.dy_b[o] : make_uint4(0u, 0u, 0u, 0u));
+          }
+      }
+      uint32_t o4[4];
+#pragma unroll
+      for (int j = 0; j < 4; ++j) {
+        const int ca = c8 * 8 + 2 * j, cb = ca + 1;
+        const float xh0 = (xf[2 * j] - km[ca]) * kr[ca], xh1 = (xf[2 * j + 1] - km[cb]) * kr[cb];
+        o4[j] = pack_bf16x2(ka[ca] * (gr[2 * j] - kb[ca] - xh0 * ks[ca]), ka[cb] * (gr[2 * j + 1] - kb[cb] - xh1 * ks[cb]));
+      }
+      *reinterpret_cast<uint4*>(sdz + m * 128 + ((c8 ^ (m & 7)) << 4)) = make_uint4(o4[0], o4[1], o4[2], o4[3]);
+    }
+  }
+  fence_proxy_async();
+  __syncthreads();
+  if (threadIdx.x == 0) TRACE_POINT();
+
+  const int wg = threadIdx.x >> 7;
+  const int num_kt = (g.K + 63) / 64;
+  const int j0 = 2 * wg;
+  const int nj = wg == 0 ? 2 : 1;
+  float acc[2][32];
+#pragma unroll
+  for (int jj = 0; jj < 2; ++jj)
+#pragma unroll
+    for (int e = 0; e < 32; ++e) acc[jj][e] = 0.f;
+  if (live) {
+    const uint32_t a0 = smem_u32(sdz), b0 = smem_u32(scol);
+    wgmma_fence();
+#pragma unroll
+    for (int kk = 0; kk < STEM_BM / 16; ++kk) {
+      const uint64_t ad = gmma_desc_sw128(a0 + kk * 2048, 8192, 1024);
+#pragma unroll
+      for (int jj = 0; jj < 2; ++jj)
+        if (jj < nj && j0 + jj < num_kt)
+          wgmma_bf16_n64<1, 1>(acc[jj], ad, gmma_desc_sw128(b0 + (j0 + jj) * (STEM_BM * 128) + kk * 2048, 8192, 1024), 1u);
+    }
+    wgmma_commit();
+    wgmma_wait<0>();
+  }
+  wgmma_fence_operands(acc[0]);
+  wgmma_fence_operands(acc[1]);
+  if (threadIdx.x == 0) TRACE_POINT();
+
+  __syncthreads();
+  float* part = reinterpret_cast<float*>(smem);
+#pragma unroll
+  for (int jj = 0; jj < 2; ++jj)
+    if (jj < nj) wg_store_acc<64>(acc[jj], part + (j0 + jj) * 64, STEM_WPART_PITCH, 0);
+
+  cluster_sync_all();
+  if (threadIdx.x == 0) TRACE_POINT();
+  const int rank = static_cast<int>(cluster_ctarank());
+  constexpr int ROWS = STEM_N / STEM_CLUSTER;
+  const int c4n = (g.K + 3) / 4;
+  const uint32_t pbase = smem_u32(part);
+  for (int i = threadIdx.x; i < ROWS * c4n; i += STEM_THREADS) {
+    const int rr = rank * ROWS + i / c4n, c4 = (i % c4n) * 4;
+    const uint32_t off = pbase + static_cast<uint32_t>((rr * STEM_WPART_PITCH + c4) * 4);
+    float4 s = make_float4(0.f, 0.f, 0.f, 0.f);
+#pragma unroll
+    for (int peer = 0; peer < STEM_CLUSTER; ++peer) {
+      const float4 t = ld_dsmem_f4(off, static_cast<uint32_t>(peer));
+      s.x += t.x; s.y += t.y; s.z += t.z; s.w += t.w;
+    }
+    float* d = a.dw + static_cast<size_t>(rr) * a.ldd + c4;
+    const float sv[4] = {s.x, s.y, s.z, s.w};
+#pragma unroll
+    for (int e = 0; e < 4; ++e)
+      if (c4 + e < g.K) atomicAdd(d + e, sv[e]);
+  }
+  if (threadIdx.x == 0) TRACE_POINT();
+  cluster_sync_all();
+}
+
+template <class K, class P>
+static int launch_stem(K kernel, unsigned grid, int smem, int cluster, cudaStream_t stream, const P& p, const StemGeom& g) {
+  static bool configured = false;
+  if (!configured) {
+    cudaError_t e = cudaFuncSetAttribute(kernel, cudaFuncAttributeMaxDynamicSharedMemorySize, 227 * 1024);
+    if (e != cudaSuccess) return static_cast<int>(e);
+    e = cudaFuncSetAttribute(kernel, cudaFuncAttributePreferredSharedMemoryCarveout, cudaSharedmemCarveoutMaxShared);
+    if (e != cudaSuccess) return static_cast<int>(e);
+    configured = true;
+  }
+  cudaLaunchConfig_t cfg = {};
+  cfg.gridDim = dim3(grid);
+  cfg.blockDim = dim3(STEM_THREADS);
+  cfg.dynamicSmemBytes = smem;
+  cfg.stream = stream;
+  cudaLaunchAttribute attr[2];
+  int na = 0;
+  if (pdl_enabled()) {
+    attr[na].id = cudaLaunchAttributeProgrammaticStreamSerialization;
+    attr[na].val.programmaticStreamSerializationAllowed = 1;
+    ++na;
+  }
+  if (cluster > 1) {
+    attr[na].id = cudaLaunchAttributeClusterDimension;
+    attr[na].val.clusterDim.x = cluster;
+    attr[na].val.clusterDim.y = 1;
+    attr[na].val.clusterDim.z = 1;
+    ++na;
+  }
+  cfg.attrs = attr;
+  cfg.numAttrs = na;
+  cudaError_t le = cudaLaunchKernelEx(&cfg, kernel, p, g);
+  if (le != cudaSuccess) return static_cast<int>(le);
+  return static_cast<int>(cudaGetLastError());
+}
+
+static int stem_in_bytes(const StemGeom& g) {
+  if (g.N <= 0 || g.Ho <= 0 || g.Wo <= 0 || (g.W * g.C) % 8 != 0 || g.K > STEM_KT * 64 || g.K <= 0 ||
+      (g.Ho * g.Wo) % STEM_BM != 0 || static_cast<long long>(g.N) * g.Ho * g.Wo > (1ll << 30))
+    return -1;
+  const int rows = (g.Wo + STEM_BM - 2) / g.Wo * g.stride + g.KH;
+  const long long bytes = static_cast<long long>(rows) * g.W * g.C * 2;
+  return bytes <= STEM_MAX_IN_BYTES ? static_cast<int>(bytes) : -1;
+}
+
+static StemGeom stem_geom(int N, int H, int W, int C, int KH, int KW, int stride, int pad) {
+  StemGeom g;
+  g.N = N; g.H = H; g.W = W; g.C = C; g.KH = KH; g.KW = KW; g.stride = stride; g.pad = pad;
+  g.Ho = stride > 0 ? (H + 2 * pad - KH) / stride + 1 : 0;
+  g.Wo = stride > 0 ? (W + 2 * pad - KW) / stride + 1 : 0;
+  g.K = KH * KW * C;
+  return g;
+}
+
+constexpr int STEM_FWD_SMEM = STEM_COL_BYTES + STEM_W_BYTES + 4 * 2 * STEM_N * 4 + STEM_TAB_BYTES + 1024;
+constexpr int STEM_BWD_SMEM = STEM_COL_BYTES + STEM_DZ_BYTES + 5 * STEM_N * 4 + STEM_TAB_BYTES + 1024;
+static_assert(STEM_N * STEM_WPART_PITCH * 4 <= STEM_COL_BYTES + STEM_DZ_BYTES, "the weight-gradient partial overlays the operands");
+static_assert(STEM_BM * STEM_PART_PITCH * 4 <= STEM_COL_BYTES, "the forward accumulator tile overlays the im2col tile");
+
+}
+
+extern "C" int b200_stem_conv_fwd(const void* x, const void* w, int ldw, void* z, float* col_stats, int N, int H, int W,
+                                  int C, int KH, int KW, int stride, int pad, cudaStream_t stream) {
+  using namespace b200;
+  const StemGeom g = stem_geom(N, H, W, C, KH, KW, stride, pad);
+  const int in_bytes = stem_in_bytes(g);
+  if (in_bytes < 0 || ldw < g.K || (reinterpret_cast<uintptr_t>(x) & 15) || (reinterpret_cast<uintptr_t>(z) & 15) ||
+      (reinterpret_cast<uintptr_t>(w) & 1))
+    return -2;
+  StemFwdParams p;
+  p.x = reinterpret_cast<const __nv_bfloat16*>(x); p.w = reinterpret_cast<const uint16_t*>(w); p.ldw = ldw;
+  p.z = reinterpret_cast<__nv_bfloat16*>(z); p.col_stats = col_stats;
+  const long long M = static_cast<long long>(N) * g.Ho * g.Wo;
+  return launch_stem(stem_conv_fwd_kernel, static_cast<unsigned>(M / STEM_BM), STEM_FWD_SMEM + in_bytes, 1, stream, p, g);
+}
+
+extern "C" int b200_stem_bn_wgrad(const void* x, const void* z, const void* p, const void* argmax, const void* dy_a,
+                                  const void* dy_b, const float* gamma, const float* save_mean, const float* save_rstd,
+                                  float* sums, float* dgamma, float* dbeta, float* dw, int ldd, int N, int H, int W, int C,
+                                  int KH, int KW, int stride, int pad, int pk, int pstride, int ppad, int Hp, int Wp,
+                                  cudaStream_t stream) {
+  using namespace b200;
+  const StemGeom g = stem_geom(N, H, W, C, KH, KW, stride, pad);
+  const int in_bytes = stem_in_bytes(g);
+  if (in_bytes < 0 || ldd < g.K || pk * pk > 255 || (reinterpret_cast<uintptr_t>(x) & 15) ||
+      (reinterpret_cast<uintptr_t>(z) & 15) || (reinterpret_cast<uintptr_t>(dw) & 3))
+    return -2;
+  int rc = b200_bn_maxpool_bwd_reduce(z, p, argmax, dy_a, dy_b, save_mean, save_rstd, sums, N, g.Ho, g.Wo, STEM_N, pk,
+                                      pstride, ppad, Hp, Wp, stream);
+  if (rc != 0) return rc;
+  StemBwdParams a;
+  a.x = reinterpret_cast<const __nv_bfloat16*>(x); a.z = reinterpret_cast<const uint4*>(z);
+  a.p = reinterpret_cast<const uint4*>(p); a.arg = reinterpret_cast<const uint2*>(argmax);
+  a.dy_a = reinterpret_cast<const uint4*>(dy_a); a.dy_b = reinterpret_cast<const uint4*>(dy_b);
+  a.gamma = gamma; a.mean = save_mean; a.rstd = save_rstd; a.sums = sums; a.dgamma = dgamma; a.dbeta = dbeta;
+  a.dw = dw; a.ldd = ldd;
+  const long long M = static_cast<long long>(N) * g.Ho * g.Wo;
+  a.M = static_cast<int>(M);
+  a.pk = pk; a.pstride = pstride; a.ppad = ppad; a.Hp = Hp; a.Wp = Wp;
+  const long long tiles = M / STEM_BM;
+  const unsigned grid = static_cast<unsigned>((tiles + STEM_CLUSTER - 1) / STEM_CLUSTER * STEM_CLUSTER);
+  return launch_stem(stem_bn_wgrad_kernel, grid, STEM_BWD_SMEM + in_bytes, STEM_CLUSTER, stream, a, g);
+}
+
+B200_TRACE_REGISTER(conv_stem)
diff --git a/baton_b200/csrc/epilogue.cuh b/baton_b200/csrc/epilogue.cuh
--- a/baton_b200/csrc/epilogue.cuh
+++ b/baton_b200/csrc/epilogue.cuh
@@ -11,6 +11,16 @@
 __device__ __forceinline__ void cluster_sync_all() {
   asm volatile("barrier.cluster.arrive.release.aligned;" ::: "memory");
   asm volatile("barrier.cluster.wait.acquire.aligned;" ::: "memory");
+}
+__device__ __forceinline__ float4 ld_dsmem_f4(uint32_t local_smem_addr, uint32_t cta_rank) {
+  uint32_t remote;
+  asm volatile("mapa.shared::cluster.u32 %0, %1, %2;" : "=r"(remote) : "r"(local_smem_addr), "r"(cta_rank));
+  float4 v;
+  asm volatile("ld.shared::cluster.v4.f32 {%0, %1, %2, %3}, [%4];"
+               : "=f"(v.x), "=f"(v.y), "=f"(v.z), "=f"(v.w)
+               : "r"(remote)
+               : "memory");
+  return v;
 }
 
 #define COLSUM_STEP(OFF, HALF)                                                  \
diff --git a/baton_b200/csrc/gemm_wgmma.cu b/baton_b200/csrc/gemm_wgmma.cu
--- a/baton_b200/csrc/gemm_wgmma.cu
+++ b/baton_b200/csrc/gemm_wgmma.cu
@@ -92,17 +92,6 @@
   return v;
 }
 
-__device__ __forceinline__ float4 ld_dsmem_f4(uint32_t local_smem_addr, uint32_t cta_rank) {
-  uint32_t remote;
-  asm volatile("mapa.shared::cluster.u32 %0, %1, %2;" : "=r"(remote) : "r"(local_smem_addr), "r"(cta_rank));
-  float4 v;
-  asm volatile("ld.shared::cluster.v4.f32 {%0, %1, %2, %3}, [%4];"
-               : "=f"(v.x), "=f"(v.y), "=f"(v.z), "=f"(v.w)
-               : "r"(remote)
-               : "memory");
-  return v;
-}
-
 __device__ __forceinline__ void accumulate_col_stats(const GemmParams& p, int col0, const float (&v)[32]) {
   float s[32], q[32];
 #pragma unroll
diff --git a/baton_b200/csrc/launch.h b/baton_b200/csrc/launch.h
--- a/baton_b200/csrc/launch.h
+++ b/baton_b200/csrc/launch.h
@@ -52,6 +52,12 @@
                           cudaStream_t stream);
 int b200_conv_halo(const void* src, const void* w, void* out, int N, int H, int W, int Nout, int dgrad, int mc,
                    float* col_stats, cudaStream_t stream);
+int b200_stem_conv_fwd(const void* x, const void* w, int ldw, void* z, float* col_stats, int N, int H, int W, int C, int KH,
+                       int KW, int stride, int pad, cudaStream_t stream);
+int b200_stem_bn_wgrad(const void* x, const void* z, const void* p, const void* argmax, const void* dy_a, const void* dy_b,
+                       const float* gamma, const float* save_mean, const float* save_rstd, float* sums, float* dgamma,
+                       float* dbeta, float* dw, int ldd, int N, int H, int W, int C, int KH, int KW, int stride, int pad,
+                       int pk, int pstride, int ppad, int Hp, int Wp, cudaStream_t stream);
 int b200_im2col_tma_probe(const void* x, void* col, int N, int H, int W, int C, int KH, int KW, int stride, int pad,
                           int Ho, int Wo, cudaStream_t stream);
 int b200_gemm_fp8(const void* a, const void* b, void* d, const float* bias, const void* sfa, const void* sfb, int M, int N,
@@ -193,6 +199,9 @@
                         const float* gamma, const float* save_mean, const float* save_rstd, float* sums, float* dgamma,
                         float* dbeta, int N, int H, int W, int C, int k, int stride, int pad, int Ho, int Wo,
                         cudaStream_t stream);
+int b200_bn_maxpool_bwd_reduce(const void* z, const void* p, const void* argmax, const void* dy_a, const void* dy_b,
+                               const float* save_mean, const float* save_rstd, float* sums, int N, int H, int W, int C, int k,
+                               int stride, int pad, int Ho, int Wo, cudaStream_t stream);
 int b200_bn_bwd_cluster(const void* x, const void* y, const void* dy_a, const void* dy_b, void* dx, void* dres,
                         const float* gamma, const float* save_mean, const float* save_rstd, float* dgamma, float* dbeta,
                         long long rows, int C, int relu, int max_cluster, cudaStream_t stream);
diff --git a/baton_b200/csrc/norm.cu b/baton_b200/csrc/norm.cu
--- a/baton_b200/csrc/norm.cu
+++ b/baton_b200/csrc/norm.cu
@@ -665,10 +665,6 @@
 }
 
 
-__device__ __forceinline__ void unpack8_bn(const uint4& u, float (&f)[8]) {
-  const float2 a = unpack_bf16x2(u.x), b = unpack_bf16x2(u.y), c = unpack_bf16x2(u.z), d = unpack_bf16x2(u.w);
-  f[0] = a.x; f[1] = a.y; f[2] = b.x; f[3] = b.y; f[4] = c.x; f[5] = c.y; f[6] = d.x; f[7] = d.y;
-}
 __device__ __forceinline__ void colred_finish(float (&a)[8], float (&q)[8], float* sm, int tpr, int cg, int rg,
                                               float* __restrict__ sums, int C) {
   float* mine = sm + static_cast<size_t>(rg) * 2 * C + cg * 8;
@@ -1391,10 +1387,9 @@
              beta, running_mean, running_var, save_mean, save_rstd, nbt, N, H, W, C, k, stride, pad, Ho, Wo, eps, momentum);
   RET_LAST();
 }
-extern "C" int b200_bn_maxpool_bwd(const void* z, const void* p, const void* argmax, const void* dy_a, const void* dy_b,
-                                   void* dz, const float* gamma, const float* save_mean, const float* save_rstd, float* sums,
-                                   float* dgamma, float* dbeta, int N, int H, int W, int C, int k, int stride, int pad, int Ho,
-                                   int Wo, cudaStream_t stream) {
+extern "C" int b200_bn_maxpool_bwd_reduce(const void* z, const void* p, const void* argmax, const void* dy_a,
+                                          const void* dy_b, const float* save_mean, const float* save_rstd, float* sums, int N,
+                                          int H, int W, int C, int k, int stride, int pad, int Ho, int Wo, cudaStream_t stream) {
   if (k * k > 255 || !colred_vec_ok(C, z, p, dy_a) || (dy_b != nullptr && (reinterpret_cast<uintptr_t>(dy_b) & 15)))
     return -2;
   const long long prow = static_cast<long long>(N) * Ho * Wo;
@@ -1405,8 +1400,15 @@
              stream, reinterpret_cast<const __nv_bfloat16*>(z), reinterpret_cast<const uint4*>(p),
              reinterpret_cast<const uint2*>(argmax), reinterpret_cast<const uint4*>(dy_a),
              reinterpret_cast<const uint4*>(dy_b), save_mean, save_rstd, sums, N, H, W, C, k, stride, pad, Ho, Wo, rpc);
-  cudaError_t e = cudaGetLastError();
-  if (e != cudaSuccess) return static_cast<int>(e);
+  RET_LAST();
+}
+extern "C" int b200_bn_maxpool_bwd(const void* z, const void* p, const void* argmax, const void* dy_a, const void* dy_b,
+                                   void* dz, const float* gamma, const float* save_mean, const float* save_rstd, float* sums,
+                                   float* dgamma, float* dbeta, int N, int H, int W, int C, int k, int stride, int pad, int Ho,
+                                   int Wo, cudaStream_t stream) {
+  const int rc = b200_bn_maxpool_bwd_reduce(z, p, argmax, dy_a, dy_b, save_mean, save_rstd, sums, N, H, W, C, k, stride,
+                                            pad, Ho, Wo, stream);
+  if (rc != 0 || static_cast<long long>(N) * Ho * Wo <= 0) return rc;
   const long long total = static_cast<long long>(N) * H * W * (C / 8);
   launch_pdl(bn_maxpool_bwd_apply_kernel, stream_grid(total), 256, 5 * C * sizeof(float), stream,
              reinterpret_cast<const uint4*>(z), reinterpret_cast<const uint4*>(p), reinterpret_cast<const uint2*>(argmax),
diff --git a/baton_b200/csrc/ptx.cuh b/baton_b200/csrc/ptx.cuh
--- a/baton_b200/csrc/ptx.cuh
+++ b/baton_b200/csrc/ptx.cuh
@@ -318,5 +318,9 @@
   __nv_bfloat162 v = *reinterpret_cast<__nv_bfloat162*>(&u);
   return __bfloat1622float2(v);
 }
-
-}
+__device__ __forceinline__ void unpack8_bn(const uint4& u, float (&f)[8]) {
+  const float2 a = unpack_bf16x2(u.x), b = unpack_bf16x2(u.y), c = unpack_bf16x2(u.z), d = unpack_bf16x2(u.w);
+  f[0] = a.x; f[1] = a.y; f[2] = b.x; f[3] = b.y; f[4] = c.x; f[5] = c.y; f[6] = d.x; f[7] = d.y;
+}
+
+}
diff --git a/baton_b200/models/resnet.py b/baton_b200/models/resnet.py
--- a/baton_b200/models/resnet.py
+++ b/baton_b200/models/resnet.py
@@ -37,9 +37,17 @@
     if (stats is None or bn.workspace is None or not bn.relu or not bn.training or bn.num_features % 8
             or bnn._grad_target(bn.weight) is None or bnn._grad_target(bn.bias) is None):
         return None
-    cc = bnn.Ctx()
-    z = bnn._ConvFn.forward(cc, x, conv.weight, conv._w_bf16(), conv.kernel_size, conv.kernel_size, conv.stride,
-                            conv.padding, None, stats, conv.flags_cfg)
+    k, s, pd = conv.kernel_size, conv.stride, conv.padding
+    n, h, w, c_in = x.shape
+    cc = None
+    if (not getattr(conv, "fp8", False) and bnn._grad_target(conv.weight) is not None
+            and bnn.F.stem_eligible(k, k, s, pd, c_in, h, w, conv.out_channels)):
+        wt = conv._w_bf16() if conv.flags_cfg is not None else conv._w_bf16(padded=False)
+        z = bnn.F.stem_conv_fwd(x, wt, k, k, s, pd, col_stats=stats)
+        z = z.view(n, bnn.F.conv_out_size(h, k, s, pd), bnn.F.conv_out_size(w, k, s, pd), conv.out_channels)
+    else:
+        cc = bnn.Ctx()
+        z = bnn._ConvFn.forward(cc, x, conv.weight, conv._w_bf16(), k, k, s, pd, None, stats, conv.flags_cfg)
     if after_conv is not None:
         after_conv()
     c = bn.num_features
@@ -48,16 +56,26 @@
     if out is None:
         raise RuntimeError("bn_relu_maxpool rejected a shape _stem_fwd accepted")
     p, arg, mean, rstd = out
-    return p, cc, z, arg, mean, rstd
-
-
-def _stem_bwd(saved, bn, pool, dy_a, dy_b=None):
-    p, cc, z, arg, mean, rstd = saved
+    return p, cc, x, z, arg, mean, rstd
+
+
+def _stem_bwd(saved, conv, bn, pool, dy_a, dy_b=None):
+    p, cc, x, z, arg, mean, rstd = saved
     c = bn.num_features
     gamma = bnn._unwrap(bn.weight)
     tg, tb = bnn._grad_target(gamma), bnn._grad_target(bnn._unwrap(bn.bias))
-    dz = bnn.F.bn_maxpool_bwd(z, p, arg, dy_a.contiguous(), dy_b.contiguous() if dy_b is not None else None, gamma, mean,
-                              rstd, bn.workspace[2 * c:], tg, tb, pool.k, pool.stride, pool.pad)
+    dy_a = dy_a.contiguous()
+    dy_b = dy_b.contiguous() if dy_b is not None else None
+    if cc is None:
+        k, cout = conv.kernel_size, conv.out_channels
+        tgt = bnn._grad_target(conv.weight)
+        dw = tgt.permute(0, 2, 3, 1).reshape(cout, conv.k_true)
+        assert dw.data_ptr() == tgt.data_ptr(), "conv weight grad must be channels_last in the arena"
+        bnn.F.stem_bn_wgrad(x, z, p, arg, dy_a, dy_b, gamma, mean, rstd, bn.workspace[2 * c:], tg, tb, dw, k, k,
+                            conv.stride, conv.padding, pool.k, pool.stride, pool.pad)
+        return
+    dz = bnn.F.bn_maxpool_bwd(z, p, arg, dy_a, dy_b, gamma, mean, rstd, bn.workspace[2 * c:], tg, tb, pool.k, pool.stride,
+                              pool.pad)
     if dz is None:
         raise RuntimeError("bn_maxpool_bwd rejected a shape bn_relu_maxpool accepted")
     cc.needs_dx = False
@@ -262,7 +280,7 @@
         for bi in range(len(tape) - 1, -1, -1):
             pieces = self._block_bwd(tape[bi], pieces)
         if fused_stem is not None:
-            _stem_bwd(fused_stem, self.bn1, self.maxpool, pieces[0], pieces[1] if len(pieces) > 1 else None)
+            _stem_bwd(fused_stem, self.conv1, self.bn1, self.maxpool, pieces[0], pieces[1] if len(pieces) > 1 else None)
         else:
             d = bnn._MaxPoolFn.backward(cp, pieces[0], pieces[1] if len(pieces) > 1 else None)[0]
             _conv_bn_bwd(stem, d, needs_dx=False)
diff --git a/baton_b200/ops/functional.py b/baton_b200/ops/functional.py
--- a/baton_b200/ops/functional.py
+++ b/baton_b200/ops/functional.py
@@ -324,6 +324,47 @@
     return 4 if tiles % 4 == 0 else 2 if tiles % 2 == 0 else 1
 
 
+STEM_BM = 128
+STEM_MAX_K = 192
+_STEM_MAX_IN_BYTES = 32 * 1024
+
+
+def stem_in_bytes(kh: int, stride: int, c: int, w: int, wo: int) -> int:
+    return ((wo + STEM_BM - 2) // wo * stride + kh) * w * c * 2
+
+
+def stem_eligible(kh: int, kw: int, stride: int, pad: int, c: int, h: int, w: int, cout: int) -> bool:
+    if stride < 1 or pad < 0:
+        return False
+    ho, wo = conv_out_size(h, kh, stride, pad), conv_out_size(w, kw, stride, pad)
+    return (ho > 0 and wo > 0 and (w * c) % 8 == 0 and kh * kw * c <= STEM_MAX_K and cout == 64 and
+            (ho * wo) % STEM_BM == 0 and stem_in_bytes(kh, stride, c, w, wo) <= _STEM_MAX_IN_BYTES)
+
+
+def stem_conv_fwd(x: torch.Tensor, w2d: torch.Tensor, kh: int, kw: int, stride: int, pad: int,
+                  col_stats: Optional[torch.Tensor] = None) -> torch.Tensor:
+    n, h, w, c = x.shape
+    if not stem_eligible(kh, kw, stride, pad, c, h, w, w2d.shape[0]):
+        raise ValueError("the stem kernel does not take this convolution (see stem_eligible)")
+    ho, wo = conv_out_size(h, kh, stride, pad), conv_out_size(w, kw, stride, pad)
+    z = torch.empty((n * ho * wo, 64), dtype=BF16, device=x.device)
+    if not load().stem_conv_fwd(x, w2d, z, col_stats, kh, kw, stride, pad):
+        raise RuntimeError("stem_conv_fwd declined a convolution stem_eligible admits")
+    return z
+
+
+def stem_bn_wgrad(x: torch.Tensor, z: torch.Tensor, p: torch.Tensor, arg: torch.Tensor, dy_a: torch.Tensor,
+                  dy_b: Optional[torch.Tensor], gamma, mean: torch.Tensor, rstd: torch.Tensor, sums_b: torch.Tensor,
+                  dgamma, dbeta, dw2d: torch.Tensor, kh: int, kw: int, stride: int, pad: int, pool_k: int,
+                  pool_stride: int, pool_pad: int) -> None:
+    n, h, w, c = x.shape
+    if not stem_eligible(kh, kw, stride, pad, c, h, w, z.shape[-1]):
+        raise ValueError("the stem kernel does not take this convolution (see stem_eligible)")
+    if not load().stem_bn_wgrad(x, z, p, arg, dy_a, dy_b, gamma, mean, rstd, sums_b, dgamma, dbeta, dw2d, kh, kw, stride,
+                                pad, pool_k, pool_stride, pool_pad):
+        raise RuntimeError("stem_bn_wgrad declined a shape stem_eligible admits")
+
+
 def _conv_path(path: Optional[str], eligible: bool) -> str:
     if path is None:
         return "halo" if eligible else "im2col"
diff --git a/baton_b200/ops/nn.py b/baton_b200/ops/nn.py
--- a/baton_b200/ops/nn.py
+++ b/baton_b200/ops/nn.py
@@ -397,12 +397,12 @@
         self.kp = F.round_up(self.k_true, 8)
         self.flags_cfg = None
 
-    def _w_bf16(self, gated: bool = True):
+    def _w_bf16(self, gated: bool = True, padded: bool = True):
         sh = getattr(self, "weight_bf16", None)
         if sh is None:
             sh = _shadow(self, "weight", self.weight)
         sh = sh.view(self.out_channels, self.k_true)
-        if self.kp != self.k_true:
+        if padded and self.kp != self.k_true:
             sh = F.pad_rows(sh, self.kp, gate=self.flags_cfg if gated else None)
         return sh
 
diff --git a/baton_b200/utils/trace.py b/baton_b200/utils/trace.py
--- a/baton_b200/utils/trace.py
+++ b/baton_b200/utils/trace.py
@@ -8,7 +8,7 @@
 import torch
 
 _TUS = ["?", "gemm_wgmma", "gemm_fp8", "quant", "attention", "im2col_tma", "gemm_simt", "fedavg", "elementwise",
-        "conv", "norm", "loss", "conv_halo"]
+        "conv", "norm", "loss", "conv_halo", "conv_stem"]
 _CSRC = os.path.join(os.path.dirname(os.path.dirname(os.path.abspath(__file__))), "csrc")
 _NAME_CACHE: Dict[int, str] = {}
 
```

Measured after the change: 210,000, median of 6. +2.3%, better.
